# baskuit/R-NaD

Hardware: AMD Instinct MI355X
Metric: env_steps_per_sec (rollout + R-NaD update, one iteration of learn/rnad.py:495-526 per step) (higher is better)
Workload: dtype f32; 1 GPU; depth-6 3x3 matrix tree, C=1, S=66431, global batch 2^20 episodes x T=12 env steps, MLP width 256, BASELINE.json configs[1]; global_batch=1048576, per_gpu_batch=1048576, T=12, T_buffer=12, parallelism=single GPU (no collectives)

## Files before the change

include/rnad_hip.h:

```cpp
#ifndef RNAD_HIP_H
#define RNAD_HIP_H

#include <stdint.h>

#ifdef __cplusplus
extern "C" {
#endif
#pragma GCC visibility push(default)

#define RNAD_MAX_ACTIONS 8
#define RNAD_MAX_TRANSITIONS 8

const char *rnad_last_error(void);
int rnad_version(void);

typedef struct rnad_tree rnad_tree_t;

int rnad_tree_create(rnad_tree_t **out, int64_t S, int C, int A, const int64_t *index, const float *value,
                     const float *chance, const float *expected_value, const float *legal, int device);
void rnad_tree_destroy(rnad_tree_t *tree);
int64_t rnad_tree_info(const rnad_tree_t *tree, int which);

int rnad_observe(const rnad_tree_t *tree, int64_t B, const int32_t *idx, int player, void *obs, int obs_half,
                 uint8_t *mask_bits, float *mask, void *stream);

int rnad_policy_head(int64_t N, int A, const float *logits, const uint8_t *mask_bits, const float *mask,
                     float *policy, float *log_policy, void *stream);

int64_t rnad_mlp_packed_size(int A, int W);
int rnad_mlp_pack(int A, int W, const float *vw0, const float *vb0, const float *vw1, const float *vb1, const float *pw0,
                  const float *pb0, const float *pw1, const float *pb1, float *packed, void *stream);
int rnad_mlp_pack_multi(int n_nets, int A, int W, const float *const *weights, float *const *packed, void *stream);
int rnad_mlp_forward(int64_t N, int A, int W, const float *packed, const void *obs, int obs_half, float *logits,
                     float *value, void *stream);
int rnad_mlp_forward_multi(int n_nets, int64_t N, int A, int W, const float *const *packed, const void *obs, int obs_half,
                           float *const *logits, float *const *value, void *stream);
int64_t rnad_mlp_backward_workspace(int64_t N, int A, int W);
int rnad_mlp_backward(int64_t N, int A, int W, const float *packed, const void *obs, int obs_half, const float *dlogits,
                      const float *dvalue, float *g_vw0, float *g_vb0, float *g_vw1, float *g_vb1, float *g_pw0,
                      float *g_pb0, float *g_pw1, float *g_pb1, float *workspace, void *stream);

int64_t rnad_compact_workspace(int64_t N);
int rnad_compact_valid(int64_t N, const int32_t *indices, int32_t *rows, int64_t *n_rows, int32_t *block_counts, void *stream);
int rnad_mlp_forward_rows(int64_t max_rows, const int32_t *rows, const int64_t *n_rows, int A, int W, const float *packed,
                          const void *obs, int obs_half, float *logits, float *value, void *stream);
int rnad_mlp_backward_rows(int64_t max_rows, const int32_t *rows, const int64_t *n_rows, int A, int W, const float *packed,
                           const void *obs, int obs_half, const float *dlogits, const float *dvalue, float *g_vw0,
                           float *g_vb0, float *g_vw1, float *g_vb1, float *g_pw0, float *g_pb0, float *g_pw1, float *g_pb1,
                           float *workspace, void *stream);

int rnad_conv_supported(int A, int Ch, int depth);
int64_t rnad_conv_packed_size(int A, int Ch, int depth);
int64_t rnad_conv_param_count(int A, int Ch, int depth);
int rnad_conv_pack(int A, int Ch, int depth, const float *const *weights, float *packed, void *stream);
int rnad_conv_forward(int64_t N, const int32_t *rows, const int64_t *n_rows, int A, int Ch, int depth, const float *packed,
                      const float *obs, float *logits, float *value, void *stream);
int64_t rnad_conv_backward_workspace(int64_t N, int A, int Ch, int depth);
int rnad_conv_backward(int64_t N, const int32_t *rows, const int64_t *n_rows, int A, int Ch, int depth, const float *packed,
                       const float *obs, const float *dlogits, const float *dvalue, float *grads, float *workspace, void *stream);

int64_t rnad_mlp_fold_packed_size(int A, int W);
int rnad_mlp_pack_fold_multi(int n_nets, int A, int W, const float *const *weights, float *const *packed, void *stream);
int rnad_mlp_forward_fold(int n_nets, int64_t N, const int32_t *rows, const int64_t *n_rows, int A, int W, const float *const *packed,
                          const void *obs, int obs_half, float *const *logits, float *const *value, void *stream);
int rnad_mlp_forward_actor(const rnad_tree_t *tree, const int32_t *rows, const int64_t *n_rows, int W, int fold, const float *packed,
                           const void *obs, int obs_half, float *logits, float *policy_rows, void *stream);
int rnad_mlp_backward_fold(int64_t N, const int32_t *rows, const int64_t *n_rows, int A, int W, const float *packed, const void *obs,
                           int obs_half, const float *dlogits, const float *dvalue, float *g_vw0, float *g_vb0, float *g_vw1, float *g_vb1,
                           float *g_pw0, float *g_pb0, float *g_pw1, float *g_pb1, float *workspace, void *stream);

int rnad_sample(int64_t B, int n, const float *probs, const float *noise, uint64_t seed, int64_t lane0, int step,
                int stream_id, int32_t *out, void *stream);

int rnad_transition(const rnad_tree_t *tree, int64_t B, const int32_t *idx, const int32_t *row_actions,
                    const int32_t *col_actions, const float *noise, uint64_t seed, int64_t lane0, int step,
                    int32_t *idx_out, float *reward, int32_t *alive, void *stream);

typedef struct rnad_traj {
    int32_t T_cap;
    int32_t obs_half;
    int64_t B;
    int32_t *indices;
    void *observations;
    uint8_t *mask_bits;
    float *policy;
    int32_t *actions;
    float *rewards;
    float *values;
    int32_t *alive;
} rnad_traj_t;

int rnad_rollout_begin(const rnad_tree_t *tree, const rnad_traj_t *traj, void *stream);

int rnad_rollout_step(const rnad_tree_t *tree, const rnad_traj_t *traj, int t, int mode, const float *logits,
                      const float *policy_in, const int32_t *actions_in, const float *value,
                      const float *noise_action, const float *noise_chance, uint64_t seed, int64_t lane0,
                      void *stream);

int rnad_rollout_run(const rnad_tree_t *tree, const rnad_traj_t *traj, int W, const float *packed, float *logits_ws,
                     int64_t logits_step_stride, float *value_ws, uint64_t seed, int64_t lane0, int32_t *live_rows,
                     int64_t *n_live, int32_t *block_counts, void *stream);

int rnad_rollout_run_tabular(const rnad_tree_t *tree, const rnad_traj_t *traj, const float *logits_table,
                             const float *value_table, uint64_t seed, int64_t lane0, void *stream);

int rnad_rollout_end(const rnad_tree_t *tree, const rnad_traj_t *traj, void *stream);

int rnad_process_policy(int64_t N, int A, const float *policy, const float *mask, int n_disc, float eps,
                        float *out, void *stream);

int rnad_vtrace(int T, int64_t B, int A, const float *v, const float *valid, const int32_t *player_id,
                const float *mu, const float *pi, const float *logpi, const void *actions, int actions_onehot,
                const float *reward, int player, float eta, float lambda_, float c, float rho, float gamma,
                float *v_target, int32_t *has_played, float *q, void *stream);

int rnad_mask_sum(int64_t N, const float *mask, double *out, void *stream);
int rnad_loss_v(int64_t N, const float *v, const float *v_target, const float *mask, const double *norm, float weight,
                double *loss, float *dv, int accumulate, void *stream);
int rnad_loss_nerd(int64_t N, int A, const float *logit, const float *pi, const float *q, const float *mask,
                   const float *legal, const double *norm, float clip, float threshold, float weight, double *loss,
                   float *dlogit, int accumulate, void *stream);

typedef struct rnad_learn_params {
    float alpha, one_minus_alpha;
    float eta, lambda_, c, rho, gamma;
    float clip, threshold;
    float w_v, w_n;
    float eps_threshold;
    int32_t n_disc;
} rnad_learn_params_t;

int rnad_learn_fused(int T, int64_t B, int A, const int32_t *indices, const uint8_t *mask_bits,
                     const int32_t *actions, const float *rewards, const float *mu, const float *logit,
                     const float *v, const float *v_target_net, const float *logit_reg, const float *logit_reg_,
                     const double *norm, const rnad_learn_params_t *hp, double *losses, float *dlogit, float *dv,
                     float *pi_out, float *v_target_out, float *q_out, void *stream);

int64_t rnad_learn_tabular_workspace(const rnad_tree_t *tree, int T, int64_t B);
int rnad_learn_fused_tabular(const rnad_tree_t *tree, int T, int64_t B, const int32_t *indices, const uint8_t *mask_bits,
                             const int32_t *actions, const float *rewards, const float *mu, const float *logit_tab,
                             const float *v_tab, const float *v_target_tab, const float *logit_reg_tab,
                             const float *logit_reg_tab_, const double *norm, const rnad_learn_params_t *hp, double *losses,
                             void *workspace, float *dlogit_tab, float *dv_tab, void *stream);
int64_t rnad_row_sums_workspace(const rnad_tree_t *tree);
int rnad_row_sums(const rnad_tree_t *tree, int T, int64_t B, const int32_t *indices, const float *dlogit, const float *dv,
                  void *workspace, float *dlogit_tab, float *dv_tab, void *stream);

int64_t rnad_learn_gather_workspace(const rnad_tree_t *tree);
int rnad_learn_fused_gather(const rnad_tree_t *tree, int T, int64_t B, const int32_t *indices, const uint8_t *mask_bits,
                            const int32_t *actions, const float *rewards, const float *mu, const float *logit_tab,
                            const float *v_tab, const float *v_target_tab, const float *logit_reg_tab,
                            const float *logit_reg_tab_, const double *norm, const rnad_learn_params_t *hp, double *losses,
                            void *workspace, float *dlogit, float *dv, void *stream);

typedef struct rnad_step_params {
    uint64_t seed;
    float alpha, one_minus_alpha;
} rnad_step_params_t;
typedef struct rnad_row_groups {
    int32_t n_groups;
    const int32_t *start;
    const int32_t *order;
    const int32_t *first;
    int32_t rows_below_cut;
} rnad_row_groups_t;

int rnad_step_params_set(rnad_step_params_t *device_params, uint64_t seed, float alpha, float one_minus_alpha, void *stream);
#define RNAD_STEP_QUEUE 32
typedef struct rnad_step_queue {
    rnad_step_params_t live;
    int64_t cursor, n;
    rnad_step_params_t ahead[RNAD_STEP_QUEUE];
} rnad_step_queue_t;
int rnad_step_queue_set(rnad_step_queue_t *device_queue, int n, const rnad_step_params_t *entries, void *stream);
int rnad_bucket_plan(const rnad_tree_t *tree, int64_t B, int64_t *out);
int rnad_bucket_map(const rnad_tree_t *tree, int64_t B, int32_t *bucket_of, int32_t *n_groups);
int rnad_bucket_shared_steps(const rnad_tree_t *tree, int64_t B, int32_t *n_shared);
int rnad_rollout_bucketed(const rnad_tree_t *tree, const rnad_traj_t *traj, const float *table, int64_t table_stride,
                          int table_is_policy, const float *value_table, int64_t value_stride, uint64_t seed, int64_t lane0,
                          const rnad_step_params_t *device_params, void *scratch, int32_t *lane_ids, int32_t *items, int32_t *n_items,
                          double *norm, void *stream);
int rnad_rollout_bucketed_compact(const rnad_tree_t *tree, int T_cap, int64_t B, const float *table, int64_t table_stride,
                                  int table_is_policy, uint64_t seed, int64_t lane0, const rnad_step_params_t *device_params,
                                  void *scratch, int32_t *lane_ids, int32_t *items, int32_t *n_items, double *norm, void *states,
                                  int32_t *alive, uint64_t *acts, float *final_reward, int32_t *visited, void *stream);
int rnad_rollout_bucketed_compact_expand(const rnad_tree_t *tree, int T_cap, int64_t B, const float *table, int64_t table_stride,
                                         int table_is_policy, uint64_t seed, int64_t lane0, const rnad_step_params_t *device_params,
                                         void *scratch, int32_t *lane_ids, int32_t *items, int32_t *n_items, double *norm, void *states,
                                         int32_t *alive, uint64_t *acts, float *final_reward, int32_t *visited, const int32_t *rep_of,
                                         int n_tables, float *const *tables, const int32_t *floats_per_row, void *stream);
#define RNAD_PLAY_LEARN_FINISH 1
#define RNAD_PLAY_LEARN_DISTINCT 2
typedef struct rnad_leaf_paths {
    int64_t n_cols;
    int32_t rows, T_cap;
    const void *states;
    const uint64_t *acts;
    const float *final_reward;
    const int32_t *items;
    const int32_t *n_items;
    int32_t max_items;
    const int32_t *col_of;
    int32_t *col_count;
    const int32_t *bucket_col0;
    int32_t crowded_lanes;
} rnad_leaf_paths_t;
int rnad_leaf_paths_pack(const rnad_tree_t *tree, int64_t plan_B, int T1, int64_t n_cols, const int32_t *indices, const int32_t *items,
                         const int32_t *n_items, int32_t max_items, void *states, int32_t *mismatch, int32_t *rows_out, int32_t *rel_bytes_out,
                         void *stream);
int rnad_rollout_learn_bucketed_compact(const rnad_tree_t *tree, int T_cap, int64_t B, const float *table, int64_t table_stride,
                                        uint64_t seed, int64_t lane0, const rnad_step_params_t *device_params, void *scratch,
                                        int32_t *lane_ids, int32_t *items, int32_t *n_items, double *norm, void *states, int32_t *alive,
                                        uint64_t *acts, float *final_reward, const int32_t *rep_of, int n_tables, float *const *tables,
                                        const int32_t *floats_per_row, const float *fast_records, const rnad_learn_params_t *hp,
                                        void *accumulators, int flags, const double *norm_global, float *dlogit_tab, float *dv_tab,
                                        const int32_t *rows, const int64_t *n_rows, const rnad_row_groups_t *groups,
                                        const rnad_leaf_paths_t *leaf, void *stream);
int rnad_bucket_indices(const rnad_tree_t *tree, int T1, int64_t B, const void *states, const int32_t *items, const int32_t *n_items,
                        int32_t *indices, void *stream);
int rnad_bucket_pack_states(const rnad_tree_t *tree, int T1, int64_t B, const int32_t *indices, const int32_t *items,
                            const int32_t *n_items, void *states, int32_t *mismatch, void *stream);
int rnad_bucket_expand(const rnad_tree_t *tree, int T, int64_t B, const int32_t *indices, const uint64_t *acts,
                       const float *final_reward, const float *records, uint8_t *mask_bits, float *policy, int32_t *actions,
                       float *rewards, void *stream);
int rnad_bucket_log_stats(const rnad_tree_t *tree, int T, int64_t B, const void *states, const int32_t *items, const int32_t *n_items,
                          const int32_t *alive, const float *records, const float *logit_target_tab, float *row_stats, double *out,
                          void *stream);
int64_t rnad_bucket_record_stride(int A);
int64_t rnad_bucket_fast_record_stride(int A);
int64_t rnad_bucket_policy_row_stride(int A);
int rnad_bucket_records(const rnad_tree_t *tree, const float *logit_tab, const float *v_tab, const float *v_target_tab,
                        const float *logit_reg_tab, const float *logit_reg_tab_, const rnad_learn_params_t *hp,
                        const rnad_step_params_t *device_params, float *records, float *fast_records, float *policy_rows,
                        const int32_t *rows, const int64_t *n_rows, void *stream);
int rnad_rows_expand(int64_t rows, const int32_t *rep_of, int n_tables, float *const *tables, const int32_t *floats_per_row, void *stream);
int rnad_rows_segment_sum(int n_groups, const int32_t *start, const int32_t *order, int A, float *dlogit_tab, float *dv_tab, void *stream);

int rnad_mlp_rows_records_supported(int A, int W, int fold, int policy_from_table);
int rnad_mlp_rows_actor_supported(int A, int W, int fold);
int rnad_mlp_rows_actor(const rnad_tree_t *tree, const int32_t *rows, const int64_t *n_rows, int W, int fold, const float *packed, const void *obs,
                        int obs_half, float *logits, float *policy_rows, void *stream);
int rnad_mlp_rows_records(const rnad_tree_t *tree, int W, int fold, const float *packed_net, const float *packed_target, const void *obs,
                          int obs_half, const int32_t *rows, const int64_t *n_rows, int policy_from_table, float *logit_tab, float *v_tab,
                          float *v_target_tab, const float *logit_reg_tab, const float *logit_reg_tab_, const rnad_learn_params_t *hp,
                          const rnad_step_params_t *device_params, float *records, float *fast_records, float *policy_rows, void *stream);
int rnad_learn_bucketed(const rnad_tree_t *tree, int T, int64_t B, const int32_t *indices, const int32_t *actions,
                        const float *rewards, const float *mu, const float *records, const int32_t *items, const int32_t *n_items,
                        const double *norm, const rnad_learn_params_t *hp, void *accumulators, double *losses, float *dlogit_tab,
                        float *dv_tab, void *stream);
int rnad_learn_bucketed_compact(const rnad_tree_t *tree, int T, int64_t B, const void *states, const uint64_t *acts,
                                const float *final_reward, const float *fast_records, const float *records, const int32_t *items,
                                const int32_t *n_items, const double *norm, const rnad_learn_params_t *hp, void *accumulators,
                                double *losses, float *dlogit_tab, float *dv_tab, const int32_t *rows, const int64_t *n_rows,
                                const void *rollout_scratch, int rollout_T_cap, int32_t *alive, double *norm_out,
                                const rnad_row_groups_t *groups, void *stream);
int rnad_bucket_alive(const rnad_tree_t *tree, int T_cap, int64_t B, const void *scratch, int32_t *alive, double *norm, void *stream);
int rnad_bucket_sort(const rnad_tree_t *tree, int T_cap, int64_t B, const float *table, int64_t table_stride, int table_is_policy,
                     uint64_t seed, int64_t lane0, const rnad_step_params_t *device_params, void *scratch, int32_t *lane_ids,
                     int32_t *items, int32_t *n_items, double *norm, int32_t *group_flags, int32_t *staged_rows, int64_t *n_staged,
                     int32_t *visited, void *stage, int32_t *stage_rows0, void *stream);
int64_t rnad_bucket_stage_bytes(const rnad_tree_t *tree, int64_t B);
int rnad_bucket_stage_rows(const rnad_tree_t *tree, int64_t B, int level, uint64_t seed, const rnad_step_params_t *device_params, void *stage,
                           int32_t *rows, void *stream);
int rnad_bucket_stage_walk(const rnad_tree_t *tree, int T_cap, int64_t B, const float *policy_rows, int64_t stride, uint64_t seed, int64_t lane0,
                           const rnad_step_params_t *device_params, const void *scratch, const int32_t *lane_ids, void *stage, void *stream);
int rnad_bucket_play(const rnad_tree_t *tree, int T_cap, int64_t B, const float *table, int64_t table_stride, int table_is_policy,
                     const int32_t *rows, const int64_t *n_rows, uint64_t seed, int64_t lane0, const rnad_step_params_t *device_params,
                     void *scratch, const int32_t *lane_ids, const int32_t *items, const int32_t *n_items, double *norm, void *states,
                     int32_t *alive, uint64_t *acts, float *final_reward, int32_t *visited, int visited_is_clear, void *stream);
int rnad_bucket_finish(const rnad_tree_t *tree, int64_t B, const double *norm, const rnad_learn_params_t *hp, void *accumulators,
                       double *losses, float *dlogit_tab, float *dv_tab, const int32_t *rows, const int64_t *n_rows,
                       const rnad_row_groups_t *groups, void *stream);

int rnad_clip_grad_norm(int64_t n, float *grads, float max_norm, float *total_norm, void *stream);

typedef struct rnad_adam_params {
    float lr, beta1, beta2, eps;
    float max_norm;
    float ema;
} rnad_adam_params_t;
int rnad_optimizer_step(int n_tensors, const int64_t *sizes, float *const *param, float *grads, float *const *exp_avg,
                        float *const *exp_avg_sq, float *const *step, float *const *target, const rnad_adam_params_t *hp,
                        float *total_norm, int mlp_A, int mlp_W, int mlp_fold, float *packed_param, float *packed_target, rnad_step_queue_t *advance,
                        uint32_t *ticket, void *stream);
int rnad_nashconv(const rnad_tree_t *tree, const float *joint_policy, const float *root_policy,
                  int64_t state_index, float reach, float *row_best, float *col_best, float *reach_out,
                  int32_t *depth_out, void *stream);
int rnad_observe_all(const rnad_tree_t *tree, float *obs_row, float *obs_col, void *stream);

int64_t rnad_tree_generate(int A, int C, int depth_bound, float transition_threshold, const float *terminal_values,
                           int n_terminal_values, int prune_num, int prune_den, uint64_t seed, int64_t capacity,
                           int64_t *index, float *value, float *chance, float *expected_value, float *legal,
                           float *root_value, float *solution);
int rnad_solve_matrix(const float *M, int ra, int ca, int max_actions, float *solution, float *value);

int rnad_prof_enable(int mask);
int rnad_prof_read(int which, int64_t *launches, double *total_ms);

#pragma GCC visibility pop
#ifdef __cplusplus
}
#endif
#endif
```

r-nad_amd/csrc/bucket.hip:

```cpp
#include "learn_math.hpp"
#include "row_records.hpp"
#include "rollout_math.hpp"

#include <algorithm>
#include <cstdlib>
#include <utility>

using namespace rnad;
using namespace rnad::dev;

#ifndef RNAD_ABLATE
#define RNAD_ABLATE 0
#endif

namespace {

constexpr int kThreads = 256;
constexpr int kMaxPath = 32;
#ifndef RNAD_PATH_SLOTS
#define RNAD_PATH_SLOTS 16
#endif
constexpr int kPathSlots = RNAD_PATH_SLOTS;
constexpr int kMaxBuckets = 12288;
constexpr int kMaxUpper = 8192;
constexpr int kSortThreads = 1024;
constexpr int kSortLanes = 4096;
constexpr int kChunkDefault = 256;
constexpr int kReplicas = 64;
constexpr int kMaxSteps = 64;
constexpr int kLaneBits = 22;
constexpr int kLearnLds = 64 * 1024;
constexpr int kKeysLds = 144 * 1024;
constexpr int kPackedSteps = 10;
constexpr int kCompactSteps = 21;
constexpr int kSharedRoot = 256;
constexpr int kFinishRows = 4;
constexpr int kTicketGroups = 64;
constexpr int kTargetLanes = 1024;
constexpr int kMinLanesLevelCut = 128;

#ifndef RNAD_PLAY_LDS
#define RNAD_PLAY_LDS 1
#endif
constexpr int kPlayLds = RNAD_PLAY_LDS;
constexpr int kMinSortTile = kSortThreads * kPlayLds > 1024 ? kSortThreads * kPlayLds : 1024;
#define RNAD_DISPATCH_TILE(p_, ...)                                                          \
    switch ((p_).tile) {                                                                     \
        case 1024: { constexpr int kTile = kMinSortTile > 1024 ? kMinSortTile : 1024; __VA_ARGS__; } break; \
        case 2048: { constexpr int kTile = kMinSortTile > 2048 ? kMinSortTile : 2048; __VA_ARGS__; } break; \
        case 8192: { constexpr int kTile = 8192; __VA_ARGS__; } break;                        \
        default: { constexpr int kTile = kSortLanes; __VA_ARGS__; } break;                    \
    }

inline unsigned blocks_for(int64_t n, int per = kThreads) { return (unsigned)((n + per - 1) / per); }

struct Switch {
    bool set;
    int v;
};
struct Switches {
    Switch bucket_rows;
    Switch bucket_chunk;
    Switch sort_tile;
    Switch keys_stage_bytes;
    Switch keys_global;
    Switch keys_lds;
    Switch keys_hybrid;
    Switch expand_blocks;
    Switch scatter_rows;
    Switch fused_distinct;
    Switch fused_chunk;
};
Switches read_switches() {
    auto read = [](const char *name) {
        const char *text = getenv(name);
        return text ? Switch{true, atoi(text)} : Switch{false, 0};
    };
    return {read("RNAD_BUCKET_ROWS"), read("RNAD_BUCKET_CHUNK"), read("RNAD_SORT_TILE"), read("RNAD_KEYS_STAGE_BYTES"),
            read("RNAD_KEYS_GLOBAL"), read("RNAD_KEYS_LDS"), read("RNAD_KEYS_HYBRID"), read("RNAD_EXPAND_BLOCKS"),
            read("RNAD_SCATTER_ROWS"), read("RNAD_FUSED_DISTINCT"), read("RNAD_FUSED_CHUNK")};
}

struct Plan {
    const BucketCut *cut = nullptr;
    int lds = 0, path_words = 0, sort_blocks = 0, chunk = kChunkDefault;
    int tile = kSortLanes;
    int rel_bytes = 1;
    int forced = 0;
    int64_t max_items = 0;
};

struct UpperWalk {
    int32_t next, key;
    float chance;
};

__global__ __launch_bounds__(kThreads) void k_upper_walk(int n, int AAC, const int32_t *__restrict__ upper_list, const Trans *__restrict__ trans,
                                                         const int32_t *__restrict__ bucket_of, UpperWalk *__restrict__ out) {
    const int i = blockIdx.x * kThreads + threadIdx.x;
    if (i >= n * AAC) return;
    const Trans t = trans[(int64_t)upper_list[i / AAC] * AAC + i % AAC];
    out[i] = UpperWalk{t.next, bucket_of[t.next], t.chance};
}

struct HostCut {
    int rows = 0, n_groups = 0, n_upper = 0, n_buckets = 0, max_path = 0;
    std::vector<int32_t> bucket_of, lo, span, path, upper_list, path_states;
    std::vector<int32_t> group_by_lo;
    std::vector<int32_t> anchor1;
};

HostCut build_cut(const rnad_tree_t *tree, int rows) {
    HostCut h;
    h.rows = rows;
    const int64_t S = tree->S;
    std::vector<int32_t> &bucket_of = h.bucket_of, &lo = h.lo, &span = h.span, &path = h.path, &upper_list = h.upper_list;
    bucket_of.assign((size_t)S, -1);
    h.anchor1.assign((size_t)S, 0);
    auto anchor_below = [&](int64_t c) {
        for (int64_t i = tree->child_offsets[(size_t)c]; i < tree->child_offsets[(size_t)c + 1]; ++i) {
            const int64_t d = tree->children[(size_t)i], d_hi = d + tree->subtree_size[(size_t)d];
            for (int64_t x = d; x < d_hi; ++x) h.anchor1[(size_t)x] = (int32_t)d;
        }
    };
    std::vector<int32_t> parent_upper((size_t)S, 0);
    std::vector<int32_t> group_parent;
    auto is_upper = [&](int64_t s) { return tree->subtree_size[(size_t)s] > rows; };
    if (!is_upper(1)) {
        lo.push_back(1);
        span.push_back((int32_t)tree->subtree_size[1]);
        path.push_back(kSharedRoot);
        group_parent.push_back(0);
        anchor_below(1);
        for (int64_t s = 1; s < S; ++s)
            if (tree->level_of[(size_t)s] >= 0) bucket_of[(size_t)s] = 0;
    } else {
        for (int64_t u = 1; u < S; ++u) {
            if (tree->level_of[(size_t)u] < 0 || !is_upper(u)) continue;
            upper_list.push_back((int32_t)u);
            const int level = tree->level_of[(size_t)u];
            int64_t g_lo = -1, g_hi = -1;
            int g_subtrees = 0;
            auto close = [&]() {
                if (g_lo < 0) return;
                const int32_t gid = (int32_t)lo.size();
                lo.push_back((int32_t)g_lo);
                span.push_back((int32_t)(g_hi - g_lo));
                path.push_back(2 * (level + 1) | (g_subtrees == 1 ? kSharedRoot : 0));
                group_parent.push_back((int32_t)u);
                for (int64_t x = g_lo; x < g_hi; ++x) bucket_of[(size_t)x] = gid;
                g_lo = g_hi = -1;
            };
            for (int64_t i = tree->child_offsets[(size_t)u]; i < tree->child_offsets[(size_t)u + 1]; ++i) {
                const int64_t c = tree->children[(size_t)i];
                if (is_upper(c)) {
                    parent_upper[(size_t)c] = (int32_t)u;
                    close();
                    continue;
                }
                const int64_t c_hi = c + tree->subtree_size[(size_t)c];
                anchor_below(c);
                if (g_lo >= 0 && c == g_hi && c_hi - g_lo <= rows) {
                    g_hi = c_hi;
                    ++g_subtrees;
                } else {
                    close();
                    g_lo = c;
                    g_hi = c_hi;
                    g_subtrees = 1;
                }
            }
            close();
        }
    }
    h.n_groups = (int)lo.size();
    h.n_upper = (int)upper_list.size();
    h.n_buckets = h.n_groups + h.n_upper;
    for (int i = 0; i < h.n_upper; ++i) {
        const int32_t u = upper_list[(size_t)i];
        bucket_of[(size_t)u] = h.n_groups + i;
        lo.push_back(u);
        span.push_back(0);
        path.push_back(2 * tree->level_of[(size_t)u] + 2);
        group_parent.push_back(u);
    }
    int max_path = 0;
    for (int32_t v : path) max_path = std::max(max_path, (int)(v & (kSharedRoot - 1)) + ((v & kSharedRoot) ? 2 : 0));
    h.max_path = max_path;
    const int stride = std::max(max_path, 1);
    h.path_states.assign((size_t)h.n_buckets * stride, 0);
    if (max_path <= kMaxPath) {
        for (int b = 0; b < h.n_buckets; ++b) {
            int32_t *row = h.path_states.data() + (size_t)b * stride;
            for (int32_t u = group_parent[(size_t)b]; u != 0; u = parent_upper[(size_t)u]) {
                const int l = tree->level_of[(size_t)u];
                row[2 * l] = row[2 * l + 1] = u;
            }
            if (path[(size_t)b] & kSharedRoot) {
                const int n_path = path[(size_t)b] & (kSharedRoot - 1);
                row[n_path] = row[n_path + 1] = lo[(size_t)b];
            }
        }
    }
    if (upper_list.empty()) upper_list.push_back(0);
    h.group_by_lo.resize((size_t)h.n_groups);
    for (int g = 0; g < h.n_groups; ++g) h.group_by_lo[(size_t)g] = g;
    std::sort(h.group_by_lo.begin(), h.group_by_lo.end(), [&](int32_t a, int32_t b) { return lo[(size_t)a] < lo[(size_t)b]; });
    return h;
}

bool cut_fits(const HostCut &c) { return c.n_buckets <= kMaxBuckets && c.n_upper <= kMaxUpper && c.max_path <= kMaxPath; }

const BucketCut *get_cut(const rnad_tree_t *tree, int rows, const Switches &sw) {
    auto it = tree->cuts.find(rows);
    if (it != tree->cuts.end()) return &it->second;
    HostCut h = build_cut(tree, rows);
    BucketCut cut;
    cut.rows = rows;
    cut.n_groups = h.n_groups;
    cut.n_upper = h.n_upper;
    cut.n_buckets = h.n_buckets;
    cut.max_path = h.max_path;
    DeviceGuard guard(tree->device);
    auto up = [&](int32_t **dst, const std::vector<int32_t> &src) {
        if (hipMalloc((void **)dst, std::max<size_t>(src.size(), 1) * sizeof(int32_t)) != hipSuccess) return false;
        return src.empty() || hipMemcpy(*dst, src.data(), src.size() * sizeof(int32_t), hipMemcpyHostToDevice) == hipSuccess;
    };
    if (!guard.ok || !up(&cut.bucket_of, h.bucket_of) || !up(&cut.bucket_lo, h.lo) || !up(&cut.bucket_path, h.path) ||
        !up(&cut.upper_list, h.upper_list) || !up(&cut.path_states, h.path_states) || !up(&cut.bucket_span, h.span) ||
        !up(&cut.group_by_lo, h.group_by_lo) || !up(&cut.anchor1, h.anchor1)) {
        for (int32_t *ptr : {cut.bucket_of, cut.bucket_lo, cut.bucket_path, cut.upper_list, cut.path_states, cut.bucket_span, cut.group_by_lo, cut.anchor1})
            if (ptr) (void)hipFree(ptr);
        return nullptr;
// ... 546 lines not shown
                }
            }
        }
#pragma unroll
        for (int l = 0; l < L; ++l) {
            const int64_t b = b0 + (int64_t)l * kSortThreads;
            my_keys[pass][l] = b < B ? key[l] : -1;
            if (b < B) {
                keys[b] = key[l];
                decisions[b] = packed[l] | ((unsigned long long)min(steps[l], kPackedSteps) << 60);
                if (stage.root) {
                    const int root = key[l] < n_groups ? state[l] : 0;
                    stage.root[b] = (uint32_t)root | ((uint32_t)steps[l] << kStageRootBits);
                    if (root) stage.mark0[root] = stage_stamp(seed);
                }
            }
        }
    }
    __syncthreads();
    int32_t *cnt = reinterpret_cast<int32_t *>(keys_smem);
    for (int i = threadIdx.x; i < n_buckets; i += kSortThreads) cnt[i] = 0;
    __syncthreads();
#pragma unroll
    for (int pass = 0; pass < kPasses; ++pass)
#pragma unroll
        for (int l = 0; l < L; ++l)
            if (my_keys[pass][l] >= 0) atomicAdd(&cnt[my_keys[pass][l]], 1);
    __syncthreads();
    int32_t *row = hist + (int64_t)blockIdx.x * n_buckets;
    for (int i = threadIdx.x; i < n_buckets; i += kSortThreads) row[i] = cnt[i];
}

template <int TILE>
__global__ __launch_bounds__(kSortThreads) void k_bucket_hist(int64_t B, int n_buckets, const int32_t *__restrict__ keys,
                                                              int32_t *__restrict__ hist) {
    extern __shared__ int32_t cnt[];
    for (int i = threadIdx.x; i < n_buckets; i += kSortThreads) cnt[i] = 0;
    __syncthreads();
    const int64_t base = (int64_t)blockIdx.x * TILE;
#pragma unroll
    for (int r = 0; r < TILE / kSortThreads; ++r) {
        const int64_t b = base + (int64_t)r * kSortThreads + threadIdx.x;
        if (b < B) atomicAdd(&cnt[keys[b]], 1);
    }
    __syncthreads();
    int32_t *row = hist + (int64_t)blockIdx.x * n_buckets;
    for (int i = threadIdx.x; i < n_buckets; i += kSortThreads) row[i] = cnt[i];
}

#ifndef RNAD_XCD_ITEMS
#define RNAD_XCD_ITEMS 1
#endif
__device__ __forceinline__ int xcd_item(int n) {
#if RNAD_XCD_ITEMS
    const int q = n >> 3, r = n & 7, xcd = (int)blockIdx.x & 7, k = (int)blockIdx.x >> 3;
    const int cnt = q + (xcd < r ? 1 : 0), start = xcd < r ? xcd * (q + 1) : r * (q + 1) + (xcd - r) * q;
    return k < cnt ? start + k : -1;
#else
    return (int)blockIdx.x < n ? (int)blockIdx.x : -1;
#endif
}

constexpr int kStagePer = 4;
template <int LEVEL>
__device__ __forceinline__ void stage_rows_chunk(int64_t chunk, int64_t S, const uint32_t *__restrict__ mark, const int32_t *__restrict__ anchor1,
                                                 uint32_t stamp, int32_t *__restrict__ rows, unsigned long long *__restrict__ count) {
    __shared__ int32_t wave_n[kSortThreads / 64];
    __shared__ unsigned long long base_s;
    const int lane = threadIdx.x & 63, wave = threadIdx.x >> 6;
    const int64_t s0 = (chunk * (kSortThreads / 64) + wave) * (kStagePer * 64) + lane;
    uint64_t votes[kStagePer];
    int32_t mine = 0;
#pragma unroll
    for (int r = 0; r < kStagePer; ++r) {
        const int64_t s = s0 + r * 64;
        bool hit = false;
        if (s > 0 && s < S) {
            if (LEVEL == 0) {
                hit = mark[s] == stamp;
            } else {
                const int32_t a = anchor1[s];
                hit = a != 0 && mark[a] == stamp;
            }
        }
        votes[r] = __ballot(hit);
        mine += (int32_t)__popcll(votes[r]);
    }
    if (lane == 0) wave_n[wave] = mine;
    __syncthreads();
    int32_t before = 0, total = 0;
#pragma unroll
    for (int w = 0; w < kSortThreads / 64; ++w) {
        if (w < wave) before += wave_n[w];
        total += wave_n[w];
    }
    if (threadIdx.x == 0) base_s = total ? atomicAdd(count, 2ull * (unsigned long long)total) : 0ull;
    __syncthreads();
    unsigned long long at = base_s + 2ull * (unsigned long long)before;
#pragma unroll
    for (int r = 0; r < kStagePer; ++r) {
        if ((votes[r] >> lane) & 1ull) {
            const unsigned long long mine_at = at + 2ull * (unsigned long long)__popcll(votes[r] & ((1ull << lane) - 1ull));
            rows[mine_at] = (int32_t)(s0 + r * 64);
            rows[mine_at + 1] = (int32_t)(S + s0 + r * 64);
        }
        at += 2ull * (unsigned long long)__popcll(votes[r]);
    }
    __syncthreads();
}

template <int LEVEL>
__global__ __launch_bounds__(kSortThreads) void k_stage_rows(int64_t S, const uint32_t *__restrict__ mark, const int32_t *__restrict__ anchor1,
                                                             uint64_t seed, const rnad_step_params_t *__restrict__ sp,
                                                             int32_t *__restrict__ rows, unsigned long long *__restrict__ count) {
    if (sp) seed = sp->seed;
    stage_rows_chunk<LEVEL>(blockIdx.x, S, mark, anchor1, stage_stamp(seed), rows, count);
}

template <int A>
__global__ __launch_bounds__(kThreads) void k_stage_walk(const Trans *__restrict__ trans, int C, int64_t S, int64_t B, int T_cap,
                                                         const float *__restrict__ policy_tab, int64_t tab_stride, int vec4,
                                                         const uint32_t *__restrict__ sorted, const int32_t *__restrict__ lane_ids,
                                                         uint64_t seed, const rnad_step_params_t *__restrict__ sp, int64_t lane0,
                                                         uint32_t *__restrict__ mark1) {
    const int nb = (int)gridDim.x, xq = nb >> 3, xr = nb & 7, xcd = (int)blockIdx.x & 7, xk = (int)blockIdx.x >> 3;
    const int64_t blk = (xcd < xr ? xcd * (xq + 1) : xr * (xq + 1) + (xcd - xr) * xq) + xk;
    if (xk >= xq + (xcd < xr ? 1 : 0)) return;
    const int64_t j = blk * kThreads + threadIdx.x;
    if (j >= B) return;
    const uint32_t word = sorted[j];
    const int root = (int)(word & ((1u << kStageRootBits) - 1u)), t = (int)(word >> kStageRootBits);
    if (root == 0 || t + 1 >= T_cap) return;
    if (sp) seed = sp->seed;
    const int64_t b = lane_ids[j];
    float pol0[A], pol1[A], u[3];
    load_policy_row<A>(policy_tab, root, tab_stride, vec4 != 0, pol0);
    load_policy_row<A>(policy_tab, S + root, tab_stride, vec4 != 0, pol1);
    rnad_decision_uniforms(seed, (uint64_t)(lane0 + b), (uint32_t)t, u);
    const int a0 = pick<A>(pol0, u[0]), a1 = pick<A>(pol1, u[1]);
    int next;
    float rew;
    transition_lane<A>(trans, C, root, a0, a1, nullptr, u[2], next, rew);
    if (next != 0) mark1[next] = stage_stamp(seed);
}

constexpr int kScanCols = 16, kScanParts = kSortThreads / kScanCols;

struct Item {
    int32_t begin, count, bucket, single;
};

constexpr int kItemsInline = 16;

__device__ __forceinline__ void items_phase(int n_buckets, int chunk, const int32_t *__restrict__ totals, int32_t *__restrict__ start_s,
                                            int32_t *__restrict__ first_s, bool write_items, Item *__restrict__ items,
                                            int32_t *__restrict__ n_items, int32_t *__restrict__ bucket_start_out = nullptr) {
    __shared__ int32_t wave_l[16], wave_i[16];
    __shared__ int32_t total_s, most;
    if (threadIdx.x == 0) most = 0;
    __syncthreads();
    const int per = (n_buckets + kSortThreads - 1) / kSortThreads;
    const int b0 = min(n_buckets, (int)threadIdx.x * per), b1 = min(n_buckets, b0 + per);
    int32_t own_l = 0, own_i = 0;
    bool big = false;
    for (int i = b0; i < b1; ++i) {
        const int32_t n = totals[i], ni = (n + chunk - 1) / chunk;
        own_l += n;
        own_i += ni;
        big |= ni > kItemsInline;
    }
    if (big) most = kItemsInline + 1;
    int32_t sl = own_l, si = own_i;
#pragma unroll
    for (int off = 1; off < 64; off <<= 1) {
        const int32_t a = __shfl_up(sl, off, 64), b = __shfl_up(si, off, 64);
        if ((int)(threadIdx.x & 63) >= off) {
            sl += a;
            si += b;
        }
    }
    if ((threadIdx.x & 63) == 63) {
        wave_l[threadIdx.x >> 6] = sl;
        wave_i[threadIdx.x >> 6] = si;
    }
    __syncthreads();
    int32_t run_l = sl - own_l, run_i = si - own_i;
    for (int w = 0; w < (int)(threadIdx.x >> 6); ++w) {
        run_l += wave_l[w];
        run_i += wave_i[w];
    }
    if (threadIdx.x == kSortThreads - 1) total_s = run_i + own_i;
    for (int i = b0; i < b1; ++i) {
        const int32_t n = totals[i], ni = (n + chunk - 1) / chunk;
        start_s[i] = run_l;
        first_s[i] = run_i;
        if (write_items && bucket_start_out) bucket_start_out[i] = run_l;
        run_l += n;
        run_i += ni;
    }
    __syncthreads();
    const int32_t total = total_s;
    if (threadIdx.x == 0) {
        first_s[n_buckets] = total;
        if (write_items) *n_items = total;
    }
    __syncthreads();
    if (!write_items) return;
    if (most <= kItemsInline) {
        for (int i = threadIdx.x; i < n_buckets; i += kSortThreads) {
            const int32_t n = totals[i], first = first_s[i], ni = first_s[i + 1] - first, start = start_s[i];
            for (int32_t j = 0; j < ni; ++j) items[first + j] = Item{start + j * chunk, min(chunk, n - j * chunk), i, ni == 1 ? 1 : 0};
        }
        return;
    }
    for (int32_t k = threadIdx.x; k < total; k += kSortThreads) {
        int lo = 0, hi = n_buckets;
        while (hi - lo > 1) {
            const int mid = (lo + hi) >> 1;
            if (first_s[mid] <= k) lo = mid;
            else hi = mid;
        }
        const int32_t n = totals[lo], j = k - first_s[lo], start = start_s[lo];
        items[k] = Item{start + j * chunk, min(chunk, n - j * chunk), lo, n <= chunk ? 1 : 0};
    }
}

__global__ __launch_bounds__(kSortThreads) void k_bucket_scan(int n_blocks, int n_buckets, int32_t *__restrict__ hist,
                                                              int32_t *__restrict__ totals, int scan_blocks, KeysExpand ex) {
    if ((int)blockIdx.x >= scan_blocks) {
        keys_expand_share(ex, kSortThreads, (int)blockIdx.x - scan_blocks, (int)gridDim.x - scan_blocks);
        return;
    }
    __shared__ int32_t part[kScanParts][kScanCols + 1];
    const int col = threadIdx.x & (kScanCols - 1), g = threadIdx.x / kScanCols;
    const int c = blockIdx.x * kScanCols + col;
    const int per = (n_blocks + kScanParts - 1) / kScanParts, r0 = min(n_blocks, g * per), r1 = min(n_blocks, r0 + per);
    constexpr int kScanKeep = 16;
    const bool keep = per <= kScanKeep;
    int32_t v[kScanKeep];
    int32_t sum = 0;
    if (c < n_buckets) {
        if (keep) {
#pragma unroll
            for (int k = 0; k < kScanKeep; ++k) v[k] = r0 + k < r1 ? hist[(int64_t)(r0 + k) * n_buckets + c] : 0;
#pragma unroll
            for (int k = 0; k < kScanKeep; ++k) sum += v[k];
        } else {
            for (int r = r0; r < r1; ++r) sum += hist[(int64_t)r * n_buckets + c];
        }
    }
    part[g][col] = sum;
    __syncthreads();
    if (g == 0) {
        int32_t run = 0;
        for (int i = 0; i < kScanParts; ++i) {
            const int32_t x = part[i][col];
            part[i][col] = run;
            run += x;
        }
        if (c < n_buckets) totals[c] = run;
    }
    __syncthreads();
    if (c < n_buckets) {
        int32_t before = part[g][col];
        if (keep) {
#pragma unroll
            for (int k = 0; k < kScanKeep; ++k) {
                if (r0 + k < r1) hist[(int64_t)(r0 + k) * n_buckets + c] = before;
                before += v[k];
            }
        } else {
            for (int r = r0; r < r1; ++r) {
                const int32_t x = hist[(int64_t)r * n_buckets + c];
                hist[(int64_t)r * n_buckets + c] = before;
                before += x;
            }
        }
    }
}

template <int TILE>
__global__ __launch_bounds__(kSortThreads) void k_bucket_scatter(int64_t B, int n_buckets, const int32_t *__restrict__ keys,
                                                                 const int32_t *__restrict__ hist, const int32_t *__restrict__ totals, int chunk,
                                                                 Item *__restrict__ items, int32_t *__restrict__ n_items,
                                                                 int32_t *__restrict__ lane_ids, int wave_rows, int64_t S, int n_groups,
                                                                 const int32_t *__restrict__ bucket_lo, const int32_t *__restrict__ bucket_span,
                                                                 const int32_t *__restrict__ group_by_lo, int32_t *__restrict__ staged_rows,
                                                                 int64_t *__restrict__ n_staged, int32_t *__restrict__ visited,
                                                                 const uint32_t *__restrict__ stage_root, uint32_t *__restrict__ stage_sorted,
                                                                 const uint32_t *__restrict__ stage_mark0, int32_t *__restrict__ stage_rows0,
                                                                 unsigned long long *__restrict__ stage_count0, uint64_t seed,
                                                                 const rnad_step_params_t *__restrict__ sp, int32_t *__restrict__ bucket_start_out) {
    extern __shared__ int32_t cnt[];
    const int wave = threadIdx.x >> 6, lane = threadIdx.x & 63;
    const int64_t base = (int64_t)blockIdx.x * TILE + (int64_t)wave * (TILE / 16);
    int32_t key[TILE / kSortThreads];
    uint32_t root_word[TILE / kSortThreads];
#pragma unroll
    for (int r = 0; r < TILE / kSortThreads; ++r) {
        const int64_t b = base + r * 64 + lane;
        key[r] = b < B ? keys[b] : -1;
        root_word[r] = (stage_root && b < B) ? stage_root[b] : 0u;
    }
    if (visited) {
        for (int64_t r = (int64_t)blockIdx.x * kSortThreads + threadIdx.x; r < 2 * S; r += (int64_t)gridDim.x * kSortThreads)
            visited[r] = (r == 0 || r == S) ? 1 : 0;
    }
    if (stage_rows0) {
        if (sp) seed = sp->seed;
        const int64_t n_chunks = (S + kSortThreads * kStagePer - 1) / (kSortThreads * kStagePer);
        for (int64_t chunk = blockIdx.x; chunk < n_chunks; chunk += gridDim.x)
            stage_rows_chunk<0>(chunk, S, stage_mark0, nullptr, stage_stamp(seed), stage_rows0, stage_count0);
    }
    if (staged_rows) {
        __shared__ int32_t wave_s[16];
        __shared__ int32_t carry_s;
        int32_t *pre = cnt;
        if (threadIdx.x == 0) carry_s = 0;
        __syncthreads();
        for (int k0 = 0; k0 < n_groups; k0 += kSortThreads) {
            const int k = k0 + threadIdx.x;
            const int g = k < n_groups ? group_by_lo[k] : 0;
            const int32_t n = (k < n_groups && totals[g] > 0) ? bucket_span[g] : 0;
            int32_t incl = n;
#pragma unroll
            for (int off = 1; off < 64; off <<= 1) {
                const int32_t o = __shfl_up(incl, off, 64);
                if (lane >= off) incl += o;
            }
            if (lane == 63) wave_s[wave] = incl;
            __syncthreads();
            int32_t before = carry_s;
            for (int w = 0; w < wave; ++w) before += wave_s[w];
            if (k < n_groups) pre[k] = before + incl - n;
            __syncthreads();
            if (threadIdx.x == kSortThreads - 1) carry_s = before + incl;
            __syncthreads();
        }
        const int32_t total = carry_s;
        if (blockIdx.x == 0 && threadIdx.x == 0) *n_staged = 2 * (int64_t)total;
        for (int k = blockIdx.x * 16 + wave; k < n_groups; k += gridDim.x * 16) {
            const int g = group_by_lo[k];
            if (totals[g] <= 0) continue;
            const int32_t lo = bucket_lo[g], n = bucket_span[g], at = pre[k];
            for (int j = lane; j < n; j += 64) {
                staged_rows[at + j] = lo + j;
                staged_rows[total + at + j] = (int32_t)S + lo + j;
            }
        }
        __syncthreads();
    }
    const int32_t *row = hist + (int64_t)blockIdx.x * n_buckets;
    const int32_t row_first = (int)threadIdx.x < n_buckets ? row[threadIdx.x] : 0;
    items_phase(n_buckets, chunk, totals, cnt, cnt + n_buckets, blockIdx.x == 0, items, n_items, bucket_start_out);
    __syncthreads();
    if ((int)threadIdx.x < n_buckets) cnt[threadIdx.x] += row_first;
    for (int i = threadIdx.x + kSortThreads; i < n_buckets; i += kSortThreads) cnt[i] += row[i];
    __syncthreads();
    const int R = wave_rows, G = 16 / R, my_row = wave / G;
    int32_t *wcnt = cnt + 2 * n_buckets + 1;
    for (int i = threadIdx.x; i < R * n_buckets; i += kSortThreads) wcnt[i] = 0;
    __syncthreads();
    int32_t rank[TILE / kSortThreads];
    for (int turn = 0; turn < G; ++turn) {
        if (wave % G == turn) {
#pragma unroll
            for (int r = 0; r < TILE / kSortThreads; ++r) rank[r] = key[r] >= 0 ? atomicAdd(&wcnt[my_row * n_buckets + key[r]], 1) : 0;
        }
        __syncthreads();
    }
    for (int i = threadIdx.x; i < n_buckets; i += kSortThreads) {
        int32_t at = cnt[i];
        for (int w = 0; w < R; ++w) {
            const int32_t n = wcnt[w * n_buckets + i];
            wcnt[w * n_buckets + i] = at;
            at += n;
        }
    }
    __syncthreads();
#pragma unroll
    for (int r = 0; r < TILE / kSortThreads; ++r)
        if (key[r] >= 0) {
            const int32_t at = wcnt[my_row * n_buckets + key[r]] + rank[r];
            lane_ids[at] = (int32_t)(base + r * 64 + lane);
            if (stage_sorted) stage_sorted[at] = root_word[r];
        }
}

template <int A>
__global__ __launch_bounds__(kThreads) void k_bucket_rollout(const Trans *__restrict__ trans, int C, int64_t S, int64_t B, int T_cap,
                                                             const float *__restrict__ policy_tab, int64_t tab_stride,
                                                             const float *__restrict__ value_tab, int64_t value_stride,
                                                             const uint8_t *__restrict__ mask_tab, uint64_t seed,
                                                             const rnad_step_params_t *__restrict__ sp, int64_t lane0,
                                                             const int32_t *__restrict__ lane_ids,
                                                             const unsigned long long *__restrict__ decisions, int32_t *__restrict__ indices,
                                                             uint8_t *__restrict__ mbits, float *__restrict__ policy,
                                                             int32_t *__restrict__ actions, float *__restrict__ rewards,
                                                             float *__restrict__ values, int32_t *__restrict__ alive_part) {
    __shared__ int32_t cnt[kThreads / 64][kMaxSteps + 1];
    const int64_t j = (int64_t)blockIdx.x * kThreads + threadIdx.x;
    const bool active = j < B;
    if (sp) seed = sp->seed;
    const int32_t lane_local = active ? lane_ids[j] : 0;
    const uint64_t lane = (uint64_t)(lane0 + lane_local);
    const unsigned long long packed = active ? decisions[lane_local] : 0ull;
    const int n_packed = (int)(packed >> 60);
    const int wave = threadIdx.x >> 6;
    int state = 1, prev = 0;
    float u[3] = {0.0f, 0.0f, 0.0f};
    for (int t = 0; t < T_cap; ++t) {
        const uint64_t live = __ballot(active && state != 0);
        if ((threadIdx.x & 63) == 0) cnt[wave][t] = (int32_t)__popcll(live);
        if (active) {
            if (!(t & 1) && t + 1 >= n_packed) rnad_decision_uniforms(seed, lane, (uint32_t)t, u);
            const int64_t i = (int64_t)t * B + j;
            const int64_t row = (int64_t)(t & 1) * S + state;
            const bool replay = t < n_packed;
            const int bits6 = replay ? (int)(packed >> (6 * t)) & 63 : 0;
            int action = bits6 & 7;
            const uint32_t bits = mask_tab[row];
            float pol[A];
#pragma unroll
            for (int a = 0; a < A; ++a) pol[a] = policy_tab[row * tab_stride + a];
            if (!replay) action = pick<A>(pol, u[t & 1]);
            indices[i] = state;
            mbits[i] = (uint8_t)bits;
#pragma unroll
            for (int a = 0; a < A; ++a) policy[i * A + a] = pol[a];
            actions[i] = action;
            if (values) values[i] = value_tab ? value_tab[row * value_stride] : 0.0f;
            int next = state;
            float rew = 0.0f;
            if (t & 1) {
                if (replay)
                    transition_apply<A>(trans, C, state, prev, action, bits6 >> 3, next, rew);
                else
                    transition_lane<A>(trans, C, state, prev, action, nullptr, u[2], next, rew);
            } else {
                prev = action;
            }
            rewards[i] = rew;
            state = next;
        }
    }
    const uint64_t live = __ballot(active && state != 0);
    if ((threadIdx.x & 63) == 0) cnt[wave][T_cap] = (int32_t)__popcll(live);
    if (active) indices[(int64_t)T_cap * B + j] = state;
    __syncthreads();
    if ((int)threadIdx.x <= T_cap) {
        int32_t s = 0;
#pragma unroll
        for (int w = 0; w < kThreads / 64; ++w) s += cnt[w][threadIdx.x];
        alive_part[(int64_t)blockIdx.x * (T_cap + 1) + threadIdx.x] = s;
    }
}

template <typename T>
__device__ __forceinline__ const T *at_bytes(const void *base, uint32_t byte_offset) {
    return reinterpret_cast<const T *>(reinterpret_cast<const char *>(base) + byte_offset);
}
template <typename T>
__device__ __forceinline__ T *at_bytes(void *base, uint32_t byte_offset) {
    return reinterpret_cast<T *>(reinterpret_cast<char *>(base) + byte_offset);
}

template <typename REL>
__device__ __forceinline__ REL rel_of(int state, int lo) {
    return (REL)(state == 0 ? 0 : state - lo + 1);
}

#ifndef RNAD_ROLLOUT_LANES
#define RNAD_ROLLOUT_LANES 1
#endif
constexpr int kRolloutLanes = RNAD_ROLLOUT_LANES;

struct Hand {
    unsigned long long acts, relq;
    float reward;
    int final_rel;
};
constexpr int kHandPairs = 4;

struct Distinct {
    int32_t *count = nullptr;
    int32_t *n = nullptr;
    int32_t *key = nullptr;
    int32_t *column = nullptr;
    int codes = 0;
    int keys = 0;
};

constexpr int kLeafHist = 1024;
struct LeafCount {
    int32_t *col_count = nullptr;
    const int32_t *bucket_col0 = nullptr;
    const int32_t *lane_total = nullptr;
    int32_t crowded_lanes = 0;
};
__device__ __forceinline__ bool leaf_crowded(const LeafCount &lc, int bucket) {
    return lc.col_count != nullptr && lc.crowded_lanes > 0 && lc.lane_total[bucket] >= lc.crowded_lanes &&
           lc.bucket_col0[bucket + 1] - lc.bucket_col0[bucket] <= kLeafHist;
}

template <int A, typename REL, int L, bool DISTINCT = false, bool HIST = false>
__device__ __forceinline__ void rollout_items_body(const Trans *__restrict__ trans, int C, int64_t S, int64_t B, int T_cap,
                                                                   const float *__restrict__ policy_tab, int64_t tab_stride, int vec4,
                                                                   uint64_t seed, const rnad_step_params_t *__restrict__ sp, int64_t lane0,
                                                                   const int32_t *__restrict__ lane_ids,
                                                                   const unsigned long long *__restrict__ decisions,
                                                                   const Item *__restrict__ items, const int32_t *__restrict__ n_items,
                                                                   const int32_t *__restrict__ bucket_path, const int32_t *__restrict__ bucket_lo,
                                                                   const int32_t *__restrict__ path_states, int path_stride, int n_groups,
                                                                   REL *__restrict__ states, int32_t *__restrict__ alive_part,
                                                                   unsigned long long *__restrict__ acts_out,
                                                                   float *__restrict__ reward_out, int32_t *__restrict__ visited,
                                                                   double *__restrict__ norm_rep = nullptr, Hand *hand = nullptr,
                                                                   const Distinct distinct = Distinct{},
                                                                   const int32_t *__restrict__ col_of = nullptr,
                                                                   int32_t *__restrict__ leaf_col = nullptr, const LeafCount lc = LeafCount{}) {
    constexpr int NT = kThreads / L, NW = NT / 64;
    __shared__ int32_t leaf_hist[HIST ? kLeafHist : 1];
    static_assert(NT >= 64 && NT > kCompactSteps, "a wave at least, and a thread per alive counter");
    __shared__ int32_t cnt[NW][kMaxSteps + 1];
    int32_t *my_alive = alive_part + (norm_rep ? (int64_t)(blockIdx.x & (kReplicas - 1)) : (int64_t)blockIdx.x) * (T_cap + 1);
    const int my_item = xcd_item(*n_items);
    if (my_item < 0) {
        if (!norm_rep && (int)threadIdx.x <= T_cap) my_alive[threadIdx.x] = 0;
        return;
    }
    const Item item = items[my_item];
    if (sp) seed = sp->seed;
    const int wave = threadIdx.x >> 6;
    const int path_word = bucket_path[item.bucket];
    const bool shared = item.bucket < n_groups && (path_word & kSharedRoot) != 0;
    const int n_shared = (path_word & (kSharedRoot - 1)) + (shared ? 2 : 0);
    const int lo = bucket_lo[item.bucket];
    const int32_t *my_path = path_states + (int64_t)item.bucket * path_stride;
    const uint32_t B32 = (uint32_t)B;
    if ((threadIdx.x & 63) == 0)
        for (int t = 0; t <= T_cap; ++t) cnt[wave][t] = 0;
    bool count_here = false;
    int32_t col0 = 0, n_bins = 0;
    if constexpr (HIST) {
        count_here = leaf_crowded(lc, item.bucket);
        if (count_here) {
            col0 = lc.bucket_col0[item.bucket];
            n_bins = lc.bucket_col0[item.bucket + 1] - col0;
            for (int i = threadIdx.x; i < n_bins; i += NT) leaf_hist[i] = 0;
            __syncthreads();
        }
    }
    for (int base = 0; base < item.count; base += kThreads) {
        bool active[L];
        uint32_t j[L];
        int32_t lane_local[L];
        uint64_t lane[L];
        unsigned long long packed[L];
#pragma unroll
        for (int l = 0; l < L; ++l) {
            const int k = base + l * NT + (int)threadIdx.x;
            active[l] = k < item.count;
            j[l] = (uint32_t)(item.begin + k);
            lane_local[l] = active[l] ? lane_ids[j[l]] : 0;
            lane[l] = (uint64_t)(lane0 + lane_local[l]);
        }
        if (shared) {
            const unsigned long long first = decisions[lane_ids[item.begin]];
            const unsigned long long uni = ((unsigned long long)(unsigned int)__builtin_amdgcn_readfirstlane((int)(first >> 32)) << 32) |
                                           (unsigned int)__builtin_amdgcn_readfirstlane((int)first);
#pragma unroll
            for (int l = 0; l < L; ++l) packed[l] = uni;
        } else {
#pragma unroll
            for (int l = 0; l < L; ++l) packed[l] = active[l] ? decisions[lane_local[l]] : 0ull;
        }
        int state[L], n_packed[L], t_from = 0;
        unsigned long long relq = 0ull;
        int last_key[L];
        unsigned long long acts[L];
        float reward_final[L];
#pragma unroll
        for (int l = 0; l < L; ++l) {
            n_packed[l] = (int)(packed[l] >> 60);
            last_key[l] = -1;
            state[l] = active[l] ? 1 : 0;
            acts[l] = 0ull;
            reward_final[l] = 0.0f;
        }
        if (shared) {
            const int n_pre = min(min(n_packed[0], T_cap) & ~1, n_shared - 2);
            int32_t live_now = 0;
#pragma unroll
            for (int l = 0; l < L; ++l) live_now += (int32_t)__popcll(__ballot(active[l]));
            for (int t = 0; t < n_pre; t += 2) {
                if ((threadIdx.x & 63) == 0) {
                    cnt[wave][t] += live_now;
                    cnt[wave][t + 1] += live_now;
                }
                const int bits0 = (int)(packed[0] >> (6 * t)) & 63, bits1 = (int)(packed[0] >> (6 * (t + 1))) & 63;
                if (visited && threadIdx.x == 0 && base == 0) {
                    const int at = my_path[t];
                    visited[at] = visited[S + at] = 1;
                }
#pragma unroll
                for (int l = 0; l < L; ++l)
                    acts[l] |= (unsigned long long)(bits0 & 7) << (3 * t) | (unsigned long long)(bits1 & 7) << (3 * (t + 1));
            }
            t_from = n_pre;
#pragma unroll
            for (int l = 0; l < L; ++l) state[l] = active[l] ? my_path[n_pre] : 0;
        }
        for (int t = t_from; t < T_cap; t += 2) {
            const bool two = t + 1 < T_cap;
            int32_t live = 0;
#pragma unroll
            for (int l = 0; l < L; ++l) live += (int32_t)__popcll(__ballot(state[l] != 0));
            if ((threadIdx.x & 63) == 0) {
                cnt[wave][t] += live;
                if (two) cnt[wave][t + 1] += live;
            }
            bool go[L], replay0[L], replay1[L];
            float pol0[L][A], pol1[L][A], u[L][3];
#pragma unroll
            for (int l = 0; l < L; ++l) {
                go[l] = active[l];
                if (go[l] && t >= n_shared) {
                    const REL r = rel_of<REL>(state[l], lo);
                    if (hand && l == 0) relq = (relq << 16) | (unsigned long long)r;
                    *at_bytes<REL>(states, ((uint32_t)t * B32 + j[l]) * (uint32_t)sizeof(REL)) = r;
                    if (two) *at_bytes<REL>(states, ((uint32_t)(t + 1) * B32 + j[l]) * (uint32_t)sizeof(REL)) = r;
                }
                go[l] = go[l] && state[l] != 0;
                replay0[l] = t < n_packed[l];
                replay1[l] = t + 1 < n_packed[l];
                if (go[l]) {
                    const int64_t row0 = state[l], row1 = S + state[l];
                    if (visited) {
                        visited[row0] = 1;
                        if (two) visited[row1] = 1;
                    }
                    if (!replay0[l]) load_policy_row<A>(policy_tab, row0, tab_stride, vec4 != 0, pol0[l]);
                    if (two && !replay1[l]) load_policy_row<A>(policy_tab, row1, tab_stride, vec4 != 0, pol1[l]);
                }
            }
#pragma unroll
            for (int l = 0; l < L; ++l)
                if (go[l] && (!replay0[l] || (two && !replay1[l]))) rnad_decision_uniforms(seed, lane[l], (uint32_t)t, u[l]);
            int a0[L], a1[L], bits1[L];
#pragma unroll
            for (int l = 0; l < L; ++l) {
                if (!go[l]) continue;
                const int bits0 = replay0[l] ? (int)(packed[l] >> (6 * t)) & 63 : 0;
                bits1[l] = replay1[l] ? (int)(packed[l] >> (6 * (t + 1))) & 63 : 0;
                a0[l] = replay0[l] ? (bits0 & 7) : pick<A>(pol0[l], u[l][0]);
                acts[l] |= (unsigned long long)a0[l] << (3 * t);
                if (two) {
                    a1[l] = replay1[l] ? (bits1[l] & 7) : pick<A>(pol1[l], u[l][1]);
                    acts[l] |= (unsigned long long)a1[l] << (3 * (t + 1));
                }
            }
            if (two) {
#pragma unroll
                for (int l = 0; l < L; ++l) {
                    if (!go[l]) continue;
                    int next, outcome;
                    float rew;
                    if (replay1[l]) {
                        outcome = bits1[l] >> 3;
                        transition_apply<A>(trans, C, state[l], a0[l], a1[l], outcome, next, rew);
                    } else {
                        transition_lane<A>(trans, C, state[l], a0[l], a1[l], nullptr, u[l][2], next, rew, &outcome);
                    }
                    if (next == 0) {
                        reward_final[l] = rew;
                        if (DISTINCT) last_key[l] = (state[l] - lo) * distinct.codes + (a0[l] * A + a1[l]) * C + outcome;
                        if (leaf_col)
                        {
                            const int32_t col = col_of[(((uint32_t)state[l] * A + a0[l]) * A + a1[l]) * C + outcome];
                            leaf_col[j[l]] = col;
                            if constexpr (HIST)
                                if (count_here) atomicAdd(&leaf_hist[col - col0], 1);
                        }

                    }
                    state[l] = next;
                }
            }
        }
        int32_t live = 0;
#pragma unroll
        for (int l = 0; l < L; ++l) {
            if (active[l]) {
                acts_out[j[l]] = acts[l];
                reward_out[j[l]] = reward_final[l];
                if (T_cap >= n_shared) *at_bytes<REL>(states, ((uint32_t)T_cap * B32 + j[l]) * (uint32_t)sizeof(REL)) = rel_of<REL>(state[l], lo);
            }
            live += (int32_t)__popcll(__ballot(state[l] != 0));
        }
        if ((threadIdx.x & 63) == 0) cnt[wave][T_cap] += live;
        if (DISTINCT) {
#pragma unroll
            for (int l = 0; l < L; ++l) {
                if (!active[l]) continue;
                const int key = state[l] != 0 ? (state[l] - lo) * distinct.codes + distinct.codes - 1 : last_key[l];
                const bool in_table = key >= 0 && key < distinct.keys;
                if (!in_table || atomicAdd(distinct.count + key, 1) == 0) {
                    const int at = atomicAdd(distinct.n, 1);
                    distinct.key[at] = in_table ? key : distinct.keys;
                    distinct.column[at] = (int32_t)j[l];
                }
            }
        }
        if (hand) *hand = Hand{acts[0], relq, reward_final[0], active[0] ? (int)rel_of<REL>(state[0], lo) : 0};
    }
    __syncthreads();
    if constexpr (HIST) {
        if (count_here) {
            for (int i = threadIdx.x; i < n_bins; i += NT) {
                const int32_t n = leaf_hist[i];
                if (n != 0) atomicAdd(lc.col_count + col0 + i, n);
            }
        }
    }
    if ((int)threadIdx.x <= T_cap) {
        int32_t sum = 0;
#pragma unroll
        for (int w = 0; w < NW; ++w) sum += cnt[w][threadIdx.x];
        if (!norm_rep) my_alive[threadIdx.x] = sum;
        else if (sum != 0) atomicAdd(my_alive + threadIdx.x, sum);
        if (norm_rep) cnt[0][threadIdx.x] = sum;
    }
    if (norm_rep) {
        __syncthreads();
        if (threadIdx.x < 2) {
            int32_t n = 0;
            for (int t = threadIdx.x; t < T_cap; t += 2) n += cnt[0][t];
            if (n != 0) atomicAdd(norm_rep + 2 * (blockIdx.x & (kReplicas - 1)) + threadIdx.x, (double)n);
        }
    }
}

template <int A, typename REL, int L>
__global__ __launch_bounds__(kThreads / L) void k_bucket_rollout_items(const Trans *__restrict__ trans, int C, int64_t S, int64_t B, int T_cap,
                                                                   const float *__restrict__ policy_tab, int64_t tab_stride, int vec4,
                                                                   uint64_t seed, const rnad_step_params_t *__restrict__ sp, int64_t lane0,
                                                                   const int32_t *__restrict__ lane_ids,
                                                                   const unsigned long long *__restrict__ decisions,
                                                                   const Item *__restrict__ items, const int32_t *__restrict__ n_items,
                                                                   const int32_t *__restrict__ bucket_path, const int32_t *__restrict__ bucket_lo,
                                                                   const int32_t *__restrict__ path_states, int path_stride, int n_groups,
                                                                   REL *__restrict__ states, int32_t *__restrict__ alive_part,
                                                                   unsigned long long *__restrict__ acts_out,
                                                                   float *__restrict__ reward_out, int32_t *__restrict__ visited) {
    rollout_items_body<A, REL, L>(trans, C, S, B, T_cap, policy_tab, tab_stride, vec4, seed, sp, lane0, lane_ids, decisions, items, n_items,
                                  bucket_path, bucket_lo, path_states, path_stride, n_groups, states, alive_part, acts_out, reward_out, visited);
}

template <typename REL>
__global__ __launch_bounds__(kThreads) void k_bucket_indices(int T1, int64_t B, const Item *__restrict__ items, const int32_t *__restrict__ n_items,
                                                             const int32_t *__restrict__ bucket_path, const int32_t *__restrict__ bucket_lo,
                                                             const int32_t *__restrict__ path_states, int path_stride, int n_groups,
                                                             const REL *__restrict__ states, int32_t *__restrict__ indices) {
    if ((int)blockIdx.x >= *n_items) return;
    const Item item = items[blockIdx.x];
    const int path_word = bucket_path[item.bucket];
    const int n_shared = (path_word & (kSharedRoot - 1)) + ((item.bucket < n_groups && (path_word & kSharedRoot)) ? 2 : 0);
    const int lo = bucket_lo[item.bucket];
    const int32_t *my_path = path_states + (int64_t)item.bucket * path_stride;
    for (int k = threadIdx.x; k < item.count; k += kThreads) {
        const int64_t j = (int64_t)item.begin + k;
        for (int t = 0; t < T1; ++t) {
            int state;
            if (t < n_shared) {
                state = my_path[t];
            } else {
                const int r = (int)states[(int64_t)t * B + j];
                state = r == 0 ? 0 : lo + r - 1;
            }
            indices[(int64_t)t * B + j] = state;
        }
    }
}

template <typename REL>
__global__ __launch_bounds__(kThreads) void k_bucket_pack(int T1, int64_t B, int rows, const Item *__restrict__ items, const int32_t *__restrict__ n_items,
                                                          const int32_t *__restrict__ bucket_path, const int32_t *__restrict__ bucket_lo,
                                                          const int32_t *__restrict__ path_states, int path_stride, int n_groups,
                                                          const int32_t *__restrict__ indices, REL *__restrict__ states,
                                                          int32_t *__restrict__ bad, int max_count) {
    if ((int)blockIdx.x >= *n_items) return;
    const Item item = items[blockIdx.x];
    if (item.count > max_count && threadIdx.x == 0) *bad = 1;
    const int path_word = bucket_path[item.bucket];
    const int n_shared = (path_word & (kSharedRoot - 1)) + ((item.bucket < n_groups && (path_word & kSharedRoot)) ? 2 : 0);
    const int lo = bucket_lo[item.bucket];
    const int32_t *my_path = path_states + (int64_t)item.bucket * path_stride;
    for (int k = threadIdx.x; k < item.count; k += kThreads) {
        const int64_t j = (int64_t)item.begin + k;
        for (int t = 0; t < T1; ++t) {
            const int state = indices[(int64_t)t * B + j];
            if (t < n_shared) {
                if (state != my_path[t]) *bad = 1;
            } else {
                if (state != 0 && (state < lo || state - lo >= rows)) *bad = 1;
                states[(int64_t)t * B + j] = rel_of<REL>(state, lo);
            }
        }
    }
}

constexpr int kLogStat = 8;
enum { LOG_E = 0, LOG_ET = 1, LOG_K = 2, LOG_N = 3, LOG_SUM = 4, LOG_MIN = 5, LOG_MAX = 6, LOG_SPARE = 7 };

__device__ __forceinline__ unsigned long long ordered_of(double d) {
    const unsigned long long u = (unsigned long long)__double_as_longlong(d);
    return (u >> 63) ? ~u : (u | 0x8000000000000000ull);
}
__device__ __forceinline__ double double_of_ordered(unsigned long long e) {
    return __longlong_as_double((long long)((e >> 63) ? (e & 0x7fffffffffffffffull) : ~e));
}

template <int A>
__global__ __launch_bounds__(kThreads) void k_log_row_stats(int64_t rows, const float *__restrict__ rec_, const float *__restrict__ logit_target,
                                                            float *__restrict__ row_stats, double *__restrict__ out) {
    if (blockIdx.x == 0 && threadIdx.x < kLogStat) {
        double init = 0.0;
        if (threadIdx.x == LOG_MIN) init = __longlong_as_double((long long)ordered_of(__longlong_as_double(0x7ff0000000000000ll)));
        if (threadIdx.x == LOG_MAX) init = __longlong_as_double((long long)ordered_of(__longlong_as_double((long long)0xfff0000000000000ull)));
        out[threadIdx.x] = init;
    }
    const int64_t r = (int64_t)blockIdx.x * kThreads + threadIdx.x;
    if (r >= rows) return;
    constexpr int RS = kRowStride<A>;
    float rec[RS];
    const float4 *rp = reinterpret_cast<const float4 *>(rec_ + r * RS);
#pragma unroll
    for (int u = 0; u < RS / 4; ++u) {
        const float4 r4 = rp[u];
        rec[4 * u] = r4.x; rec[4 * u + 1] = r4.y; rec[4 * u + 2] = r4.z; rec[4 * u + 3] = r4.w;
    }
    const uint32_t bits = __float_as_uint(rec[3 * A + 2]) & ((1u << A) - 1u);
    float lt[A], pit[A], lpt[A];
#pragma unroll
    for (int a = 0; a < A; ++a) lt[a] = logit_target[r * A + a];
    policy_head<A>(lt, bits, pit, lpt);
    const float log_q = logf(1.0f / (float)__popc(bits));
    float e = 0.0f, et = 0.0f, k = 0.0f, sum = 0.0f, lo = rec[0], hi = rec[0];
#pragma unroll
    for (int a = 0; a < A; ++a) {
        const float lg = rec[a], pi = rec[3 * A + 3 + a];
        sum += lg;
        lo = fminf(lo, lg);
        hi = fmaxf(hi, lg);
        if ((bits >> a) & 1) {
            const float log_pi = logf(pi);
            e += pi * (log_pi - log_q);
            et += pit[a] * (logf(pit[a]) - log_q);
            k += pi * (log_pi - log_pi);
        }
    }
    float4 *o4 = reinterpret_cast<float4 *>(row_stats + r * kLogStat);
    o4[0] = float4{e, et, k, sum};
    o4[1] = float4{lo, hi, 0.0f, 0.0f};
}

struct LogAcc {
    double s[5] = {0.0, 0.0, 0.0, 0.0, 0.0};
    float lo = __builtin_inff(), hi = -__builtin_inff();
    __device__ __forceinline__ void add_row(const float *__restrict__ row_stats, uint32_t row, int count) {
        const float4 *sp = at_bytes<float4>(row_stats, row * (uint32_t)(kLogStat * sizeof(float)));
        const float4 a = sp[0], b = sp[1];
        const double c = (double)count;
        s[LOG_E] += c * (double)a.x;
        s[LOG_ET] += c * (double)a.y;
        s[LOG_K] += c * (double)a.z;
        s[LOG_N] += c;
        s[LOG_SUM] += c * (double)a.w;
        lo = fminf(lo, b.x);
        hi = fmaxf(hi, b.y);
    }
};

template <typename REL>
__global__ __launch_bounds__(kThreads) void k_log_count(int T, int64_t B, int64_t S, int tab_rows, int n_groups, const Item *__restrict__ items,
                                                        const int32_t *__restrict__ n_items, const int32_t *__restrict__ bucket_lo,
                                                        const int32_t *__restrict__ bucket_path, const int32_t *__restrict__ path_states,
                                                        int path_stride, const REL *__restrict__ states, const float *__restrict__ row_stats,
                                                        double *__restrict__ out) {
    extern __shared__ int32_t visits[];
    __shared__ double part[kThreads / 64][5];
    __shared__ float part_lo[kThreads / 64], part_hi[kThreads / 64];
    if ((int)blockIdx.x >= *n_items) return;
// ... 259 lines not shown
        unsigned long long x = 0ull;
#pragma unroll
        for (int c = 0; c < kPathSlots; ++c) x += tab[(t * kPathSlots + c) * PS + a];
        tab[kPathWords + ((t & 1) * sub_rows + (path_state[t] - s_b)) * TS + a] += x;
    }
    __syncthreads();
    const int end = (int)(S - s_b < sub_rows ? S - s_b : sub_rows);
#pragma unroll
    for (int P = 0; P < 2; ++P) {
        unsigned long long *dst0 = acc + ((int64_t)P * S + s_b) * (A + 1);
        for (int r = threadIdx.x; r < end * (A + 1); r += kThreads) {
            const int row = r / (A + 1), a = r % (A + 1);
            const unsigned long long x = tab[kPathWords + (P * sub_rows + row) * TS + a];
            if (x != 0ull && !(RNAD_ABLATE & 32)) {
                if (item.single) dst0[r] = x;
                else atomicAdd(dst0 + r, x);
            }
        }
    }
}

template <int A>
__global__ __launch_bounds__(kThreads) void k_bucket_learn(int T, int64_t B, int64_t S, int sub_rows, int path_words, int n_groups, int up_stride,
                                                           const Item *__restrict__ items, const int32_t *__restrict__ n_items,
                                                           const int32_t *__restrict__ bucket_of, const int32_t *__restrict__ bucket_lo,
                                                           const int32_t *__restrict__ bucket_path, const int32_t *__restrict__ indices,
                                                           const int32_t *__restrict__ actions, const float *__restrict__ rewards,
                                                           const float *__restrict__ mu_, const float *__restrict__ rec_,
                                                           rnad_learn_params_t hp, FixedPoint fx, unsigned long long *__restrict__ acc,
                                                           unsigned long long *__restrict__ rep, double *__restrict__ losses_raw,
                                                           int32_t *__restrict__ overflow) {
    extern __shared__ unsigned long long tab[];
    constexpr int PS = (A + 1) | 1, TS = kTabStride<A>;
    const int kPathWords = path_words;
    __shared__ int32_t path_state[kMaxPath];
    __shared__ double loss_part[kThreads / 64][4];
    if ((int)blockIdx.x >= *n_items) return;
    const Item item = items[blockIdx.x];
    const int s_b = bucket_lo[item.bucket];
    const int n_path = bucket_path[item.bucket] & (kSharedRoot - 1);
    const int n_shared = n_path + ((bucket_path[item.bucket] & kSharedRoot) ? 2 : 0);
    constexpr int RS = kRowStride<A>;
    const int n_tab = item.bucket < n_groups ? kPathWords + 2 * sub_rows * TS : n_path * kPathSlots * PS;
    for (int i = threadIdx.x; i < n_tab; i += kThreads) tab[i] = 0ull;
    __syncthreads();
    const VtHp vh{-hp.eta, hp.lambda_, hp.c, hp.rho, hp.gamma};
    double part[4] = {0.0, 0.0, 0.0, 0.0};
    bool ovf = false;
    for (int base = 0; base < item.count; base += kThreads) {
        const bool active = base + (int)threadIdx.x < item.count;
        const int64_t j = (int64_t)item.begin + base + threadIdx.x;
        Carry cy[2];
        constexpr int kFetch = kRowLearn<A>;
        struct Slot {
            int act;
            float rew;
            float mu[A];
            float rec[kFetch];
        };
        auto fetch = [&](int t, int state, Slot &o) {
            if (state == 0) return;
            const int64_t i = (int64_t)t * B + j;
            const int64_t row = (int64_t)(t & 1) * S + state;
            const float4 *rp = reinterpret_cast<const float4 *>(rec_ + row * RS);
#pragma unroll
            for (int u = 0; u < kFetch / 4; ++u) {
                const float4 r4 = rp[u];
                o.rec[4 * u] = r4.x; o.rec[4 * u + 1] = r4.y; o.rec[4 * u + 2] = r4.z; o.rec[4 * u + 3] = r4.w;
            }
            o.act = actions[i];
#pragma unroll
            for (int a = 0; a < A; ++a) o.mu[a] = mu_[i * A + a];
            o.rew = (t & 1) ? rewards[i] : 0.0f;
        };
        int s_next = active ? indices[(int64_t)(T - 1) * B + j] : 0;
        int s_next2 = (active && T >= 2) ? indices[(int64_t)(T - 2) * B + j] : 0;
        Slot nxt;
        fetch(T - 1, s_next, nxt);
        for (int t = T - 1; t >= 0; --t) {
            const int state = s_next;
            const Slot cur = nxt;
            s_next = s_next2;
            if (t >= 1) fetch(t - 1, s_next, nxt);
            s_next2 = (active && t >= 2) ? indices[(int64_t)(t - 2) * B + j] : 0;
            const bool valid = state != 0;
            const int P = t & 1;
            long long q[A + 1];
#pragma unroll
            for (int a = 0; a <= A; ++a) q[a] = 0;
            if (valid) {
                const int act = cur.act;
                const float *rec = cur.rec;
                const uint32_t bits = __float_as_uint(rec[3 * A + 2]);
                float mu[A], lg[A], pip[A], lpol[A], legal[A], oh[A];
#pragma unroll
                for (int a = 0; a < A; ++a) {
                    mu[a] = cur.mu[a];
                    lg[a] = rec[a];
                    pip[a] = rec[A + 2 + a];
                    lpol[a] = rec[2 * A + 2 + a];
                    legal[a] = (float)((bits >> a) & 1);
                    oh[a] = act == a ? 1.0f : 0.0f;
                }
                const float rew = cur.rew;
                const float vtn = rec[A + 1];
                float vt[2], qv[2][A];
                vtrace_step<A>(cy[0], vh, true, P == 0, 1.0f, vtn, rew, mu, pip, lpol, oh, vt[0], qv[0]);
                vtrace_step<A>(cy[1], vh, true, P == 1, 1.0f, vtn, -rew, mu, pip, lpol, oh, vt[1], qv[1]);
                const float d = rec[A] - (P ? vt[1] : vt[0]);
                float qp[A], g[A];
#pragma unroll
                for (int a = 0; a < A; ++a) qp[a] = P ? qv[1][a] : qv[0][a];
                const float nerd = nerd_row<A>(lg, pip, qp, legal, hp.clip, hp.threshold, g);
                part[P] += (double)(d * d);
                part[2 + P] += -(double)nerd;
                const float gv = 2.0f * d;
                ovf |= !(fabsf(gv) < fx.limit_v);
                q[A] = round_to_ll((double)gv * fx.scale_v);
#pragma unroll
                for (int a = 0; a < A; ++a) {
                    ovf |= !(fabsf(g[a]) < fx.limit_l);
                    q[a] = round_to_ll((double)(-g[a]) * fx.scale_l);
                }
            } else {
                cy[0] = Carry{};
                cy[1] = Carry{};
            }
            if (t < n_shared) {
                if (threadIdx.x == 0 && base == 0) path_state[t] = state;
                if (valid) {
                    unsigned long long *dst = tab + (t * kPathSlots + (threadIdx.x & (kPathSlots - 1))) * PS;
#pragma unroll
                    for (int a = 0; a <= A; ++a) atomicAdd(dst + a, (unsigned long long)q[a]);
                }
            } else if (valid) {
                unsigned long long *dst = tab + kPathWords + (P * sub_rows + (state - s_b)) * TS;
#pragma unroll
                for (int a = 0; a <= A; ++a) atomicAdd(dst + a, (unsigned long long)q[a]);
            }
        }
    }
    learn_epilogue<A>(tab, path_state, item, s_b, n_path, n_shared, kPathWords, sub_rows, S, n_groups, up_stride, bucket_of, part, ovf,
                      loss_part, acc, rep, losses_raw, overflow);
}

#ifndef RNAD_PHASE2_VMEM
#define RNAD_PHASE2_VMEM 0
#endif
#ifdef RNAD_LEARN_WAVES
#define RNAD_LEARN_ATTR __attribute__((amdgpu_waves_per_eu(RNAD_LEARN_WAVES, RNAD_LEARN_WAVES)))
#else
#define RNAD_LEARN_ATTR
#endif
template <int A, typename REL, bool LOSSES, bool DISTINCT = false, bool WEIGHTED = false>
__device__ __forceinline__ void learn_c_body(int T, int64_t B, int64_t S, int sub_rows, int path_words, int n_groups, int up_stride,
                                                             const Item *__restrict__ items, const int32_t *__restrict__ n_items,
                                                             const int32_t *__restrict__ bucket_of, const int32_t *__restrict__ bucket_lo,
                                                             const int32_t *__restrict__ bucket_path, const int32_t *__restrict__ path_states,
                                                             int path_stride, const REL *__restrict__ states, const float *__restrict__ rec_,
                                                             const unsigned long long *__restrict__ acts_,
                                                             const float *__restrict__ reward_, const float *__restrict__ logit_,
                                                             rnad_learn_params_t hp, FixedPoint fx, unsigned long long *__restrict__ acc,
                                                             unsigned long long *__restrict__ rep, double *__restrict__ losses_raw,
                                                             int32_t *__restrict__ overflow, const int32_t *__restrict__ alive_part,
                                                             int alive_blocks, int T1, int32_t *__restrict__ alive,
                                                             double *__restrict__ norm_out, const Hand *hand = nullptr,
                                                             const Distinct distinct = Distinct{}, const int32_t *__restrict__ leaf_col = nullptr,
                                                             const int32_t *__restrict__ lane_start = nullptr,
                                                             const int32_t *__restrict__ lane_total = nullptr, const LeafCount lc = LeafCount{}) {
    extern __shared__ unsigned long long tab[];
    constexpr int PS = (A + 1) | 1, TS = kTabStride<A>, FS = kFastStride<A>, RS = kRowStride<A>;
    const int kPathWords = path_words;
    __shared__ int32_t path_state[kMaxPath];
    __shared__ double loss_part[kThreads / 64][4];
    if (alive_part && (int)blockIdx.x < T1) alive_column(alive_blocks, T1, blockIdx.x, alive_part, alive, norm_out);
    const int my_item = xcd_item(*n_items);
    if (my_item < 0) return;
    const Item item = items[my_item];
    const int s_b = bucket_lo[item.bucket];
    const int path_word = bucket_path[item.bucket];
    const int n_path = path_word & (kSharedRoot - 1);
    const int n_shared = n_path + ((item.bucket < n_groups && (path_word & kSharedRoot)) ? 2 : 0);
    const int32_t *my_path = path_states + (uint32_t)item.bucket * (uint32_t)path_stride;
    const int n_tab = item.bucket < n_groups ? kPathWords + 2 * sub_rows * TS : n_path * kPathSlots * PS;
    for (int i = threadIdx.x; i < n_tab; i += kThreads) tab[i] = 0ull;
    if ((int)threadIdx.x < n_shared) path_state[threadIdx.x] = my_path[threadIdx.x];
    __syncthreads();
    const VtHp vh{-hp.eta, hp.lambda_, hp.c, hp.rho, hp.gamma};
    const uint32_t B32 = (uint32_t)B, S32 = (uint32_t)S;
    const int t_low = min(T, n_shared);
    double part[4] = {0.0, 0.0, 0.0, 0.0};
    bool ovf = false;
    constexpr bool by_trajectory = DISTINCT || WEIGHTED;
    __shared__ int32_t w_lds[WEIGHTED ? kThreads : 1];
    if (WEIGHTED) {
        if (leaf_crowded(lc, item.bucket)) {
            int32_t w = 0;
            if ((int)threadIdx.x < item.count) {
                w = lc.col_count[item.begin + threadIdx.x];
                if (w != 0) lc.col_count[item.begin + threadIdx.x] = 0;
            }
            w_lds[threadIdx.x] = w;
        } else {
            w_lds[threadIdx.x] = 0;
            __syncthreads();
            const int32_t l0 = lane_start[item.bucket], ln = lane_total[item.bucket];
            for (int i = threadIdx.x; i < ln; i += kThreads) {
                const uint32_t c = (uint32_t)(leaf_col[l0 + i] - item.begin);
                if (c < (uint32_t)item.count) atomicAdd(&w_lds[c], 1);
            }
        }
        __syncthreads();
    }
    const int n_work = DISTINCT ? *distinct.n : item.count;
    for (int base = 0; base < n_work; base += kThreads) {
        bool active = base + (int)threadIdx.x < n_work;
        const uint32_t j = DISTINCT ? (uint32_t)(active ? distinct.column[base + threadIdx.x] : item.begin) : (uint32_t)(item.begin + base) + threadIdx.x;
        long long weight = DISTINCT ? (long long)(active ? distinct.count[distinct.key[base + threadIdx.x]] : 0) : 1ll;
        if (WEIGHTED) {
            const int32_t w = active ? w_lds[threadIdx.x] : 0;
            weight = w;
            active = w != 0;
            if (__ballot(active) == 0ull) continue;
        }
        Carry cy[2];
        const bool handed = hand != nullptr && item.count <= kThreads;
        const unsigned long long acts = handed ? hand->acts : active ? acts_[j] : 0ull;
        const float reward_final = handed ? hand->reward : active ? reward_[j] : 0.0f;
        const int last_pair = (T - 1) >> 1;
        auto state_at = [&](int t) {
            if (handed) {
                if (t == T) return hand->final_rel;
                const int k = last_pair - (t >> 1);
                if (k < kHandPairs) return (int)((hand->relq >> (16 * k)) & 0xffffull);
            }
            return (int)*at_bytes<REL>(states, ((uint32_t)t * B32 + j) * (uint32_t)sizeof(REL));
        };
        bool after_zero = active && (T < n_shared ? false : state_at(T) == 0);
        if (t_low < T && !(RNAD_ABLATE & 8)) {
            struct Slot {
                float rec[FS];
                float lg[A];
            };
            auto fetch = [&](int t, int rel, Slot &o) {
                if (rel == 0) return;
                const uint32_t row = (uint32_t)(t & 1) * S32 + (uint32_t)(s_b + rel - 1);
                const float4 *rp = at_bytes<float4>(rec_, row * (uint32_t)(FS * sizeof(float)));
#pragma unroll
                for (int u = 0; u < FS / 4; ++u) {
                    const float4 r4 = rp[u];
                    o.rec[4 * u] = r4.x; o.rec[4 * u + 1] = r4.y; o.rec[4 * u + 2] = r4.z; o.rec[4 * u + 3] = r4.w;
                }
                if (LOSSES) {
                    const float *lp = at_bytes<float>(logit_, row * (uint32_t)(RS * sizeof(float)));
#pragma unroll
                    for (int a = 0; a < A; ++a) o.lg[a] = lp[a];
                }
            };
            int r_next = active ? state_at(T - 1) : 0;
            int r_next2 = (active && T - 2 >= t_low) ? state_at(T - 2) : 0;
            Slot nxt;
            fetch(T - 1, r_next, nxt);
            for (int t = T - 1; t >= t_low; --t) {
                const int rel = r_next;
                const Slot cur = nxt;
                r_next = r_next2;
                if (t - 1 >= t_low) fetch(t - 1, r_next, nxt);
                r_next2 = (active && t - 2 >= t_low) ? state_at(t - 2) : 0;
                const bool valid = rel != 0;
                long long q[A + 1];
#pragma unroll
                for (int a = 0; a <= A; ++a) q[a] = 0;
                if (valid) {
                    const int act = (int)(acts >> (3 * t)) & 7;
                    if (t & 1)
                        fast_slot<A, LOSSES, 1>(cur.rec, cur.lg, act, after_zero ? reward_final : 0.0f, vh, hp, fx, cy, q, part, ovf);
                    else
                        fast_slot<A, LOSSES, 0>(cur.rec, cur.lg, act, 0.0f, vh, hp, fx, cy, q, part, ovf);
#if RNAD_ABLATE & 1
                    ovf |= (q[0] ^ q[1] ^ q[A]) == 0x123456789ll;
#else
                    unsigned long long *dst = tab + kPathWords + ((t & 1) * sub_rows + (rel - 1)) * TS;
#pragma unroll
                    for (int a = 0; a <= A; ++a) atomicAdd(dst + a, (unsigned long long)(by_trajectory ? q[a] * weight : q[a]));
#endif
                } else {
                    cy[0] = Carry{};
                    cy[1] = Carry{};
                }
                after_zero = !valid;
            }
        }
        if (active && t_low > 0 && !(RNAD_ABLATE & 16)) {
            auto row_of = [&](int t, int state) { return (uint32_t)(t & 1) * S32 + (uint32_t)state; };
            auto load_rec = [&](uint32_t row, float (&f)[FS], float (&lg)[A]) {
#if RNAD_PHASE2_VMEM
                asm volatile("" : "+v"(row));
                const float4 *r4p = at_bytes<float4>(rec_, row * (uint32_t)(FS * sizeof(float)));
#pragma unroll
                for (int u = 0; u < FS / 4; ++u) {
                    const float4 r4 = r4p[u];
                    f[4 * u] = r4.x; f[4 * u + 1] = r4.y; f[4 * u + 2] = r4.z; f[4 * u + 3] = r4.w;
                }
#else
                const float *rp = at_bytes<float>(rec_, row * (uint32_t)(FS * sizeof(float)));
#pragma unroll
                for (int u = 0; u < FS; ++u) f[u] = rp[u];
#endif
                if (LOSSES) {
                    const float *lp = at_bytes<float>(logit_, row * (uint32_t)(RS * sizeof(float)));
#pragma unroll
                    for (int a = 0; a < A; ++a) lg[a] = lp[a];
                }
            };
            auto slot = [&](int t, const float (&f)[FS], const float (&lg)[A]) {
                const int act = (int)(acts >> (3 * t)) & 7;
                long long q[A + 1];
                if (t & 1)
                    fast_slot<A, LOSSES, 1>(f, lg, act, after_zero ? reward_final : 0.0f, vh, hp, fx, cy, q, part, ovf);
                else
                    fast_slot<A, LOSSES, 0>(f, lg, act, 0.0f, vh, hp, fx, cy, q, part, ovf);
                after_zero = false;
#if RNAD_ABLATE & 1
                ovf |= (q[0] ^ q[1] ^ q[A]) == 0x123456789ll;
#else
                unsigned long long *dst = tab + (t * kPathSlots + (threadIdx.x & (kPathSlots - 1))) * PS;
#pragma unroll
                for (int a = 0; a <= A; ++a) atomicAdd(dst + a, (unsigned long long)(by_trajectory ? q[a] * weight : q[a]));
#endif
            };
            float fa[FS], la[A], fb[FS], lb[A];
            int t = t_low - 1;
            load_rec(row_of(t, __builtin_amdgcn_readfirstlane(my_path[t])), fa, la);
            if (!(t & 1)) {
                slot(t, fa, la);
                --t;
                if (t >= 0) load_rec(row_of(t, __builtin_amdgcn_readfirstlane(my_path[t])), fa, la);
            }
            for (; t >= 1; t -= 2) {
                load_rec(row_of(t - 1, __builtin_amdgcn_readfirstlane(my_path[t - 1])), fb, lb);
                slot(t, fa, la);
                if (t >= 2) load_rec(row_of(t - 2, __builtin_amdgcn_readfirstlane(my_path[t - 2])), fa, la);
                slot(t - 1, fb, lb);
            }
        }
    }
    learn_epilogue<A>(tab, path_state, item, s_b, n_path, n_shared, kPathWords, sub_rows, S, n_groups, up_stride, bucket_of, part, ovf,
                      loss_part, acc, rep, losses_raw, overflow);
}

template <int A, typename REL, bool LOSSES, bool WEIGHTED = false>
__global__ __launch_bounds__(kThreads) RNAD_LEARN_ATTR void k_bucket_learn_c(int T, int64_t B, int64_t S, int sub_rows, int path_words, int n_groups, int up_stride,
                                                             const Item *__restrict__ items, const int32_t *__restrict__ n_items,
                                                             const int32_t *__restrict__ bucket_of, const int32_t *__restrict__ bucket_lo,
                                                             const int32_t *__restrict__ bucket_path, const int32_t *__restrict__ path_states,
                                                             int path_stride, const REL *__restrict__ states, const float *__restrict__ rec_,
                                                             const unsigned long long *__restrict__ acts_,
                                                             const float *__restrict__ reward_, const float *__restrict__ logit_,
                                                             rnad_learn_params_t hp, FixedPoint fx, unsigned long long *__restrict__ acc,
                                                             unsigned long long *__restrict__ rep, double *__restrict__ losses_raw,
                                                             int32_t *__restrict__ overflow, const int32_t *__restrict__ alive_part,
                                                             int alive_blocks, int T1, int32_t *__restrict__ alive,
                                                             double *__restrict__ norm_out, const int32_t *__restrict__ leaf_col,
                                                             const int32_t *__restrict__ lane_start, const int32_t *__restrict__ lane_total,
                                                             LeafCount lc) {
    learn_c_body<A, REL, LOSSES, false, WEIGHTED>(T, B, S, sub_rows, path_words, n_groups, up_stride, items, n_items, bucket_of, bucket_lo, bucket_path,
                                                  path_states, path_stride, states, rec_, acts_, reward_, logit_, hp, fx, acc, rep, losses_raw, overflow,
                                                  alive_part, alive_blocks, T1, alive, norm_out, nullptr, Distinct{}, leaf_col, lane_start, lane_total, lc);
}

template <int A, typename REL>
__global__ __launch_bounds__(kThreads) void k_bucket_play_count(const Trans *__restrict__ trans, int C, int64_t S, int64_t B, int T_cap,
                                                                const float *__restrict__ policy_tab, int64_t tab_stride, int vec4, uint64_t seed,
                                                                const rnad_step_params_t *__restrict__ sp, int64_t lane0,
                                                                const int32_t *__restrict__ lane_ids,
                                                                const unsigned long long *__restrict__ decisions, const Item *__restrict__ items,
                                                                const int32_t *__restrict__ n_items, const int32_t *__restrict__ bucket_path,
                                                                const int32_t *__restrict__ bucket_lo, const int32_t *__restrict__ path_states,
                                                                int path_stride, int n_groups, REL *__restrict__ states,
                                                                int32_t *__restrict__ alive_rep, double *__restrict__ norm_rep,
                                                                unsigned long long *__restrict__ acts_out, float *__restrict__ reward_out,
                                                                const int32_t *__restrict__ col_of, int32_t *__restrict__ leaf_col, LeafCount lc) {
    rollout_items_body<A, REL, 1, false, true>(trans, C, S, B, T_cap, policy_tab, tab_stride, vec4, seed, sp, lane0, lane_ids, decisions, items, n_items,
                                  bucket_path, bucket_lo, path_states, path_stride, n_groups, states, alive_rep, acts_out, reward_out, nullptr,
                                  norm_rep, nullptr, Distinct{}, col_of, leaf_col, lc);
}

#ifndef RNAD_HANDOVER
#define RNAD_HANDOVER 0
#endif
#ifndef RNAD_PLAY_LEARN_WAVES
#define RNAD_PLAY_LEARN_WAVES 0
#endif
#if RNAD_PLAY_LEARN_WAVES > 0
#define RNAD_PLAY_LEARN_ATTR __attribute__((amdgpu_waves_per_eu(RNAD_PLAY_LEARN_WAVES, RNAD_PLAY_LEARN_WAVES)))
#else
#define RNAD_PLAY_LEARN_ATTR
#endif
template <int A, typename REL, bool DISTINCT>
__global__ __launch_bounds__(kThreads) RNAD_PLAY_LEARN_ATTR void k_bucket_play_learn(
    const Trans *__restrict__ trans, int C, int64_t S, int64_t B, int T_cap, const float *__restrict__ policy_tab, int64_t tab_stride, int vec4,
    uint64_t seed, const rnad_step_params_t *__restrict__ sp, int64_t lane0, const int32_t *__restrict__ lane_ids,
    const unsigned long long *__restrict__ decisions, const Item *__restrict__ items, const int32_t *__restrict__ n_items,
    const int32_t *__restrict__ bucket_path, const int32_t *__restrict__ bucket_lo, const int32_t *__restrict__ path_states, int path_stride,
    int n_groups, REL *states, int32_t *__restrict__ alive_rep, double *__restrict__ norm_rep, unsigned long long *acts, float *reward,
    int sub_rows, int path_words, int up_stride, const int32_t *__restrict__ bucket_of, const float *__restrict__ rec_, rnad_learn_params_t hp,
    FixedPoint fx, unsigned long long *__restrict__ acc, unsigned long long *__restrict__ rep, int32_t *__restrict__ overflow,
    int distinct_words, int distinct_keys, int distinct_capacity) {
    extern __shared__ unsigned long long lds_all[];
    Distinct dd;
    dd.count = reinterpret_cast<int32_t *>(lds_all + distinct_words);
    dd.n = dd.count + distinct_keys + 1;
    dd.key = dd.n + 1;
    dd.column = dd.key + distinct_capacity;
    dd.codes = A * A * C + 1;
    dd.keys = distinct_keys;
    if (DISTINCT) {
        for (int i = threadIdx.x; i < distinct_keys + 2; i += kThreads) dd.count[i] = i == distinct_keys ? 1 : 0;
        __syncthreads();
    }
    Hand hand{0ull, 0ull, 0.0f, 0};
    rollout_items_body<A, REL, 1, DISTINCT>(trans, C, S, B, T_cap, policy_tab, tab_stride, vec4, seed, sp, lane0, lane_ids, decisions, items, n_items,
                                  bucket_path, bucket_lo, path_states, path_stride, n_groups, states, alive_rep, acts, reward, nullptr, norm_rep,
                                  RNAD_HANDOVER ? &hand : nullptr, dd);
    learn_c_body<A, REL, false, DISTINCT>(T_cap, B, S, sub_rows, path_words, n_groups, up_stride, items, n_items, bucket_of, bucket_lo, bucket_path,
                                path_states, path_stride, states, rec_, acts, reward, nullptr, hp, fx, acc, rep, nullptr, overflow, nullptr, 0,
                                T_cap + 1, nullptr, nullptr, RNAD_HANDOVER ? &hand : nullptr, dd);
}

template <int A>
__global__ __launch_bounds__(kThreads) void k_bucket_finish(int64_t S, int row_blocks, const int32_t *__restrict__ row_list,
                                                            const int64_t *__restrict__ n_rows, int n_upper, int n_groups,
                                                            const int32_t *__restrict__ upper_list, const int32_t *__restrict__ bucket_of,
                                                            unsigned long long *__restrict__ acc, unsigned long long *__restrict__ rep,
                                                            const double *__restrict__ norm, float w_v, float w_n, FixedPoint fx,
                                                            int32_t *__restrict__ overflow, double *__restrict__ losses_raw,
                                                            double *__restrict__ losses, float *__restrict__ dlogit_tab,
                                                            float *__restrict__ dv_tab, int upper_blocks, int n_multi,
                                                            const int32_t *__restrict__ multi_start,
                                                            const int32_t *__restrict__ multi_order,
                                                            const int32_t *__restrict__ multi_first, int rows_below_cut,
                                                            int32_t *__restrict__ alive_rep,
                                                            double *__restrict__ norm_rep, int T1, int32_t *__restrict__ alive_out,
                                                            double *__restrict__ norm_out) {
    static_assert(kReplicas == 64, "one replica per lane");
    float nf0, nf1;
    if (norm_rep) {
        double n0 = norm_rep[2 * (threadIdx.x & 63)], n1 = norm_rep[2 * (threadIdx.x & 63) + 1];
#pragma unroll
        for (int off = 32; off > 0; off >>= 1) {
            n0 += __shfl_xor(n0, off, 64);
            n1 += __shfl_xor(n1, off, 64);
        }
        nf0 = norm ? norm_of(norm) : norm_of(&n0);
        nf1 = norm ? norm_of(norm + 1) : norm_of(&n1);
        if (blockIdx.x == 0) alive_from_replicas(T1, alive_rep, norm_rep, alive_out, norm_out);
    } else {
        nf0 = norm_of(norm);
        nf1 = norm_of(norm + 1);
    }
    const bool bad = *overflow != 0;
    const float nan = __uint_as_float(0x7fc00000u);
    if (blockIdx.x == 0 && threadIdx.x == 0 && losses) {
        losses[0] = losses_raw[0] / (double)nf0 + losses_raw[1] / (double)nf1;
        losses[1] = losses_raw[2] / (double)nf0 + losses_raw[3] / (double)nf1;
    }
#ifndef RNAD_FINISH_ABLATE
#define RNAD_FINISH_ABLATE 0
#endif
    if ((int)blockIdx.x < row_blocks) {
        if (RNAD_FINISH_ABLATE & 1) return;
        const int64_t limit = row_list ? *n_rows : 2 * S;
        const int64_t stride = (int64_t)row_blocks * kThreads;
        for (int64_t i0 = (int64_t)blockIdx.x * kThreads + threadIdx.x; i0 < limit; i0 += stride * kFinishRows) {
            int64_t r[kFinishRows];
            bool on[kFinishRows];
            long long x[kFinishRows][A + 1];
#pragma unroll
            for (int k = 0; k < kFinishRows; ++k) {
                const int64_t i = i0 + k * stride;
                r[k] = i < limit ? (row_list ? (int64_t)row_list[i] : i) : 0;
                on[k] = i < limit;
            }
#pragma unroll
            for (int k = 0; k < kFinishRows; ++k) {
                const int64_t s = r[k] >= S ? r[k] - S : r[k];
                if (!rows_below_cut) on[k] = on[k] && !(n_upper > 0 && bucket_of[s] >= n_groups);
            }
#pragma unroll
            for (int k = 0; k < kFinishRows; ++k)
#pragma unroll
                for (int a = 0; a <= A; ++a) x[k][a] = on[k] ? (long long)acc[r[k] * (A + 1) + a] : 0ll;
#pragma unroll
            for (int k = 0; k < kFinishRows; ++k) {
                if (!on[k]) continue;
#pragma unroll
                for (int a = 0; a <= A; ++a)
                    if (x[k][a] != 0) acc[r[k] * (A + 1) + a] = 0ull;
                const float nf = r[k] >= S ? nf1 : nf0;
#pragma unroll
                for (int a = 0; a < A; ++a) dlogit_tab[r[k] * A + a] = bad ? nan : w_n * ((float)((double)x[k][a] * fx.inv_l) / nf);
                dv_tab[r[k]] = bad ? nan : w_v * ((float)((double)x[k][A] * fx.inv_v) / nf);
            }
        }
    } else if ((int)blockIdx.x >= row_blocks + upper_blocks) {
        const int g = ((int)blockIdx.x - row_blocks - upper_blocks) * (kThreads / 64) + (threadIdx.x >> 6), lane = threadIdx.x & 63;
        if (RNAD_FINISH_ABLATE & 2) return;
        if (g < n_multi) {
            float sum[A + 1];
#pragma unroll
            for (int a = 0; a <= A; ++a) sum[a] = 0.0f;
            auto add_rows = [&](const int64_t (&r)[kFinishRows]) {
                long long x[kFinishRows][A + 1];
#pragma unroll
                for (int k = 0; k < kFinishRows; ++k)
#pragma unroll
                    for (int a = 0; a <= A; ++a) x[k][a] = r[k] >= 0 ? (long long)acc[r[k] * (A + 1) + a] : 0ll;
#pragma unroll
                for (int k = 0; k < kFinishRows; ++k) {
                    if (r[k] < 0) continue;
#pragma unroll
                    for (int a = 0; a <= A; ++a)
                        if (x[k][a] != 0) acc[r[k] * (A + 1) + a] = 0ull;
                    const float nf = r[k] >= S ? nf1 : nf0;
#pragma unroll
                    for (int a = 0; a < A; ++a) sum[a] += bad ? nan : w_n * ((float)((double)x[k][a] * fx.inv_l) / nf);
                    sum[A] += bad ? nan : w_v * ((float)((double)x[k][A] * fx.inv_v) / nf);
                }
            };
            int64_t rep_row;
            if (multi_first) {
                int64_t r[kFinishRows];
#pragma unroll
                for (int k = 0; k < kFinishRows; ++k) r[k] = (int64_t)multi_first[((int64_t)g * kFinishRows + k) * 64 + lane];
                const int lo = multi_start[g], hi = multi_start[g + 1];
                rep_row = __shfl(r[0], 0, 64);
                add_rows(r);
                for (int i0 = lo + 64 * kFinishRows + lane; i0 < hi; i0 += 64 * kFinishRows) {
#pragma unroll
                    for (int k = 0; k < kFinishRows; ++k) r[k] = i0 + 64 * k < hi ? (int64_t)multi_order[i0 + 64 * k] : -1;
                    add_rows(r);
                }
            } else {
                const int lo = multi_start[g], hi = multi_start[g + 1];
                for (int i0 = lo + lane; i0 < hi; i0 += 64 * kFinishRows) {
                    int64_t r[kFinishRows];
#pragma unroll
                    for (int k = 0; k < kFinishRows; ++k) r[k] = i0 + 64 * k < hi ? (int64_t)multi_order[i0 + 64 * k] : -1;
                    add_rows(r);
                }
                rep_row = multi_order[lo];
            }
#pragma unroll
            for (int off = 32; off > 0; off >>= 1) {
#pragma unroll
                for (int a = 0; a <= A; ++a) sum[a] += __shfl_xor(sum[a], off, 64);
            }
            if (lane == 0) {
                const int64_t r = rep_row;
#pragma unroll
                for (int a = 0; a < A; ++a) dlogit_tab[r * A + a] = sum[a];
                dv_tab[r] = sum[A];
            }
        }
    } else {
        const int u = ((int)blockIdx.x - row_blocks) * (kThreads / 64) + (threadIdx.x >> 6), c = threadIdx.x & 63;
        if (RNAD_FINISH_ABLATE & 4) return;
        if (u < 2 * n_upper) {
            const int P = u / n_upper, pos = u % n_upper;
            unsigned long long *src = rep + (((int64_t)P * n_upper + pos) * kReplicas + c) * (A + 1);
            const int64_t r = (int64_t)P * S + upper_list[pos];
            long long x[A + 1];
#pragma unroll
            for (int a = 0; a <= A; ++a) {
                const unsigned long long v = src[a];
                if (v != 0ull) src[a] = 0ull;
                x[a] = wave_total_in_lane63((long long)v);
            }
            if (c == 63) {
                const float nf = P ? nf1 : nf0;
// ... 14 lines not shown
        if (atomicAdd(sub + g, 1) == members - 1) {
            sub[g] = 0;
            if (atomicAdd(ticket, 1) == groups - 1) {
                *ticket = 0;
                *overflow = 0;
#pragma unroll
                for (int u = 0; u < 4; ++u) losses_raw[u] = 0.0;
                last_s = 1;
            }
        }
    }
    if (norm_rep) {
        __syncthreads();
        if (last_s) {
            for (int i = threadIdx.x; i < kReplicas * T1; i += kThreads) alive_rep[i] = 0;
            if (threadIdx.x < 2 * kReplicas) norm_rep[threadIdx.x] = 0.0;
        }
    }
}

FixedPoint fixed_point_for(const rnad_learn_params_t &hp) {
    const int budget = 62 - kLaneBits;
    int e_l = 1;
    while (std::ldexp(1.0, e_l) <= 2.0 * std::fabs((double)hp.clip) && e_l < 30) ++e_l;
    const int e_v = 11;
    FixedPoint fx;
    fx.scale_l = std::ldexp(1.0, budget - e_l);
    fx.scale_v = std::ldexp(1.0, budget - e_v);
    fx.inv_l = std::ldexp(1.0, -(budget - e_l));
    fx.inv_v = std::ldexp(1.0, -(budget - e_v));
    fx.limit_l = (float)std::ldexp(1.0, e_l);
    fx.limit_v = (float)std::ldexp(1.0, e_v);
    fx.scale_l32 = (float)fx.scale_l;
    fx.scale_v32 = (float)fx.scale_v;
    fx.check_l = !(2.0 * std::fabs((double)hp.clip) < std::ldexp(1.0, e_l)) ? 1 : 0;
    return fx;
}

}

namespace {
struct Carver {
    uintptr_t at;
    template <class T>
    T *take(int64_t n) {
        T *first = (T *)at;
        at += (uintptr_t)n * sizeof(T);
        return first;
    }
};

struct Accumulators {
    unsigned long long *acc;
    unsigned long long *rep;
    double *losses_raw;
    int32_t *overflow;
    double *norm_rep;
    int32_t *alive_rep;
    int64_t bytes;
};
Accumulators carve_accumulators(void *base, const rnad_tree_t *tree, const Plan &p) {
    const int64_t A1 = tree->A + 1;
    Carver c{(uintptr_t)base};
    Accumulators a;
    a.acc = c.take<unsigned long long>(2 * tree->S * A1);
    a.rep = c.take<unsigned long long>((int64_t)kReplicas * 2 * std::max(p.cut->n_upper, 1) * A1);
    a.losses_raw = c.take<double>(4);
    a.overflow = c.take<int32_t>(2 + kTicketGroups);
    a.norm_rep = c.take<double>(2 * kReplicas);
    a.alive_rep = c.take<int32_t>(kReplicas * (kCompactSteps + 1));
    a.bytes = (int64_t)(c.at - (uintptr_t)base) + 8;
    return a;
}

int64_t alive_rows(int64_t B, const Plan &p, bool compact) { return compact ? p.max_items : (int64_t)blocks_for(B); }
int64_t alive_rows_max(int64_t B, const Plan &p) { return std::max<int64_t>(p.max_items, (int64_t)blocks_for(B)); }
struct Scratch {
    unsigned long long *decisions;
    int32_t *keys;
    int32_t *hist;
    int32_t *totals, *bucket_start;
    int32_t *alive_part;
    float *policy;
    int64_t bytes;
};
Scratch carve_scratch(void *ws, const rnad_tree_t *tree, int64_t B, const Plan &p) {
    const int64_t nb = p.cut->n_buckets;
    Carver c{(uintptr_t)ws};
    Scratch s;
    s.decisions = c.take<unsigned long long>(B);
    s.keys = c.take<int32_t>(B);
    s.hist = c.take<int32_t>(p.sort_blocks * nb);
    s.totals = c.take<int32_t>(nb);
    s.bucket_start = c.take<int32_t>(nb);
    s.alive_part = c.take<int32_t>(alive_rows_max(B, p) * (kMaxSteps + 1));
    const uintptr_t pad = (0 - c.at) & 15;
    c.at += pad;
    s.policy = c.take<float>(2 * tree->S * ((tree->A + 3) & ~3));
    s.bytes = (int64_t)(c.at - pad - (uintptr_t)ws) + 256;
    return s;
}

StageOut carve_stage(void *stage, int64_t B, int64_t S, int64_t *bytes = nullptr) {
    StageOut st;
    if (!stage && !bytes) return st;
    Carver c{(uintptr_t)stage};
    st.counts = c.take<unsigned long long>(2);
    st.root = c.take<uint32_t>(B);
    st.sorted = c.take<uint32_t>(B);
    st.mark0 = c.take<uint32_t>(S);
    st.mark1 = c.take<uint32_t>(S);
    if (bytes) *bytes = (int64_t)(c.at - (uintptr_t)stage);
    return st;
}

#define RNAD_DISPATCH_REL(p_, ...)        \
    if ((p_).rel_bytes == 1) {            \
        using REL = uint8_t;              \
        __VA_ARGS__;                      \
    } else {                              \
        using REL = uint16_t;             \
        __VA_ARGS__;                      \
    }

template <class... Params, class... Args>
int launch_lds(void (*kern)(Params...), dim3 grid, dim3 block, size_t lds, hipStream_t stream, Args &&...args) {
    if (lds > 48 * 1024) RNAD_HIP_OK(hipFuncSetAttribute((const void *)kern, hipFuncAttributeMaxDynamicSharedMemorySize, (int)lds));
    hipLaunchKernelGGL(kern, grid, block, lds, stream, std::forward<Args>(args)...);
    return 0;
}
}

extern "C" int rnad_bucket_plan(const rnad_tree_t *tree, int64_t B, int64_t *out) {
    RNAD_REQUIRE(tree && out, "rnad_bucket_plan: null argument");
    Plan p;
    if (!make_plan(tree, B, read_switches(), p)) {
        set_error("rnad_bucket_plan: this tree / batch cannot be bucketed (ids not DFS pre-order, no level whose subtree table fits "
                  "the LDS, or more than 2^%d lanes)", kLaneBits);
        return 3;
    }
    out[0] = p.cut->rows;
    out[1] = p.cut->n_buckets;
    out[2] = p.cut->n_upper;
    out[3] = p.cut->n_groups;
    out[4] = p.max_items;
    out[5] = carve_scratch(nullptr, tree, B, p).bytes;
    out[6] = carve_accumulators(nullptr, tree, p).bytes;
    out[7] = p.lds;
    out[8] = p.rel_bytes;
    out[9] = p.tile;
    out[10] = p.chunk;
    note_sized(tree, B, p);
    return 0;
}

extern "C" int rnad_bucket_map(const rnad_tree_t *tree, int64_t B, int32_t *bucket_of, int32_t *n_groups) {
    RNAD_REQUIRE(tree && bucket_of && n_groups, "rnad_bucket_map: null argument");
    Plan p;
    if (int rc = plan_for(tree, B, read_switches(), "rnad_bucket_map", false, p)) return rc;
    std::copy(p.cut->host_bucket_of.begin(), p.cut->host_bucket_of.end(), bucket_of);
    *n_groups = p.cut->n_groups;
    return 0;
}

extern "C" int rnad_bucket_shared_steps(const rnad_tree_t *tree, int64_t B, int32_t *n_shared) {
    RNAD_REQUIRE(tree && n_shared, "rnad_bucket_shared_steps: null argument");
    Plan p;
    if (int rc = plan_for(tree, B, read_switches(), "rnad_bucket_shared_steps", false, p)) return rc;
    std::vector<int32_t> path((size_t)p.cut->n_buckets);
    DeviceGuard guard(tree->device);
    RNAD_HIP_OK(hipMemcpy(path.data(), p.cut->bucket_path, path.size() * sizeof(int32_t), hipMemcpyDeviceToHost));
    for (int b = 0; b < p.cut->n_buckets; ++b)
        n_shared[b] = (path[(size_t)b] & (kSharedRoot - 1)) + ((b < p.cut->n_groups && (path[(size_t)b] & kSharedRoot)) ? 2 : 0);
    return 0;
}

namespace {
__global__ void k_step_params_set(rnad_step_params_t *dst, uint64_t seed, float alpha, float one_minus_alpha) {
    dst->seed = seed;
    dst->alpha = alpha;
    dst->one_minus_alpha = one_minus_alpha;
}

struct QueueEntries {
    rnad_step_params_t e[RNAD_STEP_QUEUE];
};
__global__ void k_step_queue_set(rnad_step_queue_t *q, int n, QueueEntries entries) {
    const int k = threadIdx.x;
    if (k < n) q->ahead[k] = entries.e[k];
    if (k == 0) {
        q->live = entries.e[0];
        q->cursor = 0;
        q->n = n;
    }
}
}

extern "C" int rnad_step_queue_set(rnad_step_queue_t *device_queue, int n, const rnad_step_params_t *entries, void *stream) {
    RNAD_REQUIRE(device_queue && entries && n >= 1 && n <= RNAD_STEP_QUEUE, "rnad_step_queue_set: 1..%d entries", RNAD_STEP_QUEUE);
    QueueEntries q{};
    for (int k = 0; k < n; ++k) q.e[k] = entries[k];
    hipLaunchKernelGGL(k_step_queue_set, dim3(1), dim3(64), 0, (hipStream_t)stream, device_queue, n, q);
    RNAD_HIP_OK(hipGetLastError());
    return 0;
}

extern "C" int rnad_step_params_set(rnad_step_params_t *device_params, uint64_t seed, float alpha, float one_minus_alpha, void *stream) {
    RNAD_REQUIRE(device_params, "rnad_step_params_set: null argument");
    hipLaunchKernelGGL(k_step_params_set, dim3(1), dim3(1), 0, (hipStream_t)stream, device_params, seed, alpha, one_minus_alpha);
    RNAD_HIP_OK(hipGetLastError());
    return 0;
}

extern "C" int64_t rnad_bucket_record_stride(int A) { return (4 * (int64_t)A + 3 + 3) & ~(int64_t)3; }
extern "C" int64_t rnad_bucket_fast_record_stride(int A) { return 4 + 4 * (int64_t)A; }
extern "C" int64_t rnad_bucket_policy_row_stride(int A) { return ((int64_t)A + 3) & ~(int64_t)3; }

extern "C" int rnad_bucket_records(const rnad_tree_t *tree, const float *logit_tab, const float *v_tab, const float *v_target_tab,
                                   const float *logit_reg_tab, const float *logit_reg_tab_, const rnad_learn_params_t *hp,
                                   const rnad_step_params_t *device_params, float *records, float *fast_records, float *policy_rows,
                                   const int32_t *rows, const int64_t *n_rows, void *stream) {
    RNAD_REQUIRE(tree && logit_tab && v_tab && v_target_tab && logit_reg_tab && logit_reg_tab_ && hp && records,
                 "rnad_bucket_records: null argument");
    RNAD_REQUIRE(((uintptr_t)records & 15) == 0 && ((uintptr_t)fast_records & 15) == 0 && ((uintptr_t)policy_rows & 15) == 0,
                 "rnad_bucket_records: records must be 16-byte aligned");
    RNAD_REQUIRE(hp->n_disc >= 1, "rnad_bucket_records: n_disc must be positive");
    RNAD_REQUIRE(!rows == !n_rows, "rnad_bucket_records: rows and n_rows go together");
    RNAD_DISPATCH_A(tree->A, hipLaunchKernelGGL((k_row_records<kA>), dim3(blocks_for(2 * tree->S)), dim3(kThreads), 0, (hipStream_t)stream,
                                                2 * tree->S, logit_tab, v_tab, v_target_tab, logit_reg_tab, logit_reg_tab_,
                                                (const uint8_t *)tree->mask_tab, *hp, device_params, records, fast_records, policy_rows, rows, n_rows));
    RNAD_HIP_OK(hipGetLastError());
    return 0;
}

namespace {
__global__ __launch_bounds__(kThreads) void k_clear_visited(int64_t rows, int64_t S, int32_t *__restrict__ visited) {
#pragma unroll
    for (int u = 0; u < 4; ++u) {
        const int64_t r = ((int64_t)blockIdx.x * 4 + u) * kThreads + threadIdx.x;
        if (r < rows) visited[r] = (r == 0 || r == S) ? 1 : 0;
    }
}

struct ActorTable {
    const float *table;
    int64_t stride;
    int is_policy;
};
struct LaneDraws {
    uint64_t seed;
    int64_t lane0;
    const rnad_step_params_t *device_params;
};
struct SortBuffers {
    void *scratch;
    int32_t *lane_ids, *items, *n_items;
    double *norm;
};
struct CompactTraj {
    void *states = nullptr;
    int32_t *alive = nullptr;
    unsigned long long *acts = nullptr;
    float *final_reward = nullptr;
    int32_t *visited = nullptr;
};
struct FusedLearn {
    const float *fast;
    const rnad_learn_params_t *hp;
    void *accumulators;
    bool distinct;
    const rnad_leaf_paths_t *leaf = nullptr;
};
struct RolloutRequest {
    int T_cap;
    int64_t B;
    ActorTable actor;
    LaneDraws draws;
    SortBuffers sort;
    hipStream_t stream;
    int phases = 3;
    const rnad_traj_t *dense = nullptr;
    CompactTraj out;
    const float *value_table = nullptr;
    int64_t value_stride = 1;
    int32_t *group_flags = nullptr, *staged_rows = nullptr, *stage_rows0 = nullptr;
    int64_t *n_staged = nullptr;
    void *stage = nullptr;
    const int32_t *play_rows = nullptr;
    const int64_t *n_play_rows = nullptr;
    bool visited_is_clear = false;
    KeysExpand expand;
    const FusedLearn *fused = nullptr;
};

int keys_expand_for(const char *who, const rnad_tree_t *tree, const int32_t *rep_of, int n_tables, float *const *tables,
                    const int32_t *floats_per_row, KeysExpand &ex) {
    ex.rep_of = rep_of;
    ex.rows = 2 * tree->S;
    ex.n = n_tables;
    for (int k = 0; k < n_tables; ++k) {
        RNAD_REQUIRE(tables[k] && floats_per_row[k] > 0 && floats_per_row[k] % 4 == 0 && ((uintptr_t)tables[k] & 15) == 0,
                     "%s: table %d must be 16-byte aligned with a row of a multiple of 4 floats", who, k);
        ex.tab[k] = reinterpret_cast<float4 *>(tables[k]);
        ex.quads[k] = floats_per_row[k] / 4;
        ex.max_quads = std::max(ex.max_quads, ex.quads[k]);
    }
    return 0;
}

enum class KeysWalk { Lds, Hybrid, Global };
struct KeysChoice {
    KeysWalk walk;
    size_t lds;
};
KeysChoice choose_keys_walk(const rnad_tree_t *tree, const Plan &p, const Switches &sw) {
    const BucketCut &cut = *p.cut;
    const bool walk_global = sw.keys_global.set && sw.keys_global.v != 0;
    const bool no_full_lds = sw.keys_lds.set && sw.keys_lds.v == 0;
    const bool no_hybrid = sw.keys_hybrid.set && sw.keys_hybrid.v == 0;
    const size_t full = keys_lds_bytes(cut.n_upper, cut.n_buckets, tree->A, tree->C);
    if (cut.upper_walk && full <= kKeysLds && !walk_global && !no_full_lds) return {KeysWalk::Lds, full};
    if (cut.upper_walk && cut.n_hot > 0 && cut.n_hot < cut.n_upper && !walk_global && !no_hybrid)
        return {KeysWalk::Hybrid,
                std::max(keys_hybrid_lds_bytes(cut.n_hot, cut.n_upper, tree->A, tree->C), (size_t)cut.n_buckets * sizeof(int32_t))};
    return {KeysWalk::Global, 0};
}

constexpr int kFusedChunkDefault = 512;
constexpr int kFusedLdsBudget = 26 * 1024;
struct FusedPlan {
    int chunk;
    int distinct_keys;
    size_t lds;
};
FusedPlan plan_fused(const rnad_tree_t *tree, const Plan &p, const Switches &sw, bool asked) {
    if (sw.fused_distinct.set) asked = sw.fused_distinct.v != 0;
    const int keys = asked ? p.cut->rows * (tree->A * tree->A * tree->C + 1) : 0;
    auto lds_with = [&](int chunk) { return (size_t)p.lds + ((size_t)keys + 2 + 2 * (size_t)chunk) * 4; };
    FusedPlan f{p.chunk, 0, (size_t)p.lds};
    if (keys == 0) return f;
    const int chunk = std::max(sw.fused_chunk.set ? std::max(64, sw.fused_chunk.v) : kFusedChunkDefault, p.chunk);
    if (lds_with(chunk) <= (size_t)kFusedLdsBudget) f.chunk = chunk;
    if ((f.chunk > p.chunk || sw.fused_chunk.set) && lds_with(f.chunk) <= (size_t)kFusedLdsBudget) {
        f.distinct_keys = keys;
        f.lds = lds_with(f.chunk);
    }
    return f;
}

struct RolloutCall {
    const rnad_tree_t *tree;
    const RolloutRequest &rq;
    const Switches &sw;
    const Plan &p;
    const BucketCut &cut;
    const Scratch s;
    const StageOut stage;
    const FusedPlan fplan;
    const int64_t B, S;
    const int n_steps;
    const hipStream_t stream;
    const uint64_t seed;
    const int64_t lane0;
    const rnad_step_params_t *device_params;
    const float *policy_tab;
    int64_t policy_stride;
    int vec4;

    template <int A, int TILE>
    int keys_lds(size_t lds, const KeysExpand &ex) const {
        return launch_lds(k_bucket_keys_lds<A, kPlayLds, TILE>, dim3(p.sort_blocks), dim3(kSortThreads), lds, stream, (const UpperWalk *)cut.upper_walk,
                          (const int32_t *)cut.upper_list, cut.n_upper, cut.n_buckets, tree->C, S, B, n_steps, policy_tab, policy_stride,
                          (int)cut.host_bucket_of[1], cut.n_groups, seed, device_params, lane0, s.keys, s.decisions, s.hist, rq.sort.norm, stage, ex);
    }
    template <int A, int TILE>
    int keys_hybrid(size_t lds) const {
        return launch_lds(k_bucket_keys_hybrid<A, kPlayLds, TILE>, dim3(p.sort_blocks), dim3(kSortThreads), lds, stream, (const UpperWalk *)cut.upper_walk,
                          (const int32_t *)cut.upper_list, (const int32_t *)cut.hot_list, (const int32_t *)cut.hot_of, cut.n_hot, cut.n_upper,
                          tree->trans, (const int32_t *)cut.bucket_of, tree->C, S, B, n_steps, policy_tab, policy_stride, vec4,
                          (int)cut.host_bucket_of[1], cut.n_groups, seed, device_params, lane0, s.keys, s.decisions, rq.sort.norm, stage,
                          cut.n_buckets, s.hist);
    }
    template <int A>
    void keys_global() const {
        hipLaunchKernelGGL((k_bucket_keys<A, kPlay>), dim3(blocks_for(B, kThreads * kPlay)), dim3(kThreads), 0, stream, tree->trans, tree->C, S, B, n_steps,
                           policy_tab, policy_stride, vec4, (const int32_t *)cut.bucket_of, cut.n_groups, seed, device_params, lane0, s.keys,
                           s.decisions, rq.sort.norm, stage);
    }
    template <int A>
    void rollout_dense() const {
        const rnad_traj_t &tr = *rq.dense;
        hipLaunchKernelGGL((k_bucket_rollout<A>), dim3(blocks_for(B)), dim3(kThreads), 0, stream, tree->trans, tree->C, S, B, rq.T_cap, policy_tab,
                           policy_stride, rq.value_table, rq.value_stride, (const uint8_t *)tree->mask_tab, seed, device_params, lane0,
                           (const int32_t *)rq.sort.lane_ids, (const unsigned long long *)s.decisions, tr.indices, tr.mask_bits, tr.policy, tr.actions,
                           tr.rewards, tr.values, s.alive_part);
    }
    template <int A, class REL>
    void rollout_items() const {
        hipLaunchKernelGGL((k_bucket_rollout_items<A, REL, kRolloutLanes>), dim3((unsigned)p.max_items), dim3(kThreads / kRolloutLanes), 0, stream,
                           tree->trans, tree->C, S, B, rq.T_cap, policy_tab, policy_stride, vec4, seed, device_params, lane0,
                           (const int32_t *)rq.sort.lane_ids, (const unsigned long long *)s.decisions, (const Item *)rq.sort.items,
                           (const int32_t *)rq.sort.n_items, (const int32_t *)cut.bucket_path, (const int32_t *)cut.bucket_lo,
                           (const int32_t *)cut.path_states, std::max(cut.max_path, 1), cut.n_groups, (REL *)rq.out.states, s.alive_part, rq.out.acts,
                           rq.out.final_reward, rq.out.visited);
    }
    template <int A, class REL>
    int play_learn(const Accumulators &acc, const FixedPoint &fx) const {
        auto kern = fplan.distinct_keys > 0 ? k_bucket_play_learn<A, REL, true> : k_bucket_play_learn<A, REL, false>;
        return launch_lds(kern, dim3((unsigned)p.max_items), dim3(kThreads), fplan.lds, stream, tree->trans, tree->C, S, B, rq.T_cap, policy_tab,
                          policy_stride, vec4, seed, device_params, lane0, (const int32_t *)rq.sort.lane_ids, (const unsigned long long *)s.decisions,
                          (const Item *)rq.sort.items, (const int32_t *)rq.sort.n_items, (const int32_t *)cut.bucket_path,
                          (const int32_t *)cut.bucket_lo, (const int32_t *)cut.path_states, std::max(cut.max_path, 1), cut.n_groups,
                          (REL *)rq.out.states, acc.alive_rep, acc.norm_rep, rq.out.acts, rq.out.final_reward, cut.rows, p.path_words,
                          std::max(cut.n_upper, 1), (const int32_t *)cut.bucket_of, rq.fused->fast, *rq.fused->hp, fx, acc.acc, acc.rep, acc.overflow,
                          p.lds / 8, fplan.distinct_keys, fplan.chunk);
    }
    template <int A, class REL>
    int play_count(const Accumulators &acc, const FixedPoint &fx, const LeafCount &lcount) const {
        const rnad_leaf_paths_t &lf = *rq.fused->leaf;
        hipLaunchKernelGGL((k_bucket_play_count<A, REL>), dim3((unsigned)p.max_items), dim3(kThreads), 0, stream, tree->trans, tree->C, S, B, rq.T_cap,
                           policy_tab, policy_stride, vec4, seed, device_params, lane0, (const int32_t *)rq.sort.lane_ids,
                           (const unsigned long long *)s.decisions, (const Item *)rq.sort.items, (const int32_t *)rq.sort.n_items,
                           (const int32_t *)cut.bucket_path, (const int32_t *)cut.bucket_lo, (const int32_t *)cut.path_states,
                           std::max(cut.max_path, 1), cut.n_groups, (REL *)rq.out.states, acc.alive_rep, acc.norm_rep, rq.out.acts,
                           rq.out.final_reward, lf.col_of, s.keys, lcount);
        return launch_lds(k_bucket_learn_c<A, REL, false, true>, dim3((unsigned)lf.max_items + 7), dim3(kThreads), (size_t)p.lds, stream, rq.T_cap,
                          lf.n_cols, S, cut.rows, p.path_words, cut.n_groups, std::max(cut.n_upper, 1), (const Item *)lf.items, lf.n_items,
                          (const int32_t *)cut.bucket_of, (const int32_t *)cut.bucket_lo, (const int32_t *)cut.bucket_path,
                          (const int32_t *)cut.path_states, std::max(cut.max_path, 1), (const REL *)lf.states, rq.fused->fast,
                          (const unsigned long long *)lf.acts, lf.final_reward, (const float *)nullptr, *rq.fused->hp, fx, acc.acc, acc.rep,
                          (double *)nullptr, acc.overflow, (const int32_t *)nullptr, 0, rq.T_cap + 1, (int32_t *)nullptr, (double *)nullptr,
                          (const int32_t *)s.keys, (const int32_t *)s.bucket_start, (const int32_t *)s.totals, lcount);
    }

    int sort_lanes() const {
        const int nb = cut.n_buckets;
        const KeysChoice keys = choose_keys_walk(tree, p, sw);
        bool copies = rq.expand.rep_of != nullptr;
        {
            ProfScope one(PROF_BUCKET_KEYS, stream);
            if (copies && keys.walk != KeysWalk::Lds) {
                float *tabs[4];
                int32_t widths[4];
                for (int k = 0; k < rq.expand.n; ++k) {
                    tabs[k] = reinterpret_cast<float *>(rq.expand.tab[k]);
                    widths[k] = 4 * rq.expand.quads[k];
                }
                if (int rc = rnad_rows_expand(rq.expand.rows, rq.expand.rep_of, rq.expand.n, tabs, widths, stream)) return rc;
                copies = false;
            }
            if (keys.walk == KeysWalk::Lds) {
                RNAD_DISPATCH_TILE(p, RNAD_DISPATCH_A(tree->A, if (int rc = keys_lds<kA, kTile>(keys.lds, copies ? rq.expand : KeysExpand{})) return rc));
            } else if (keys.walk == KeysWalk::Hybrid) {
                RNAD_DISPATCH_TILE(p, RNAD_DISPATCH_A(tree->A, if (int rc = keys_hybrid<kA, kTile>(keys.lds)) return rc));
            } else {
                RNAD_DISPATCH_A(tree->A, keys_global<kA>());
            }
        }
        ProfScope sort_passes(PROF_BUCKET_SORT, stream);
        if (keys.walk == KeysWalk::Global)
            RNAD_DISPATCH_TILE(p, hipLaunchKernelGGL(k_bucket_hist<kTile>, dim3(p.sort_blocks), dim3(kSortThreads), (size_t)nb * sizeof(int32_t), stream, B, nb,
                                                     (const int32_t *)s.keys, s.hist));
        const int scan_blocks = (nb + kScanCols - 1) / kScanCols;
        int copy_blocks = 0;
        if (copies) {
            copy_blocks = (int)std::min<int64_t>(1024, std::max<int64_t>(1, (rq.expand.rows * rq.expand.max_quads + 2 * kSortThreads - 1) / (2 * kSortThreads)));
            if (sw.expand_blocks.set) copy_blocks = std::max(1, sw.expand_blocks.v);
        }
        hipLaunchKernelGGL(k_bucket_scan, dim3(scan_blocks + copy_blocks), dim3(kSortThreads), 0, stream, p.sort_blocks, nb, s.hist, s.totals, scan_blocks,
                           copies ? rq.expand : KeysExpand{});
        int wave_rows = 16;
        while (wave_rows > 1 && ((2 + wave_rows) * (size_t)nb + 1) * sizeof(int32_t) > kKeysLds) wave_rows >>= 1;
        if (sw.scatter_rows.set) wave_rows = std::max(1, std::min(wave_rows, sw.scatter_rows.v));
        const size_t scatter_lds = ((2 + wave_rows) * (size_t)nb + 1) * sizeof(int32_t);
        RNAD_REQUIRE(scatter_lds <= 160 * 1024, "rnad_bucket_sort: %d buckets do not fit the sort's LDS", nb);
        RNAD_DISPATCH_TILE(p, if (int rc = launch_lds(k_bucket_scatter<kTile>, dim3(p.sort_blocks), dim3(kSortThreads), scatter_lds, stream, B, nb,
                                                      (const int32_t *)s.keys, (const int32_t *)s.hist, (const int32_t *)s.totals, fplan.chunk,
                                                      (Item *)rq.sort.items, rq.sort.n_items, rq.sort.lane_ids, wave_rows, S, cut.n_groups,
                                                      (const int32_t *)cut.bucket_lo, (const int32_t *)cut.bucket_span, (const int32_t *)cut.group_by_lo,
                                                      rq.staged_rows, rq.n_staged, rq.out.visited, (const uint32_t *)stage.root, stage.sorted,
                                                      (const uint32_t *)stage.mark0, stage.root ? rq.stage_rows0 : nullptr, stage.counts, seed,
                                                      device_params, s.bucket_start)) return rc);
        if (rq.group_flags)
            hipLaunchKernelGGL(k_group_flags, dim3(blocks_for(S)), dim3(kThreads), 0, stream, S, (const int32_t *)cut.bucket_of, cut.n_groups,
                               (const int32_t *)s.totals, rq.group_flags);
        return 0;
    }

    int play_lanes() const {
        const FusedLearn *fused = rq.fused;
        ProfScope one(fused ? PROF_BUCKET_LEARN : PROF_BUCKET_ROLLOUT, stream);
        if (rq.dense) {
            RNAD_DISPATCH_A(tree->A, rollout_dense<kA>());
            return 0;
        }
        RNAD_REQUIRE(rq.sort.items && rq.sort.n_items, "rnad_rollout_bucketed_compact: the work list of the sort is needed to play");
        if (!fused) {
            RNAD_DISPATCH_REL(p, RNAD_DISPATCH_A(tree->A, rollout_items<kA, REL>()));
            return 0;
        }
        const Accumulators acc = carve_accumulators(fused->accumulators, tree, p);
        const FixedPoint fx = fixed_point_for(*fused->hp);
        RNAD_REQUIRE(!fx.check_l, "rnad_rollout_learn_bucketed_compact: a NeuRD clip of 2^29 or more takes the two-launch path");
        RNAD_REQUIRE(!rq.out.visited, "rnad_rollout_learn_bucketed_compact: no visited flags (lazy rows evaluate their records after the rollout)");
        if (!fused->leaf) {
            RNAD_DISPATCH_REL(p, RNAD_DISPATCH_A(tree->A, if (int rc = play_learn<kA, REL>(acc, fx)) return rc));
            return 0;
        }
        const rnad_leaf_paths_t &lf = *fused->leaf;
        RNAD_REQUIRE(lf.n_cols >= 1 && lf.states && lf.acts && lf.final_reward && lf.items && lf.n_items && lf.col_of && lf.max_items >= 1,
                     "rnad_rollout_learn_bucketed_compact: incomplete rnad_leaf_paths_t");
        RNAD_REQUIRE(lf.rows == cut.rows && lf.T_cap == rq.T_cap && rq.T_cap == 2 * tree->max_depth,
                     "rnad_rollout_learn_bucketed_compact: the leaf paths were built for another cut / window (rows %d vs %d, T_cap %d vs %d, "
                     "2 * depth %d)", lf.rows, cut.rows, lf.T_cap, rq.T_cap, 2 * tree->max_depth);
        LeafCount lcount;
        if (lf.col_count && lf.bucket_col0 && lf.crowded_lanes > 0)
            lcount = LeafCount{lf.col_count, lf.bucket_col0, (const int32_t *)s.totals, lf.crowded_lanes};
        RNAD_DISPATCH_REL(p, RNAD_DISPATCH_A(tree->A, if (int rc = play_count<kA, REL>(acc, fx, lcount)) return rc));
        return 0;
    }
};

int rollout_bucketed_impl(const rnad_tree_t *tree, const Switches &sw, const RolloutRequest &rq) {
    Plan p;
    if (int rc = plan_for(tree, rq.B, sw, "rnad_rollout_bucketed", true, p)) return rc;
    const int64_t B = rq.B, S = tree->S;
    const hipStream_t stream = rq.stream;
    RolloutCall c{tree, rq, sw, p, *p.cut, carve_scratch(rq.sort.scratch, tree, B, p), carve_stage(rq.stage, B, S),
                  rq.fused ? plan_fused(tree, p, sw, rq.fused->distinct) : FusedPlan{p.chunk, 0, (size_t)p.lds}, B, S,
                  std::min(p.cut->max_path, rq.T_cap), stream, rq.draws.seed, rq.draws.lane0, rq.draws.device_params, rq.actor.table, rq.actor.stride, 0};
    ProfScope prof(PROF_ACT, stream);
    const bool sort_phase = (rq.phases & 1) != 0, play_phase = (rq.phases & 2) != 0;
    if (rq.out.visited && play_phase && !sort_phase && !rq.visited_is_clear)
        hipLaunchKernelGGL(k_clear_visited, dim3(blocks_for(2 * S, kThreads * 4)), dim3(kThreads), 0, stream, 2 * S, S, rq.out.visited);
    if (!rq.actor.is_policy) {
        const bool upper = rq.phases == 1, listed = rq.phases == 2;
        const int nu = upper ? p.cut->n_upper : 0;
        RNAD_REQUIRE(!listed || (rq.play_rows && rq.n_play_rows), "rnad_bucket_play: a logits table needs the list of rows that were evaluated for it");
        RNAD_DISPATCH_A(tree->A, hipLaunchKernelGGL((k_policy_rows<kA>), dim3(blocks_for(upper ? 2 * ((int64_t)nu + 1) : 2 * S)), dim3(kThreads), 0, stream,
                                                    2 * S, rq.actor.table, rq.actor.stride, (const uint8_t *)tree->mask_tab, c.s.policy,
                                                    listed ? rq.play_rows : nullptr, listed ? rq.n_play_rows : nullptr,
                                                    upper ? (const int32_t *)p.cut->upper_list : nullptr, nu, S));
        c.policy_tab = c.s.policy;
        c.policy_stride = (tree->A + 3) & ~3;
    }
    c.vec4 = (c.policy_stride % 4 == 0 && ((uintptr_t)c.policy_tab & 15) == 0) ? 1 : 0;
    if (sort_phase)
        if (int rc = c.sort_lanes()) return rc;
    RNAD_HIP_OK(hipGetLastError());
    if (!play_phase) return 0;
    if (int rc = c.play_lanes()) return rc;
    int32_t *alive = rq.dense ? rq.dense->alive : rq.out.alive;
    if (alive && !rq.fused)
        hipLaunchKernelGGL(k_bucket_alive, dim3(rq.T_cap + 1), dim3(kThreads), 0, stream, (int)alive_rows(B, p, !rq.dense), rq.T_cap + 1,
                           (const int32_t *)c.s.alive_part, alive, rq.sort.norm);
    RNAD_HIP_OK(hipGetLastError());
    return 0;
}

struct FinishOut {
    double *losses;
    float *dlogit_tab, *dv_tab;
    const int32_t *rows = nullptr;
    const int64_t *n_rows = nullptr;
    const rnad_row_groups_t *groups = nullptr;
};
struct Counts {
    int T1;
    int32_t *alive_out;
    double *norm_out;
};
int finish_impl(const rnad_tree_t *tree, const Plan &p, const Accumulators &acc, const double *norm, const rnad_learn_params_t *hp,
                const FinishOut &out, hipStream_t stream, const Counts *counts = nullptr) {
    const int64_t S = tree->S;
    const int nu = p.cut->n_upper;
    const rnad_row_groups_t *groups = out.groups;
    const FixedPoint fx = fixed_point_for(*hp);
    const int n_multi = groups ? groups->n_groups : 0;
    RNAD_REQUIRE(n_multi >= 0 && (n_multi == 0 || (groups->start && groups->order && out.rows)),
                 "rnad_bucket_finish: row groups come with their start / order arrays and with the list of the rows outside them");
    ProfScope fin(PROF_BUCKET_FINISH, stream);
    const unsigned row_blocks = std::min(blocks_for(2 * S, kThreads * kFinishRows), 512u), upper_blocks = nu > 0 ? blocks_for(2 * (int64_t)nu, kThreads / 64) : 0;
    const unsigned group_blocks = n_multi > 0 ? blocks_for(n_multi, kThreads / 64) : 0;
    RNAD_DISPATCH_A(tree->A, hipLaunchKernelGGL((k_bucket_finish<kA>), dim3(row_blocks + upper_blocks + group_blocks), dim3(kThreads), 0, stream, S,
                                                (int)row_blocks, out.rows, out.n_rows, nu, p.cut->n_groups, (const int32_t *)p.cut->upper_list,
                                                (const int32_t *)p.cut->bucket_of, acc.acc, acc.rep, norm, hp->w_v, hp->w_n, fx, acc.overflow,
                                                acc.losses_raw, out.losses, out.dlogit_tab, out.dv_tab, (int)upper_blocks, n_multi,
                                                n_multi ? groups->start : (const int32_t *)nullptr,
                                                n_multi ? groups->order : (const int32_t *)nullptr,
                                                n_multi ? groups->first : (const int32_t *)nullptr, (groups && out.rows) ? groups->rows_below_cut : 0,
                                                counts ? acc.alive_rep : (int32_t *)nullptr, counts ? acc.norm_rep : (double *)nullptr,
                                                counts ? counts->T1 : 0, counts ? counts->alive_out : (int32_t *)nullptr,
                                                counts ? counts->norm_out : (double *)nullptr));
    RNAD_HIP_OK(hipGetLastError());
    return 0;
}
}

extern "C" int rnad_bucket_sort(const rnad_tree_t *tree, int T_cap, int64_t B, const float *table, int64_t table_stride, int table_is_policy,
                                uint64_t seed, int64_t lane0, const rnad_step_params_t *device_params, void *scratch, int32_t *lane_ids,
                                int32_t *items, int32_t *n_items, double *norm, int32_t *group_flags, int32_t *staged_rows, int64_t *n_staged,
                                int32_t *visited, void *stage, int32_t *stage_rows0, void *stream) {
    RNAD_REQUIRE(tree && table && scratch && lane_ids && items && n_items, "rnad_bucket_sort: null argument");
    RNAD_REQUIRE(!stage_rows0 || stage, "rnad_bucket_sort: stage_rows0 goes with stage");
    RNAD_REQUIRE(!staged_rows == !n_staged, "rnad_bucket_sort: staged_rows and n_staged go together");
    RNAD_REQUIRE(T_cap >= 1 && T_cap <= kCompactSteps && B >= 1, "rnad_bucket_sort: 1 <= T_cap <= %d, got %d", kCompactSteps, T_cap);
    RNAD_REQUIRE(table_stride >= tree->A, "rnad_bucket_sort: bad table stride");
    RolloutRequest rq{T_cap, B, {table, table_stride, table_is_policy}, {seed, lane0, device_params}, {scratch, lane_ids, items, n_items, norm},
                      (hipStream_t)stream};
    rq.phases = 1;
    rq.out.visited = visited;
    rq.group_flags = group_flags;
    rq.staged_rows = staged_rows;
    rq.n_staged = n_staged;
    rq.stage = stage;
    rq.stage_rows0 = stage_rows0;
    return rollout_bucketed_impl(tree, read_switches(), rq);
}

extern "C" int64_t rnad_bucket_stage_bytes(const rnad_tree_t *tree, int64_t B) {
    if (!tree || B < 1) return -1;
    if (tree->S > ((int64_t)1 << kStageRootBits)) return -1;
    int64_t bytes = 0;
    carve_stage(nullptr, B, tree->S, &bytes);
    return bytes;
}

extern "C" int rnad_bucket_stage_rows(const rnad_tree_t *tree, int64_t B, int level, uint64_t seed, const rnad_step_params_t *device_params,
                                      void *stage, int32_t *rows, void *stream) {
    RNAD_REQUIRE(tree && stage && rows && (level == 0 || level == 1), "rnad_bucket_stage_rows: null argument / level must be 0 or 1");
    Plan p;
    if (int rc = plan_for(tree, B, read_switches(), "rnad_bucket_stage_rows", true, p)) return rc;
    const StageOut st = carve_stage(stage, B, tree->S);
    if (level == 0)
        hipLaunchKernelGGL(k_stage_rows<0>, dim3(blocks_for(tree->S, kSortThreads * kStagePer)), dim3(kSortThreads), 0, (hipStream_t)stream, tree->S, (const uint32_t *)st.mark0,
                           (const int32_t *)p.cut->anchor1, seed, device_params, rows, st.counts);
    else
        hipLaunchKernelGGL(k_stage_rows<1>, dim3(blocks_for(tree->S, kSortThreads * kStagePer)), dim3(kSortThreads), 0, (hipStream_t)stream, tree->S, (const uint32_t *)st.mark1,
                           (const int32_t *)p.cut->anchor1, seed, device_params, rows, st.counts + 1);
    RNAD_HIP_OK(hipGetLastError());
    return 0;
}

extern "C" int rnad_bucket_stage_walk(const rnad_tree_t *tree, int T_cap, int64_t B, const float *policy_rows, int64_t stride, uint64_t seed,
                                      int64_t lane0, const rnad_step_params_t *device_params, const void *scratch, const int32_t *lane_ids,
                                      void *stage, void *stream) {
    RNAD_REQUIRE(tree && policy_rows && scratch && stage && lane_ids, "rnad_bucket_stage_walk: null argument");
    RNAD_REQUIRE(stride >= tree->A && T_cap >= 1, "rnad_bucket_stage_walk: bad table stride / T_cap");
    Plan p;
    if (int rc = plan_for(tree, B, read_switches(), "rnad_bucket_stage_walk", true, p)) return rc;
    const StageOut st = carve_stage(stage, B, tree->S);
    const int vec4 = (stride % 4 == 0 && ((uintptr_t)policy_rows & 15) == 0) ? 1 : 0;
    RNAD_DISPATCH_A(tree->A, hipLaunchKernelGGL((k_stage_walk<kA>), dim3(blocks_for(B)), dim3(kThreads), 0, (hipStream_t)stream, tree->trans, tree->C,
                                                tree->S, B, T_cap, policy_rows, stride, vec4, (const uint32_t *)st.sorted, lane_ids, seed,
                                                device_params, lane0, st.mark1));
    RNAD_HIP_OK(hipGetLastError());
    return 0;
}

extern "C" int rnad_bucket_play(const rnad_tree_t *tree, int T_cap, int64_t B, const float *table, int64_t table_stride, int table_is_policy,
                                const int32_t *rows, const int64_t *n_rows, uint64_t seed, int64_t lane0,
                                const rnad_step_params_t *device_params, void *scratch, const int32_t *lane_ids, const int32_t *items,
                                const int32_t *n_items, double *norm, void *states, int32_t *alive, uint64_t *acts, float *final_reward,
                                int32_t *visited, int visited_is_clear, void *stream) {
    RNAD_REQUIRE(tree && table && scratch && lane_ids && items && n_items && states && acts && final_reward, "rnad_bucket_play: null argument");
    RNAD_REQUIRE(T_cap >= 1 && T_cap <= kCompactSteps && B >= 1, "rnad_bucket_play: 1 <= T_cap <= %d, got %d", kCompactSteps, T_cap);
    RNAD_REQUIRE(table_stride >= tree->A && (!rows == !n_rows), "rnad_bucket_play: bad table stride / row list");
    RolloutRequest rq{T_cap, B, {table, table_stride, table_is_policy}, {seed, lane0, device_params},
                      {scratch, const_cast<int32_t *>(lane_ids), const_cast<int32_t *>(items), const_cast<int32_t *>(n_items), norm}, (hipStream_t)stream};
    rq.phases = 2;
    rq.out = {states, alive, (unsigned long long *)acts, final_reward, visited};
    rq.play_rows = rows;
    rq.n_play_rows = n_rows;
    rq.visited_is_clear = visited_is_clear != 0;
    return rollout_bucketed_impl(tree, read_switches(), rq);
}

extern "C" int rnad_bucket_alive(const rnad_tree_t *tree, int T_cap, int64_t B, const void *scratch, int32_t *alive, double *norm, void *stream) {
    RNAD_REQUIRE(tree && scratch && alive, "rnad_bucket_alive: null argument");
    RNAD_REQUIRE(T_cap >= 1 && T_cap <= kMaxSteps && B >= 1, "rnad_bucket_alive: bad shape");
    Plan p;
    if (int rc = plan_for(tree, B, read_switches(), "rnad_bucket_alive", true, p)) return rc;
// ... 349 lines not shown
```

r-nad_amd/rnad_hip/__init__.py:

```python
import ctypes as C
import os
import threading
import weakref

import torch

_HERE = os.path.dirname(os.path.realpath(__file__))
SO_PATH = os.environ.get("RNAD_HIP_SO") or os.path.join(_HERE, "..", "csrc", "librnad_hip.so")

MAX_ACTIONS = 8
MAX_TRANSITIONS = 8


class RnadHipError(RuntimeError):
    pass


class Traj(C.Structure):

    _fields_ = [
        ("T_cap", C.c_int32), ("obs_half", C.c_int32), ("B", C.c_int64),
        ("indices", C.c_void_p), ("observations", C.c_void_p), ("mask_bits", C.c_void_p),
        ("policy", C.c_void_p), ("actions", C.c_void_p), ("rewards", C.c_void_p),
        ("values", C.c_void_p), ("alive", C.c_void_p),
# ... 667 lines not shown
    T, B, A = mu.shape
    onehot = actions.dtype == F32
    v_target = torch.empty((T, B), dtype=F32, device=mu.device)
    q = torch.empty((T, B, A), dtype=F32, device=mu.device)
    has_played = torch.empty((T, B), dtype=I32, device=mu.device) if want_has_played else None
    _check(lib().rnad_vtrace(T, C.c_int64(B), A, _dp(v, F32, "v"), _dp(valid, F32, "valid"), _dp(player_id, I32, "player_id", True),
                             _dp(mu, F32, "mu"), _dp(pi, F32, "pi"), _dp(logpi, F32, "logpi"),
                             _dp(actions, F32 if onehot else I32, "actions"), int(onehot), _dp(reward, F32, "reward"), int(player),
                             C.c_float(eta), C.c_float(lambda_), C.c_float(c), C.c_float(rho), C.c_float(gamma),
                             _dp(v_target, F32, "v_target"), _dp(has_played, I32, "has_played", True), _dp(q, F32, "q"), _stream()))
    return v_target, has_played, q


def mask_sum(mask):
    out = torch.empty((1,), dtype=F64, device=mask.device)
    _check(lib().rnad_mask_sum(C.c_int64(mask.numel()), _dp(mask, F32, "mask"), _dp(out, F64, "out"), _stream()))
    return out


def loss_v(v, v_target, mask, norm, weight, loss, dv, accumulate):
    _check(lib().rnad_loss_v(C.c_int64(v.numel()), _dp(v, F32, "v"), _dp(v_target, F32, "v_target"), _dp(mask, F32, "mask"),
                             _dp(norm, F64, "norm"), C.c_float(weight), _dp(loss, F64, "loss", True), _dp(dv, F32, "dv", True),
                             int(accumulate), _stream()))


def loss_nerd(logit, pi, q, mask, legal, norm, clip, threshold, weight, loss, dlogit, accumulate):
    A = logit.shape[-1]
    _check(lib().rnad_loss_nerd(C.c_int64(logit.numel() // A), A, _dp(logit, F32, "logit"), _dp(pi, F32, "pi"), _dp(q, F32, "q"),
                                _dp(mask, F32, "mask"), _dp(legal, F32, "legal"), _dp(norm, F64, "norm"), C.c_float(clip),
                                C.c_float(threshold), C.c_float(weight), _dp(loss, F64, "loss", True),
                                _dp(dlogit, F32, "dlogit", True), int(accumulate), _stream()))


def learn_fused(indices, mask_bits, actions, rewards, mu, logit, v, v_target_net, logit_reg, logit_reg_, norm, hp,
                want_aux=False):
    T, B, A = mu.shape
    dev = mu.device
    dlogit = torch.empty((T, B, A), dtype=F32, device=dev)
    dv = torch.empty((T, B), dtype=F32, device=dev)
    losses = torch.empty((2,), dtype=F64, device=dev)
    pi = torch.empty((T, B, A), dtype=F32, device=dev) if want_aux else None
    vt = torch.empty((2, T, B), dtype=F32, device=dev) if want_aux else None
    q = torch.empty((2, T, B, A), dtype=F32, device=dev) if want_aux else None
    _check(lib().rnad_learn_fused(T, C.c_int64(B), A, _dp(indices, I32, "indices"), _dp(mask_bits, U8, "mask_bits"),
                                  _dp(actions, I32, "actions"), _dp(rewards, F32, "rewards"), _dp(mu, F32, "mu"),
                                  _dp(logit, F32, "logit"), _dp(v, F32, "v"), _dp(v_target_net, F32, "v_target_net"),
                                  _dp(logit_reg, F32, "logit_reg"), _dp(logit_reg_, F32, "logit_reg_"), _dp(norm, F64, "norm"),
                                  C.byref(hp), _dp(losses, F64, "losses"), _dp(dlogit, F32, "dlogit"), _dp(dv, F32, "dv"),
                                  _dp(pi, F32, "pi", True), _dp(vt, F32, "vt", True), _dp(q, F32, "q", True), _stream()))
    return dlogit, dv, losses, pi, vt, q


def learn_fused_tabular(tree, indices, mask_bits, actions, rewards, mu, logit_tab, v_tab, v_target_tab, logit_reg_tab, logit_reg_tab_,
                        norm, hp):
    T, B, A = mu.shape
    dev = mu.device
    S = tree.S
    ws = torch.empty((int(lib().rnad_learn_tabular_workspace(tree.ptr, T, C.c_int64(B))) // 8 + 1,), dtype=F64, device=dev)
    dlogit = torch.empty((2 * S, A), dtype=F32, device=dev)
    dv = torch.empty((2 * S, 1), dtype=F32, device=dev)
    losses = torch.empty((2,), dtype=F64, device=dev)
    _check(lib().rnad_learn_fused_tabular(tree.ptr, T, C.c_int64(B), _dp(indices, I32, "indices"), _dp(mask_bits, U8, "mask_bits"),
                                          _dp(actions, I32, "actions"), _dp(rewards, F32, "rewards"), _dp(mu, F32, "mu"),
                                          _dp(logit_tab, F32, "logit_tab"), _dp(v_tab, F32, "v_tab"), _dp(v_target_tab, F32, "v_target_tab"),
                                          _dp(logit_reg_tab, F32, "logit_reg_tab"), _dp(logit_reg_tab_, F32, "logit_reg_tab_"),
                                          _dp(norm, F64, "norm"), C.byref(hp), _dp(losses, F64, "losses"), _dp(ws, F64, "workspace"),
                                          _dp(dlogit, F32, "dlogit_tab"), _dp(dv, F32, "dv_tab"), _stream()))
    return dlogit, dv, losses


def row_sums(tree, indices, dlogit, dv):
    T, B = indices.shape
    A, S, dev = tree.A, tree.S, indices.device
    ws = torch.empty((int(lib().rnad_row_sums_workspace(tree.ptr)) // 8 + 1,), dtype=F64, device=dev)
    out_l = torch.empty((2 * S, A), dtype=F32, device=dev)
    out_v = torch.empty((2 * S, 1), dtype=F32, device=dev)
    _check(lib().rnad_row_sums(tree.ptr, T, C.c_int64(B), _dp(indices, I32, "indices"), _dp(dlogit, F32, "dlogit"), _dp(dv, F32, "dv"),
                               _dp(ws, F64, "workspace"), _dp(out_l, F32, "dlogit_tab"), _dp(out_v, F32, "dv_tab"), _stream()))
    return out_l, out_v


class TabularMLP(torch.autograd.Function):

    @staticmethod
    def forward(ctx, table, indices, tree, A, packed, *weights):
        T, B = indices.shape
        logit_tab, v_tab = mlp_forward(packed, weights[0].shape[0], table, A)
        rows = (indices.long() + (torch.arange(T, device=indices.device) & 1).view(T, 1) * tree.S).reshape(-1)
        ctx.A, ctx.tree = A, tree
        ctx.save_for_backward(table, indices, packed, *weights)
        return logit_tab.index_select(0, rows), v_tab.index_select(0, rows)

    @staticmethod
    def backward(ctx, dlogits, dvalue):
        table, indices, packed, *weights = ctx.saved_tensors
        T, B = indices.shape
        dl_tab, dv_tab = row_sums(ctx.tree, indices, dlogits.contiguous().view(T, B, ctx.A), dvalue.contiguous().view(T, B))
        grads = mlp_backward(packed, weights, table, ctx.A, dl_tab, dv_tab)
        return (None, None, None, None, None, *grads)


def learn_fused_gather(tree, indices, mask_bits, actions, rewards, mu, logit_tab, v_tab, v_target_tab, logit_reg_tab, logit_reg_tab_,
                       norm, hp):
    T, B, A = mu.shape
    dev = mu.device
    dlogit = torch.empty((T, B, A), dtype=F32, device=dev)
    dv = torch.empty((T, B), dtype=F32, device=dev)
    losses = torch.empty((2,), dtype=F64, device=dev)
    ws = torch.empty((int(lib().rnad_learn_gather_workspace(tree.ptr)) // 4,), dtype=F32, device=dev)
    _check(lib().rnad_learn_fused_gather(tree.ptr, T, C.c_int64(B), _dp(indices, I32, "indices"), _dp(mask_bits, U8, "mask_bits"),
                                         _dp(actions, I32, "actions"), _dp(rewards, F32, "rewards"), _dp(mu, F32, "mu"),
                                         _dp(logit_tab, F32, "logit_tab"), _dp(v_tab, F32, "v_tab"), _dp(v_target_tab, F32, "v_target_tab"),
                                         _dp(logit_reg_tab, F32, "logit_reg_tab"), _dp(logit_reg_tab_, F32, "logit_reg_tab_"),
                                         _dp(norm, F64, "norm"), C.byref(hp), _dp(losses, F64, "losses"), _dp(ws, F32, "workspace"),
                                         _dp(dlogit, F32, "dlogit"), _dp(dv, F32, "dv"), _stream()))
    return dlogit, dv, losses


class BucketPlan:

    def __init__(self, tree, B, out):
        self.B = B
        (self.rows, self.n_buckets, self.n_upper, self.n_groups, self.max_items, self.scratch_bytes, self.acc_bytes, self.lds,
         self.rel_bytes, self.sort_tile, self.chunk) = (int(x) for x in out)
        dev = tree.device
        self.scratch = torch.empty((self.scratch_bytes // 4 + 1,), dtype=I32, device=dev)
        self.accumulators = torch.zeros((self.acc_bytes // 8 + 1,), dtype=torch.int64, device=dev)


_owner = threading.local()


class WorkspaceToken:

    __slots__ = ("__weakref__",)


class workspace_owner:

    def __init__(self, token):
        self.token, self.prev = token, None

    def __enter__(self):
        self.prev = getattr(_owner, "token", None)
        _owner.token = self.token
        return self

    def __exit__(self, *exc):
        _owner.token = self.prev
        return False


def plan_knobs():
    return tuple(os.environ.get(k) for k in ("RNAD_BUCKET_ROWS", "RNAD_BUCKET_CHUNK", "RNAD_SORT_TILE"))


def bucket_plan(tree, B):
    destroy_deferred()
    token = getattr(_owner, "token", None)
    if token is None:
        cache = tree.__dict__.setdefault("_bucket_plans", {})
    else:
        cache = tree.__dict__.setdefault("_owner_plans", weakref.WeakKeyDictionary()).setdefault(token, {})
    key = (B,) + plan_knobs()
    if key not in cache:
        out = (C.c_int64 * 11)()
        rc = lib().rnad_bucket_plan(tree.ptr, B, out)
        cache[key] = BucketPlan(tree, B, list(out)) if rc == 0 else None
    return cache[key]


def bucket_map(tree, B):
    out = torch.empty((tree.S,), dtype=I32)
    n_groups = C.c_int32()
    _check(lib().rnad_bucket_map(tree.ptr, B, C.c_void_p(out.data_ptr()), C.byref(n_groups)))
    return out, n_groups.value


def bucket_shared_steps(tree, B):
    plan = bucket_plan(tree, B)
    out = torch.empty((plan.n_buckets,), dtype=I32)
    _check(lib().rnad_bucket_shared_steps(tree.ptr, B, C.c_void_p(out.data_ptr())))
    return out


def stored_state_slots(tree, buckets, T):
    n = int(buckets.n_items.item())
    items = buckets.items[:n].cpu().long()
    shared = bucket_shared_steps(tree, buckets.plan.B).long()[items[:, 2]]
    return int((items[:, 1] * (T + 1 - shared).clamp(min=0)).sum().item())


class Buckets:

    def __init__(self, plan, device):
        self.plan = plan
        self.lane_ids = torch.empty((plan.B,), dtype=I32, device=device)
        self.items = torch.empty((plan.max_items, 4), dtype=I32, device=device)
        self.n_items = torch.empty((1,), dtype=I32, device=device)
        self.norm = torch.empty((2,), dtype=F64, device=device)
        self.alive_pending = None


def rollout_bucketed(tree, traj, table, value_table=None, seed=0, lane0=0, table_is_policy=False, column=0, step_params=None):
    plan = bucket_plan(tree, traj.B)
    if plan is None:
        raise RnadHipError(lib().rnad_last_error().decode())
    assert table.shape[0] == 2 * tree.S and table.shape[1] >= column + tree.A
    buckets = Buckets(plan, traj.device)
    base = _dp(table, F32, "table")
    _check(lib().rnad_rollout_bucketed(tree.ptr, C.byref(traj.c), C.c_void_p(base.value + 4 * column), table.shape[1], int(table_is_policy),
                                       _dp(value_table, F32, "value_table", True), 1, seed, lane0,
                                       _dp(step_params, torch.int64, "step_params", True), _dp(plan.scratch, I32, "scratch"),
                                       _dp(buckets.lane_ids, I32, "lane_ids"), _dp(buckets.items, I32, "items"),
                                       _dp(buckets.n_items, I32, "n_items"), _dp(buckets.norm, F64, "norm"), _stream()))
    return buckets


COMPACT_MAX_STEPS = 21
BUCKET_REPLICAS = 64
BUCKET_MAX_LANES = 1 << 22


def rollout_bucketed_compact(tree, traj, table, seed=0, lane0=0, step_params=None, table_is_policy=True, column=None, visited=None,
                             defer_alive=False):
    assert traj.compact and traj.T_cap <= COMPACT_MAX_STEPS
    plan = bucket_plan(tree, traj.B)
    if plan is None:
        raise RnadHipError(lib().rnad_last_error().decode())
    given = table
    pol_rows = getattr(table, "_policy_rows", None)
    if table_is_policy and column is None and pol_rows is not None:
        table, column = pol_rows, 0
    if column is None:
        column = policy_column(tree.A) if table_is_policy else 0
    assert table.shape[0] == 2 * tree.S and table.shape[1] >= column + tree.A
    assert visited is None or visited.numel() == 2 * tree.S
    buckets = Buckets(plan, traj.device)
    _complete_pending(tree, plan)
    base = _dp(table, F32, "table")
    pending = getattr(given, "_expand", None) if table_is_policy else None
    if pending is not None:
        dedup, tabs = pending
        tabs = [t for t in tabs if t is not None]
        ptrs = (C.c_void_p * len(tabs))(*[_dp(t, F32, "table").value for t in tabs])
        widths = (C.c_int32 * len(tabs))(*[int(t.shape[1]) for t in tabs])
        _check(lib().rnad_rollout_bucketed_compact_expand(
            tree.ptr, traj.T_cap, traj.B, C.c_void_p(base.value + 4 * column), table.shape[1], int(table_is_policy), seed, lane0,
            _dp(step_params, torch.int64, "step_params", True), _dp(plan.scratch, I32, "scratch"), _dp(buckets.lane_ids, I32, "lane_ids"),
            _dp(buckets.items, I32, "items"), _dp(buckets.n_items, I32, "n_items"), _dp(buckets.norm, F64, "norm"),
            _dp(traj.states, traj.states.dtype, "states"), None if defer_alive else _dp(traj.alive, I32, "alive"),
            _dp(traj.acts, torch.int64, "acts"), _dp(traj.final_reward, F32, "final_reward"), _dp(visited, I32, "visited", True),
            _dp(dedup.rep_of, I32, "rep_of"), len(tabs), ptrs, widths, _stream()))
        given._expand = None
    else:
        _rollout_compact_plain(tree, traj, table, base, column, table_is_policy, seed, lane0, step_params, plan, buckets, defer_alive, visited)
    buckets.alive_pending = traj if defer_alive else None
    plan._pending = buckets if defer_alive else None
    traj._owner = (tree, buckets)
    traj.invalidate()
    return buckets


PLAY_LEARN_FINISH, PLAY_LEARN_DISTINCT = 1, 2


class _LeafPathsC(C.Structure):

    _fields_ = [("n_cols", C.c_int64), ("rows", C.c_int32), ("T_cap", C.c_int32), ("states", C.c_void_p), ("acts", C.c_void_p),
                ("final_reward", C.c_void_p), ("items", C.c_void_p), ("n_items", C.c_void_p), ("max_items", C.c_int32),
                ("col_of", C.c_void_p), ("col_count", C.c_void_p), ("bucket_col0", C.c_void_p), ("crowded_lanes", C.c_int32)]


LEAF_CROWDED_SHARE = 4.0


class LeafPaths:

    def __init__(self, tree, plan_B, index, chance, value):
        dev = tree.device
        S, Cc, A = tree.S, tree.C, tree.A
        T_cap = 2 * tree.max_depth
        assert T_cap <= COMPACT_MAX_STEPS
        bucket_of, n_groups = bucket_map(tree, plan_B)
        cols = leaf_columns(index.to(dev), chance.to(dev), value.to(dev), bucket_of.to(dev), tree.max_depth)
        n = cols["n_cols"]
        self.n_cols, self.T_cap, self.plan_B = n, T_cap, plan_B
        indices = cols["indices"]
        self.acts, self.final_reward, self.col_of = cols["acts"], cols["final_reward"], cols["col_of"]
        items = leaf_items(cols["bucket"], max(64, min(256, int(os.environ.get("RNAD_LEAF_CHUNK", "256")))))
        self.max_items = len(items)
        self.items = torch.tensor(items, dtype=I32, device=dev).contiguous()
        self.n_items = torch.tensor([len(items)], dtype=I32, device=dev)
        bad = torch.zeros((1,), dtype=I32, device=dev)
        rows, rel = C.c_int32(), C.c_int32()
        states8 = torch.empty((T_cap + 1, n), dtype=torch.int16, device=dev)
        _check(lib().rnad_leaf_paths_pack(tree.ptr, C.c_int64(plan_B), T_cap + 1, C.c_int64(n), _dp(indices, I32, "indices"),
                                          _dp(self.items, I32, "items"), _dp(self.n_items, I32, "n_items"), self.max_items,
                                          C.c_void_p(states8.data_ptr()), _dp(bad, I32, "mismatch"), C.byref(rows), C.byref(rel), _stream()))
        if int(bad.item()) != 0:
            raise RnadHipError("leaf paths: a column does not lie in its work item's bucket")
        self.rows, self.rel_bytes = rows.value, rel.value
        self.states = states8
        self.indices = indices
        plan = bucket_plan(tree, plan_B)
        self.col_count = torch.zeros((n,), dtype=I32, device=dev)
        self.bucket_col0 = torch.searchsorted(cols["bucket"].long().contiguous(), torch.arange(plan.n_buckets + 1, device=dev)).to(I32).contiguous()
# ... 592 lines not shown
```

Before: 72.93 billion env-steps/s.

## Size fused play-learn chunks to resident block slots with balanced item splits

For the non-distinct fused play+learn path, the chunk size is now chosen from the device's resident block capacity (CUs times occupancy) so the number of work items roughly fits one wave of resident blocks. Buckets are split into equal-sized items instead of fixed-chunk pieces, the grid is trimmed to the expected item count, and each block loops over multiple passes of its item with split prologue/pass/epilogue helpers. This aims to cut tail effects and per-item overhead of many small blocks, at the cost of larger per-block work and dependence on the occupancy query.

```diff
diff --git a/include/rnad_hip.h b/include/rnad_hip.h
--- a/include/rnad_hip.h
+++ b/include/rnad_hip.h
@@ -175,6 +175,7 @@
 int rnad_step_queue_set(rnad_step_queue_t *device_queue, int n, const rnad_step_params_t *entries, void *stream);
 int rnad_bucket_plan(const rnad_tree_t *tree, int64_t B, int64_t *out);
 int rnad_bucket_map(const rnad_tree_t *tree, int64_t B, int32_t *bucket_of, int32_t *n_groups);
+int rnad_fused_chunk(int64_t B, int n_buckets, int slots);
 int rnad_bucket_shared_steps(const rnad_tree_t *tree, int64_t B, int32_t *n_shared);
 int rnad_rollout_bucketed(const rnad_tree_t *tree, const rnad_traj_t *traj, const float *table, int64_t table_stride,
                           int table_is_policy, const float *value_table, int64_t value_stride, uint64_t seed, int64_t lane0,
diff --git a/r-nad_amd/csrc/bucket.hip b/r-nad_amd/csrc/bucket.hip
--- a/r-nad_amd/csrc/bucket.hip
+++ b/r-nad_amd/csrc/bucket.hip
@@ -4,6 +4,7 @@
 
 #include <algorithm>
 #include <cstdlib>
+#include <mutex>
 #include <utility>
 
 using namespace rnad;
@@ -70,6 +71,7 @@
     Switch scatter_rows;
     Switch fused_distinct;
     Switch fused_chunk;
+    Switch fused_slots;
 };
 Switches read_switches() {
     auto read = [](const char *name) {
@@ -78,7 +80,19 @@
     };
     return {read("RNAD_BUCKET_ROWS"), read("RNAD_BUCKET_CHUNK"), read("RNAD_SORT_TILE"), read("RNAD_KEYS_STAGE_BYTES"),
             read("RNAD_KEYS_GLOBAL"), read("RNAD_KEYS_LDS"), read("RNAD_KEYS_HYBRID"), read("RNAD_EXPAND_BLOCKS"),
-            read("RNAD_SCATTER_ROWS"), read("RNAD_FUSED_DISTINCT"), read("RNAD_FUSED_CHUNK")};
+            read("RNAD_SCATTER_ROWS"), read("RNAD_FUSED_DISTINCT"), read("RNAD_FUSED_CHUNK"), read("RNAD_FUSED_SLOTS")};
+}
+
+constexpr int kFusedPassesMax = 4;
+int fused_passes(int64_t B, int n_buckets, int64_t slots) {
+    for (int r = 1; r < kFusedPassesMax; ++r)
+        if ((int64_t)n_buckets + B / ((int64_t)kChunkDefault * r) <= slots) return r;
+    return kFusedPassesMax;
+}
+int fused_lane_chunk(int64_t B, int n_buckets, int64_t slots, const Switches &sw, int plan_chunk) {
+    if (sw.bucket_chunk.set || sw.fused_chunk.set) return plan_chunk;
+    if (sw.fused_slots.set) slots = std::max(1, sw.fused_slots.v);
+    return kChunkDefault * fused_passes(B, n_buckets, slots);
 }
 
 struct Plan {
@@ -931,9 +945,16 @@
 
 constexpr int kItemsInline = 16;
 
+__device__ __forceinline__ Item cut_item(int32_t start, int32_t n, int32_t ni, int32_t j, int chunk, int bucket, bool equal) {
+    if (!equal) return Item{start + j * chunk, min(chunk, n - j * chunk), bucket, ni == 1 ? 1 : 0};
+    const int32_t q = n / ni, r = n - q * ni;
+    return Item{start + j * q + min(j, r), q + (j < r ? 1 : 0), bucket, ni == 1 ? 1 : 0};
+}
+
 __device__ __forceinline__ void items_phase(int n_buckets, int chunk, const int32_t *__restrict__ totals, int32_t *__restrict__ start_s,
                                             int32_t *__restrict__ first_s, bool write_items, Item *__restrict__ items,
-                                            int32_t *__restrict__ n_items, int32_t *__restrict__ bucket_start_out = nullptr) {
+                                            int32_t *__restrict__ n_items, int32_t *__restrict__ bucket_start_out = nullptr,
+                                            bool equal = false) {
     __shared__ int32_t wave_l[16], wave_i[16];
     __shared__ int32_t total_s, most;
     if (threadIdx.x == 0) most = 0;
@@ -988,7 +1009,7 @@
     if (most <= kItemsInline) {
         for (int i = threadIdx.x; i < n_buckets; i += kSortThreads) {
             const int32_t n = totals[i], first = first_s[i], ni = first_s[i + 1] - first, start = start_s[i];
-            for (int32_t j = 0; j < ni; ++j) items[first + j] = Item{start + j * chunk, min(chunk, n - j * chunk), i, ni == 1 ? 1 : 0};
+            for (int32_t j = 0; j < ni; ++j) items[first + j] = cut_item(start, n, ni, j, chunk, i, equal);
         }
         return;
     }
@@ -1000,7 +1021,7 @@
             else hi = mid;
         }
         const int32_t n = totals[lo], j = k - first_s[lo], start = start_s[lo];
-        items[k] = Item{start + j * chunk, min(chunk, n - j * chunk), lo, n <= chunk ? 1 : 0};
+        items[k] = cut_item(start, n, (n + chunk - 1) / chunk, j, chunk, lo, equal);
     }
 }
 
@@ -1069,7 +1090,8 @@
                                                                  const uint32_t *__restrict__ stage_root, uint32_t *__restrict__ stage_sorted,
                                                                  const uint32_t *__restrict__ stage_mark0, int32_t *__restrict__ stage_rows0,
                                                                  unsigned long long *__restrict__ stage_count0, uint64_t seed,
-                                                                 const rnad_step_params_t *__restrict__ sp, int32_t *__restrict__ bucket_start_out) {
+                                                                 const rnad_step_params_t *__restrict__ sp, int32_t *__restrict__ bucket_start_out,
+                                                                 int equal_items) {
     extern __shared__ int32_t cnt[];
     const int wave = threadIdx.x >> 6, lane = threadIdx.x & 63;
     const int64_t base = (int64_t)blockIdx.x * TILE + (int64_t)wave * (TILE / 16);
@@ -1131,7 +1153,7 @@
     }
     const int32_t *row = hist + (int64_t)blockIdx.x * n_buckets;
     const int32_t row_first = (int)threadIdx.x < n_buckets ? row[threadIdx.x] : 0;
-    items_phase(n_buckets, chunk, totals, cnt, cnt + n_buckets, blockIdx.x == 0, items, n_items, bucket_start_out);
+    items_phase(n_buckets, chunk, totals, cnt, cnt + n_buckets, blockIdx.x == 0, items, n_items, bucket_start_out, equal_items != 0);
     __syncthreads();
     if ((int)threadIdx.x < n_buckets) cnt[threadIdx.x] += row_first;
     for (int i = threadIdx.x + kSortThreads; i < n_buckets; i += kSortThreads) cnt[i] += row[i];
@@ -1282,55 +1304,62 @@
            lc.bucket_col0[bucket + 1] - lc.bucket_col0[bucket] <= kLeafHist;
 }
 
-template <int A, typename REL, int L, bool DISTINCT = false, bool HIST = false>
-__device__ __forceinline__ void rollout_items_body(const Trans *__restrict__ trans, int C, int64_t S, int64_t B, int T_cap,
-                                                                   const float *__restrict__ policy_tab, int64_t tab_stride, int vec4,
-                                                                   uint64_t seed, const rnad_step_params_t *__restrict__ sp, int64_t lane0,
-                                                                   const int32_t *__restrict__ lane_ids,
-                                                                   const unsigned long long *__restrict__ decisions,
-                                                                   const Item *__restrict__ items, const int32_t *__restrict__ n_items,
-                                                                   const int32_t *__restrict__ bucket_path, const int32_t *__restrict__ bucket_lo,
-                                                                   const int32_t *__restrict__ path_states, int path_stride, int n_groups,
-                                                                   REL *__restrict__ states, int32_t *__restrict__ alive_part,
-                                                                   unsigned long long *__restrict__ acts_out,
-                                                                   float *__restrict__ reward_out, int32_t *__restrict__ visited,
-                                                                   double *__restrict__ norm_rep = nullptr, Hand *hand = nullptr,
-                                                                   const Distinct distinct = Distinct{},
-                                                                   const int32_t *__restrict__ col_of = nullptr,
-                                                                   int32_t *__restrict__ leaf_col = nullptr, const LeafCount lc = LeafCount{}) {
-    constexpr int NT = kThreads / L, NW = NT / 64;
-    __shared__ int32_t leaf_hist[HIST ? kLeafHist : 1];
-    static_assert(NT >= 64 && NT > kCompactSteps, "a wave at least, and a thread per alive counter");
-    __shared__ int32_t cnt[NW][kMaxSteps + 1];
-    int32_t *my_alive = alive_part + (norm_rep ? (int64_t)(blockIdx.x & (kReplicas - 1)) : (int64_t)blockIdx.x) * (T_cap + 1);
-    const int my_item = xcd_item(*n_items);
-    if (my_item < 0) {
-        if (!norm_rep && (int)threadIdx.x <= T_cap) my_alive[threadIdx.x] = 0;
-        return;
-    }
-    const Item item = items[my_item];
-    if (sp) seed = sp->seed;
+struct PlayItem {
+    Item item;
+    uint64_t seed;
+    bool shared;
+    int n_shared, lo;
+    const int32_t *my_path;
+    bool count_here = false;
+    int32_t col0 = 0, n_bins = 0;
+};
+using AliveRow = int32_t[kMaxSteps + 1];
+
+template <bool HIST, int NT>
+__device__ __forceinline__ PlayItem rollout_prologue(const Item &item, int T_cap, uint64_t seed, const rnad_step_params_t *__restrict__ sp,
+                                                     const int32_t *__restrict__ bucket_path, const int32_t *__restrict__ bucket_lo,
+                                                     const int32_t *__restrict__ path_states, int path_stride, int n_groups, AliveRow *cnt,
+                                                     int32_t *leaf_hist, const LeafCount &lc) {
+    PlayItem pi;
+    pi.item = item;
+    pi.seed = sp ? sp->seed : seed;
     const int wave = threadIdx.x >> 6;
     const int path_word = bucket_path[item.bucket];
-    const bool shared = item.bucket < n_groups && (path_word & kSharedRoot) != 0;
-    const int n_shared = (path_word & (kSharedRoot - 1)) + (shared ? 2 : 0);
-    const int lo = bucket_lo[item.bucket];
-    const int32_t *my_path = path_states + (int64_t)item.bucket * path_stride;
-    const uint32_t B32 = (uint32_t)B;
+    pi.shared = item.bucket < n_groups && (path_word & kSharedRoot) != 0;
+    pi.n_shared = (path_word & (kSharedRoot - 1)) + (pi.shared ? 2 : 0);
+    pi.lo = bucket_lo[item.bucket];
+    pi.my_path = path_states + (int64_t)item.bucket * path_stride;
     if ((threadIdx.x & 63) == 0)
         for (int t = 0; t <= T_cap; ++t) cnt[wave][t] = 0;
-    bool count_here = false;
-    int32_t col0 = 0, n_bins = 0;
     if constexpr (HIST) {
-        count_here = leaf_crowded(lc, item.bucket);
-        if (count_here) {
-            col0 = lc.bucket_col0[item.bucket];
-            n_bins = lc.bucket_col0[item.bucket + 1] - col0;
-            for (int i = threadIdx.x; i < n_bins; i += NT) leaf_hist[i] = 0;
+        pi.count_here = leaf_crowded(lc, item.bucket);
+        if (pi.count_here) {
+            pi.col0 = lc.bucket_col0[item.bucket];
+            pi.n_bins = lc.bucket_col0[item.bucket + 1] - pi.col0;
+            for (int i = threadIdx.x; i < pi.n_bins; i += NT) leaf_hist[i] = 0;
             __syncthreads();
         }
     }
-    for (int base = 0; base < item.count; base += kThreads) {
+    return pi;
+}
+
+template <int A, typename REL, int L, bool DISTINCT, bool HIST>
+__device__ __forceinline__ void rollout_pass(const PlayItem &pi, int base, const unsigned tid, const Trans *__restrict__ trans, int C, int64_t S, int64_t B, int T_cap,
+                                             const float *__restrict__ policy_tab, int64_t tab_stride, int vec4, int64_t lane0,
+                                             const int32_t *__restrict__ lane_ids, const unsigned long long *__restrict__ decisions,
+                                             REL *__restrict__ states, unsigned long long *__restrict__ acts_out,
+                                             float *__restrict__ reward_out, int32_t *__restrict__ visited, AliveRow *cnt, int32_t *leaf_hist,
+                                             Hand *hand, const Distinct &distinct, const int32_t *__restrict__ col_of,
+                                             int32_t *__restrict__ leaf_col) {
+    constexpr int NT = kThreads / L;
+    const Item &item = pi.item;
+    const uint64_t seed = pi.seed;
+    const bool shared = pi.shared, count_here = pi.count_here;
+    const int n_shared = pi.n_shared, lo = pi.lo, wave = tid >> 6;
+    const int32_t *my_path = pi.my_path;
+    const int32_t col0 = pi.col0;
+    const uint32_t B32 = (uint32_t)B;
+    {
         bool active[L];
         uint32_t j[L];
         int32_t lane_local[L];
@@ -1338,7 +1367,7 @@
         unsigned long long packed[L];
 #pragma unroll
         for (int l = 0; l < L; ++l) {
-            const int k = base + l * NT + (int)threadIdx.x;
+            const int k = base + l * NT + (int)tid;
             active[l] = k < item.count;
             j[l] = (uint32_t)(item.begin + k);
             lane_local[l] = active[l] ? lane_ids[j[l]] : 0;
@@ -1373,12 +1402,12 @@
 #pragma unroll
             for (int l = 0; l < L; ++l) live_now += (int32_t)__popcll(__ballot(active[l]));
             for (int t = 0; t < n_pre; t += 2) {
-                if ((threadIdx.x & 63) == 0) {
+                if ((tid & 63) == 0) {
                     cnt[wave][t] += live_now;
                     cnt[wave][t + 1] += live_now;
                 }
                 const int bits0 = (int)(packed[0] >> (6 * t)) & 63, bits1 = (int)(packed[0] >> (6 * (t + 1))) & 63;
-                if (visited && threadIdx.x == 0 && base == 0) {
+                if (visited && tid == 0 && base == 0) {
                     const int at = my_path[t];
                     visited[at] = visited[S + at] = 1;
                 }
@@ -1395,7 +1424,7 @@
             int32_t live = 0;
 #pragma unroll
             for (int l = 0; l < L; ++l) live += (int32_t)__popcll(__ballot(state[l] != 0));
-            if ((threadIdx.x & 63) == 0) {
+            if ((tid & 63) == 0) {
                 cnt[wave][t] += live;
                 if (two) cnt[wave][t + 1] += live;
             }
@@ -1477,7 +1506,7 @@
             }
             live += (int32_t)__popcll(__ballot(state[l] != 0));
         }
-        if ((threadIdx.x & 63) == 0) cnt[wave][T_cap] += live;
+        if ((tid & 63) == 0) cnt[wave][T_cap] += live;
         if (DISTINCT) {
 #pragma unroll
             for (int l = 0; l < L; ++l) {
@@ -1493,12 +1522,18 @@
         }
         if (hand) *hand = Hand{acts[0], relq, reward_final[0], active[0] ? (int)rel_of<REL>(state[0], lo) : 0};
     }
+}
+
+template <bool HIST, int NT>
+__device__ __forceinline__ void rollout_epilogue(const PlayItem &pi, int T_cap, int32_t *__restrict__ my_alive, double *__restrict__ norm_rep,
+                                                 AliveRow *cnt, const int32_t *leaf_hist, const LeafCount &lc) {
+    constexpr int NW = NT / 64;
     __syncthreads();
     if constexpr (HIST) {
-        if (count_here) {
-            for (int i = threadIdx.x; i < n_bins; i += NT) {
+        if (pi.count_here) {
+            for (int i = threadIdx.x; i < pi.n_bins; i += NT) {
                 const int32_t n = leaf_hist[i];
-                if (n != 0) atomicAdd(lc.col_count + col0 + i, n);
+                if (n != 0) atomicAdd(lc.col_count + pi.col0 + i, n);
             }
         }
     }
@@ -1518,6 +1553,40 @@
             if (n != 0) atomicAdd(norm_rep + 2 * (blockIdx.x & (kReplicas - 1)) + threadIdx.x, (double)n);
         }
     }
+}
+
+template <int A, typename REL, int L, bool DISTINCT = false, bool HIST = false>
+__device__ __forceinline__ void rollout_items_body(const Trans *__restrict__ trans, int C, int64_t S, int64_t B, int T_cap,
+                                                                   const float *__restrict__ policy_tab, int64_t tab_stride, int vec4,
+                                                                   uint64_t seed, const rnad_step_params_t *__restrict__ sp, int64_t lane0,
+                                                                   const int32_t *__restrict__ lane_ids,
+                                                                   const unsigned long long *__restrict__ decisions,
+                                                                   const Item *__restrict__ items, const int32_t *__restrict__ n_items,
+                                                                   const int32_t *__restrict__ bucket_path, const int32_t *__restrict__ bucket_lo,
+                                                                   const int32_t *__restrict__ path_states, int path_stride, int n_groups,
+                                                                   REL *__restrict__ states, int32_t *__restrict__ alive_part,
+                                                                   unsigned long long *__restrict__ acts_out,
+                                                                   float *__restrict__ reward_out, int32_t *__restrict__ visited,
+                                                                   double *__restrict__ norm_rep = nullptr, Hand *hand = nullptr,
+                                                                   const Distinct distinct = Distinct{},
+                                                                   const int32_t *__restrict__ col_of = nullptr,
+                                                                   int32_t *__restrict__ leaf_col = nullptr, const LeafCount lc = LeafCount{}) {
+    constexpr int NT = kThreads / L, NW = NT / 64;
+    __shared__ int32_t leaf_hist[HIST ? kLeafHist : 1];
+    static_assert(NT >= 64 && NT > kCompactSteps, "a wave at least, and a thread per alive counter");
+    __shared__ AliveRow cnt[NW];
+    int32_t *my_alive = alive_part + (norm_rep ? (int64_t)(blockIdx.x & (kReplicas - 1)) : (int64_t)blockIdx.x) * (T_cap + 1);
+    const int my_item = xcd_item(*n_items);
+    if (my_item < 0) {
+        if (!norm_rep && (int)threadIdx.x <= T_cap) my_alive[threadIdx.x] = 0;
+        return;
+    }
+    const PlayItem pi = rollout_prologue<HIST, NT>(items[my_item], T_cap, seed, sp, bucket_path, bucket_lo, path_states, path_stride, n_groups, cnt,
+                                                   leaf_hist, lc);
+    for (int base = 0; base < pi.item.count; base += kThreads)
+        rollout_pass<A, REL, L, DISTINCT, HIST>(pi, base, threadIdx.x, trans, C, S, B, T_cap, policy_tab, tab_stride, vec4, lane0, lane_ids, decisions, states,
+                                                acts_out, reward_out, visited, cnt, leaf_hist, hand, distinct, col_of, leaf_col);
+    rollout_epilogue<HIST, NT>(pi, T_cap, my_alive, norm_rep, cnt, leaf_hist, lc);
 }
 
 template <int A, typename REL, int L>
@@ -2083,6 +2152,182 @@
 #else
 #define RNAD_LEARN_ATTR
 #endif
+struct LearnItem {
+    Item item;
+    int s_b, n_path, n_shared;
+    int t_low;
+    const int32_t *my_path;
+};
+template <int A>
+__device__ __forceinline__ LearnItem learn_prologue(const Item &item, int T, int sub_rows, int path_words, int n_groups,
+                                                    const int32_t *__restrict__ bucket_lo, const int32_t *__restrict__ bucket_path,
+                                                    const int32_t *__restrict__ path_states, int path_stride, unsigned long long *tab,
+                                                    int32_t *path_state) {
+    constexpr int PS = (A + 1) | 1, TS = kTabStride<A>;
+    LearnItem li;
+    li.item = item;
+    li.s_b = bucket_lo[item.bucket];
+    const int path_word = bucket_path[item.bucket];
+    li.n_path = path_word & (kSharedRoot - 1);
+    li.n_shared = li.n_path + ((item.bucket < n_groups && (path_word & kSharedRoot)) ? 2 : 0);
+    li.my_path = path_states + (int64_t)item.bucket * path_stride;
+    li.t_low = min(T, li.n_shared);
+    const int n_tab = item.bucket < n_groups ? path_words + 2 * sub_rows * TS : li.n_path * kPathSlots * PS;
+    for (int i = threadIdx.x; i < n_tab; i += kThreads) tab[i] = 0ull;
+    if ((int)threadIdx.x < li.n_shared) path_state[threadIdx.x] = li.my_path[threadIdx.x];
+    __syncthreads();
+    return li;
+}
+
+template <int A, typename REL, bool LOSSES, bool DISTINCT, bool WEIGHTED>
+__device__ __forceinline__ void learn_pass(const LearnItem &li, int base, const unsigned tid, int n_work, int T, int64_t B, int64_t S, int sub_rows, int path_words,
+                                           const REL *__restrict__ states, const float *__restrict__ rec_,
+                                           const unsigned long long *__restrict__ acts_, const float *__restrict__ reward_,
+                                           const float *__restrict__ logit_, const rnad_learn_params_t &hp, const FixedPoint &fx,
+                                           unsigned long long *tab, const int32_t *w_lds, const Hand *hand, const Distinct &distinct,
+                                           double (&part)[4], bool &ovf) {
+    constexpr int PS = (A + 1) | 1, TS = kTabStride<A>, FS = kFastStride<A>, RS = kRowStride<A>;
+    constexpr bool by_trajectory = DISTINCT || WEIGHTED;
+    const int kPathWords = path_words;
+    const Item &item = li.item;
+    const int s_b = li.s_b, t_low = li.t_low, n_shared = li.n_shared;
+    const int32_t *my_path = li.my_path;
+    const VtHp vh{-hp.eta, hp.lambda_, hp.c, hp.rho, hp.gamma};
+    const uint32_t B32 = (uint32_t)B, S32 = (uint32_t)S;
+    {
+        bool active = base + (int)tid < n_work;
+        const uint32_t j = DISTINCT ? (uint32_t)(active ? distinct.column[base + tid] : item.begin) : (uint32_t)(item.begin + base) + tid;
+        long long weight = DISTINCT ? (long long)(active ? distinct.count[distinct.key[base + tid]] : 0) : 1ll;
+        if (WEIGHTED) {
+            const int32_t w = active ? w_lds[tid] : 0;
+            weight = w;
+            active = w != 0;
+            if (__ballot(active) == 0ull) return;
+        }
+        Carry cy[2];
+        const bool handed = hand != nullptr && item.count <= kThreads;
+        const unsigned long long acts = handed ? hand->acts : active ? acts_[j] : 0ull;
+        const float reward_final = handed ? hand->reward : active ? reward_[j] : 0.0f;
+        const int last_pair = (T - 1) >> 1;
+        auto state_at = [&](int t) {
+            if (handed) {
+                if (t == T) return hand->final_rel;
+                const int k = last_pair - (t >> 1);
+                if (k < kHandPairs) return (int)((hand->relq >> (16 * k)) & 0xffffull);
+            }
+            return (int)*at_bytes<REL>(states, ((uint32_t)t * B32 + j) * (uint32_t)sizeof(REL));
+        };
+        bool after_zero = active && (T < n_shared ? false : state_at(T) == 0);
+        if (t_low < T && !(RNAD_ABLATE & 8)) {
+            struct Slot {
+                float rec[FS];
+                float lg[A];
+            };
+            auto fetch = [&](int t, int rel, Slot &o) {
+                if (rel == 0) return;
+                const uint32_t row = (uint32_t)(t & 1) * S32 + (uint32_t)(s_b + rel - 1);
+                const float4 *rp = at_bytes<float4>(rec_, row * (uint32_t)(FS * sizeof(float)));
+#pragma unroll
+                for (int u = 0; u < FS / 4; ++u) {
+                    const float4 r4 = rp[u];
+                    o.rec[4 * u] = r4.x; o.rec[4 * u + 1] = r4.y; o.rec[4 * u + 2] = r4.z; o.rec[4 * u + 3] = r4.w;
+                }
+                if (LOSSES) {
+                    const float *lp = at_bytes<float>(logit_, row * (uint32_t)(RS * sizeof(float)));
+#pragma unroll
+                    for (int a = 0; a < A; ++a) o.lg[a] = lp[a];
+                }
+            };
+            int r_next = active ? state_at(T - 1) : 0;
+            int r_next2 = (active && T - 2 >= t_low) ? state_at(T - 2) : 0;
+            Slot nxt;
+            fetch(T - 1, r_next, nxt);
+            for (int t = T - 1; t >= t_low; --t) {
+                const int rel = r_next;
+                const Slot cur = nxt;
+                r_next = r_next2;
+                if (t - 1 >= t_low) fetch(t - 1, r_next, nxt);
+                r_next2 = (active && t - 2 >= t_low) ? state_at(t - 2) : 0;
+                const bool valid = rel != 0;
+                long long q[A + 1];
+#pragma unroll
+                for (int a = 0; a <= A; ++a) q[a] = 0;
+                if (valid) {
+                    const int act = (int)(acts >> (3 * t)) & 7;
+                    if (t & 1)
+                        fast_slot<A, LOSSES, 1>(cur.rec, cur.lg, act, after_zero ? reward_final : 0.0f, vh, hp, fx, cy, q, part, ovf);
+                    else
+                        fast_slot<A, LOSSES, 0>(cur.rec, cur.lg, act, 0.0f, vh, hp, fx, cy, q, part, ovf);
+#if RNAD_ABLATE & 1
+                    ovf |= (q[0] ^ q[1] ^ q[A]) == 0x123456789ll;
+#else
+                    unsigned long long *dst = tab + kPathWords + ((t & 1) * sub_rows + (rel - 1)) * TS;
+#pragma unroll
+                    for (int a = 0; a <= A; ++a) atomicAdd(dst + a, (unsigned long long)(by_trajectory ? q[a] * weight : q[a]));
+#endif
+                } else {
+                    cy[0] = Carry{};
+                    cy[1] = Carry{};
+                }
+                after_zero = !valid;
+            }
+        }
+        if (active && t_low > 0 && !(RNAD_ABLATE & 16)) {
+            auto row_of = [&](int t, int state) { return (uint32_t)(t & 1) * S32 + (uint32_t)state; };
+            auto load_rec = [&](uint32_t row, float (&f)[FS], float (&lg)[A]) {
+#if RNAD_PHASE2_VMEM
+                asm volatile("" : "+v"(row));
+                const float4 *r4p = at_bytes<float4>(rec_, row * (uint32_t)(FS * sizeof(float)));
+#pragma unroll
+                for (int u = 0; u < FS / 4; ++u) {
+                    const float4 r4 = r4p[u];
+                    f[4 * u] = r4.x; f[4 * u + 1] = r4.y; f[4 * u + 2] = r4.z; f[4 * u + 3] = r4.w;
+                }
+#else
+                const float *rp = at_bytes<float>(rec_, row * (uint32_t)(FS * sizeof(float)));
+#pragma unroll
+                for (int u = 0; u < FS; ++u) f[u] = rp[u];
+#endif
+                if (LOSSES) {
+                    const float *lp = at_bytes<float>(logit_, row * (uint32_t)(RS * sizeof(float)));
+#pragma unroll
+                    for (int a = 0; a < A; ++a) lg[a] = lp[a];
+                }
+            };
+            auto slot = [&](int t, const float (&f)[FS], const float (&lg)[A]) {
+                const int act = (int)(acts >> (3 * t)) & 7;
+                long long q[A + 1];
+                if (t & 1)
+                    fast_slot<A, LOSSES, 1>(f, lg, act, after_zero ? reward_final : 0.0f, vh, hp, fx, cy, q, part, ovf);
+                else
+                    fast_slot<A, LOSSES, 0>(f, lg, act, 0.0f, vh, hp, fx, cy, q, part, ovf);
+                after_zero = false;
+#if RNAD_ABLATE & 1
+                ovf |= (q[0] ^ q[1] ^ q[A]) == 0x123456789ll;
+#else
+                unsigned long long *dst = tab + (t * kPathSlots + (tid & (kPathSlots - 1))) * PS;
+#pragma unroll
+                for (int a = 0; a <= A; ++a) atomicAdd(dst + a, (unsigned long long)(by_trajectory ? q[a] * weight : q[a]));
+#endif
+            };
+            float fa[FS], la[A], fb[FS], lb[A];
+            int t = t_low - 1;
+            load_rec(row_of(t, __builtin_amdgcn_readfirstlane(my_path[t])), fa, la);
+            if (!(t & 1)) {
+                slot(t, fa, la);
+                --t;
+                if (t >= 0) load_rec(row_of(t, __builtin_amdgcn_readfirstlane(my_path[t])), fa, la);
+            }
+            for (; t >= 1; t -= 2) {
+                load_rec(row_of(t - 1, __builtin_amdgcn_readfirstlane(my_path[t - 1])), fb, lb);
+                slot(t, fa, la);
+                if (t >= 2) load_rec(row_of(t - 2, __builtin_amdgcn_readfirstlane(my_path[t - 2])), fa, la);
+                slot(t - 1, fb, lb);
+            }
+        }
+    }
+}
+
 template <int A, typename REL, bool LOSSES, bool DISTINCT = false, bool WEIGHTED = false>
 __device__ __forceinline__ void learn_c_body(int T, int64_t B, int64_t S, int sub_rows, int path_words, int n_groups, int up_stride,
                                                              const Item *__restrict__ items, const int32_t *__restrict__ n_items,
@@ -2100,29 +2345,16 @@
                                                              const int32_t *__restrict__ lane_start = nullptr,
                                                              const int32_t *__restrict__ lane_total = nullptr, const LeafCount lc = LeafCount{}) {
     extern __shared__ unsigned long long tab[];
-    constexpr int PS = (A + 1) | 1, TS = kTabStride<A>, FS = kFastStride<A>, RS = kRowStride<A>;
-    const int kPathWords = path_words;
     __shared__ int32_t path_state[kMaxPath];
     __shared__ double loss_part[kThreads / 64][4];
     if (alive_part && (int)blockIdx.x < T1) alive_column(alive_blocks, T1, blockIdx.x, alive_part, alive, norm_out);
     const int my_item = xcd_item(*n_items);
     if (my_item < 0) return;
-    const Item item = items[my_item];
-    const int s_b = bucket_lo[item.bucket];
-    const int path_word = bucket_path[item.bucket];
-    const int n_path = path_word & (kSharedRoot - 1);
-    const int n_shared = n_path + ((item.bucket < n_groups && (path_word & kSharedRoot)) ? 2 : 0);
-    const int32_t *my_path = path_states + (uint32_t)item.bucket * (uint32_t)path_stride;
-    const int n_tab = item.bucket < n_groups ? kPathWords + 2 * sub_rows * TS : n_path * kPathSlots * PS;
-    for (int i = threadIdx.x; i < n_tab; i += kThreads) tab[i] = 0ull;
-    if ((int)threadIdx.x < n_shared) path_state[threadIdx.x] = my_path[threadIdx.x];
-    __syncthreads();
-    const VtHp vh{-hp.eta, hp.lambda_, hp.c, hp.rho, hp.gamma};
-    const uint32_t B32 = (uint32_t)B, S32 = (uint32_t)S;
-    const int t_low = min(T, n_shared);
+    const LearnItem li = learn_prologue<A>(items[my_item], T, sub_rows, path_words, n_groups, bucket_lo, bucket_path, path_states, path_stride, tab,
+                                           path_state);
+    const Item &item = li.item;
     double part[4] = {0.0, 0.0, 0.0, 0.0};
     bool ovf = false;
-    constexpr bool by_trajectory = DISTINCT || WEIGHTED;
     __shared__ int32_t w_lds[WEIGHTED ? kThreads : 1];
     if (WEIGHTED) {
         if (leaf_crowded(lc, item.bucket)) {
@@ -2144,139 +2376,10 @@
         __syncthreads();
     }
     const int n_work = DISTINCT ? *distinct.n : item.count;
-    for (int base = 0; base < n_work; base += kThreads) {
-        bool active = base + (int)threadIdx.x < n_work;
-        const uint32_t j = DISTINCT ? (uint32_t)(active ? distinct.column[base + threadIdx.x] : item.begin) : (uint32_t)(item.begin + base) + threadIdx.x;
-        long long weight = DISTINCT ? (long long)(active ? distinct.count[distinct.key[base + threadIdx.x]] : 0) : 1ll;
-        if (WEIGHTED) {
-            const int32_t w = active ? w_lds[threadIdx.x] : 0;
-            weight = w;
-            active = w != 0;
-            if (__ballot(active) == 0ull) continue;
-        }
-        Carry cy[2];
-        const bool handed = hand != nullptr && item.count <= kThreads;
-        const unsigned long long acts = handed ? hand->acts : active ? acts_[j] : 0ull;
-        const float reward_final = handed ? hand->reward : active ? reward_[j] : 0.0f;
-        const int last_pair = (T - 1) >> 1;
-        auto state_at = [&](int t) {
-            if (handed) {
-                if (t == T) return hand->final_rel;
-                const int k = last_pair - (t >> 1);
-                if (k < kHandPairs) return (int)((hand->relq >> (16 * k)) & 0xffffull);
-            }
-            return (int)*at_bytes<REL>(states, ((uint32_t)t * B32 + j) * (uint32_t)sizeof(REL));
-        };
-        bool after_zero = active && (T < n_shared ? false : state_at(T) == 0);
-        if (t_low < T && !(RNAD_ABLATE & 8)) {
-            struct Slot {
-                float rec[FS];
-                float lg[A];
-            };
-            auto fetch = [&](int t, int rel, Slot &o) {
-                if (rel == 0) return;
-                const uint32_t row = (uint32_t)(t & 1) * S32 + (uint32_t)(s_b + rel - 1);
-                const float4 *rp = at_bytes<float4>(rec_, row * (uint32_t)(FS * sizeof(float)));
-#pragma unroll
-                for (int u = 0; u < FS / 4; ++u) {
-                    const float4 r4 = rp[u];
-                    o.rec[4 * u] = r4.x; o.rec[4 * u + 1] = r4.y; o.rec[4 * u + 2] = r4.z; o.rec[4 * u + 3] = r4.w;
-                }
-                if (LOSSES) {
-                    const float *lp = at_bytes<float>(logit_, row * (uint32_t)(RS * sizeof(float)));
-#pragma unroll
-                    for (int a = 0; a < A; ++a) o.lg[a] = lp[a];
-                }
-            };
-            int r_next = active ? state_at(T - 1) : 0;
-            int r_next2 = (active && T - 2 >= t_low) ? state_at(T - 2) : 0;
-            Slot nxt;
-            fetch(T - 1, r_next, nxt);
-            for (int t = T - 1; t >= t_low; --t) {
-                const int rel = r_next;
-                const Slot cur = nxt;
-                r_next = r_next2;
-                if (t - 1 >= t_low) fetch(t - 1, r_next, nxt);
-                r_next2 = (active && t - 2 >= t_low) ? state_at(t - 2) : 0;
-                const bool valid = rel != 0;
-                long long q[A + 1];
-#pragma unroll
-                for (int a = 0; a <= A; ++a) q[a] = 0;
-                if (valid) {
-                    const int act = (int)(acts >> (3 * t)) & 7;
-                    if (t & 1)
-                        fast_slot<A, LOSSES, 1>(cur.rec, cur.lg, act, after_zero ? reward_final : 0.0f, vh, hp, fx, cy, q, part, ovf);
-                    else
-                        fast_slot<A, LOSSES, 0>(cur.rec, cur.lg, act, 0.0f, vh, hp, fx, cy, q, part, ovf);
-#if RNAD_ABLATE & 1
-                    ovf |= (q[0] ^ q[1] ^ q[A]) == 0x123456789ll;
-#else
-                    unsigned long long *dst = tab + kPathWords + ((t & 1) * sub_rows + (rel - 1)) * TS;
-#pragma unroll
-                    for (int a = 0; a <= A; ++a) atomicAdd(dst + a, (unsigned long long)(by_trajectory ? q[a] * weight : q[a]));
-#endif
-                } else {
-                    cy[0] = Carry{};
-                    cy[1] = Carry{};
-                }
-                after_zero = !valid;
-            }
-        }
-        if (active && t_low > 0 && !(RNAD_ABLATE & 16)) {
-            auto row_of = [&](int t, int state) { return (uint32_t)(t & 1) * S32 + (uint32_t)state; };
-            auto load_rec = [&](uint32_t row, float (&f)[FS], float (&lg)[A]) {
-#if RNAD_PHASE2_VMEM
-                asm volatile("" : "+v"(row));
-                const float4 *r4p = at_bytes<float4>(rec_, row * (uint32_t)(FS * sizeof(float)));
-#pragma unroll
-                for (int u = 0; u < FS / 4; ++u) {
-                    const float4 r4 = r4p[u];
-                    f[4 * u] = r4.x; f[4 * u + 1] = r4.y; f[4 * u + 2] = r4.z; f[4 * u + 3] = r4.w;
-                }
-#else
-                const float *rp = at_bytes<float>(rec_, row * (uint32_t)(FS * sizeof(float)));
-#pragma unroll
-                for (int u = 0; u < FS; ++u) f[u] = rp[u];
-#endif
-                if (LOSSES) {
-                    const float *lp = at_bytes<float>(logit_, row * (uint32_t)(RS * sizeof(float)));
-#pragma unroll
-                    for (int a = 0; a < A; ++a) lg[a] = lp[a];
-                }
-            };
-            auto slot = [&](int t, const float (&f)[FS], const float (&lg)[A]) {
-                const int act = (int)(acts >> (3 * t)) & 7;
-                long long q[A + 1];
-                if (t & 1)
-                    fast_slot<A, LOSSES, 1>(f, lg, act, after_zero ? reward_final : 0.0f, vh, hp, fx, cy, q, part, ovf);
-                else
-                    fast_slot<A, LOSSES, 0>(f, lg, act, 0.0f, vh, hp, fx, cy, q, part, ovf);
-                after_zero = false;
-#if RNAD_ABLATE & 1
-                ovf |= (q[0] ^ q[1] ^ q[A]) == 0x123456789ll;
-#else
-                unsigned long long *dst = tab + (t * kPathSlots + (threadIdx.x & (kPathSlots - 1))) * PS;
-#pragma unroll
-                for (int a = 0; a <= A; ++a) atomicAdd(dst + a, (unsigned long long)(by_trajectory ? q[a] * weight : q[a]));
-#endif
-            };
-            float fa[FS], la[A], fb[FS], lb[A];
-            int t = t_low - 1;
-            load_rec(row_of(t, __builtin_amdgcn_readfirstlane(my_path[t])), fa, la);
-            if (!(t & 1)) {
-                slot(t, fa, la);
-                --t;
-                if (t >= 0) load_rec(row_of(t, __builtin_amdgcn_readfirstlane(my_path[t])), fa, la);
-            }
-            for (; t >= 1; t -= 2) {
-                load_rec(row_of(t - 1, __builtin_amdgcn_readfirstlane(my_path[t - 1])), fb, lb);
-                slot(t, fa, la);
-                if (t >= 2) load_rec(row_of(t - 2, __builtin_amdgcn_readfirstlane(my_path[t - 2])), fa, la);
-                slot(t - 1, fb, lb);
-            }
-        }
-    }
-    learn_epilogue<A>(tab, path_state, item, s_b, n_path, n_shared, kPathWords, sub_rows, S, n_groups, up_stride, bucket_of, part, ovf,
+    for (int base = 0; base < n_work; base += kThreads)
+        learn_pass<A, REL, LOSSES, DISTINCT, WEIGHTED>(li, base, threadIdx.x, n_work, T, B, S, sub_rows, path_words, states, rec_, acts_, reward_, logit_, hp, fx, tab,
+                                                       w_lds, hand, distinct, part, ovf);
+    learn_epilogue<A>(tab, path_state, item, li.s_b, li.n_path, li.n_shared, path_words, sub_rows, S, n_groups, up_stride, bucket_of, part, ovf,
                       loss_part, acc, rep, losses_raw, overflow);
 }
 
@@ -2351,12 +2454,50 @@
         __syncthreads();
     }
     Hand hand{0ull, 0ull, 0.0f, 0};
-    rollout_items_body<A, REL, 1, DISTINCT>(trans, C, S, B, T_cap, policy_tab, tab_stride, vec4, seed, sp, lane0, lane_ids, decisions, items, n_items,
-                                  bucket_path, bucket_lo, path_states, path_stride, n_groups, states, alive_rep, acts, reward, nullptr, norm_rep,
-                                  RNAD_HANDOVER ? &hand : nullptr, dd);
-    learn_c_body<A, REL, false, DISTINCT>(T_cap, B, S, sub_rows, path_words, n_groups, up_stride, items, n_items, bucket_of, bucket_lo, bucket_path,
-                                path_states, path_stride, states, rec_, acts, reward, nullptr, hp, fx, acc, rep, nullptr, overflow, nullptr, 0,
-                                T_cap + 1, nullptr, nullptr, RNAD_HANDOVER ? &hand : nullptr, dd);
+    if constexpr (!DISTINCT) {
+        __shared__ AliveRow cnt[kThreads / 64];
+        __shared__ int32_t path_state[kMaxPath];
+        struct Late {
+            int32_t *alive_rep, *overflow;
+            double *norm_rep;
+            const int32_t *bucket_of;
+            unsigned long long *acc, *rep;
+            int64_t S;
+            int up_stride, n_groups;
+        };
+        __shared__ Late late_s;
+        const int my_item = xcd_item(*n_items);
+        if (my_item < 0) return;
+        const Item item = items[my_item];
+        if (threadIdx.x == 0) late_s = Late{alive_rep, overflow, norm_rep, bucket_of, acc, rep, S, up_stride, n_groups};
+        const PlayItem pi = rollout_prologue<false, kThreads>(item, T_cap, seed, sp, bucket_path, bucket_lo, path_states, path_stride, n_groups, cnt,
+                                                              nullptr, LeafCount{});
+        const LearnItem li = learn_prologue<A>(item, T_cap, sub_rows, path_words, n_groups, bucket_lo, bucket_path, path_states, path_stride, lds_all,
+                                               path_state);
+        double part[4] = {0.0, 0.0, 0.0, 0.0};
+        bool ovf = false;
+        for (int base = 0; base < item.count; base += kThreads) {
+            unsigned tid = threadIdx.x;
+            asm volatile("" : "+v"(tid));
+            rollout_pass<A, REL, 1, false, false>(pi, base, tid, trans, C, S, B, T_cap, policy_tab, tab_stride, vec4, lane0, lane_ids, decisions, states, acts,
+                                                  reward, nullptr, cnt, nullptr, RNAD_HANDOVER ? &hand : nullptr, dd, nullptr, nullptr);
+            asm volatile("" : "+v"(tid));
+            learn_pass<A, REL, false, false, false>(li, base, tid, item.count, T_cap, B, S, sub_rows, path_words, states, rec_, acts, reward, nullptr, hp, fx,
+                                                    lds_all, nullptr, RNAD_HANDOVER ? &hand : nullptr, dd, part, ovf);
+        }
+        const Late late = late_s;
+        rollout_epilogue<false, kThreads>(pi, T_cap, late.alive_rep + (int64_t)(blockIdx.x & (kReplicas - 1)) * (T_cap + 1), late.norm_rep, cnt,
+                                          nullptr, LeafCount{});
+        learn_epilogue<A>(lds_all, path_state, item, li.s_b, li.n_path, li.n_shared, path_words, sub_rows, late.S, late.n_groups, late.up_stride,
+                          late.bucket_of, part, ovf, nullptr, late.acc, late.rep, nullptr, late.overflow);
+    } else {
+        rollout_items_body<A, REL, 1, true>(trans, C, S, B, T_cap, policy_tab, tab_stride, vec4, seed, sp, lane0, lane_ids, decisions, items, n_items,
+                                            bucket_path, bucket_lo, path_states, path_stride, n_groups, states, alive_rep, acts, reward, nullptr,
+                                            norm_rep, RNAD_HANDOVER ? &hand : nullptr, dd);
+        learn_c_body<A, REL, false, true>(T_cap, B, S, sub_rows, path_words, n_groups, up_stride, items, n_items, bucket_of, bucket_lo, bucket_path,
+                                          path_states, path_stride, states, rec_, acts, reward, nullptr, hp, fx, acc, rep, nullptr, overflow, nullptr,
+                                          0, T_cap + 1, nullptr, nullptr, RNAD_HANDOVER ? &hand : nullptr, dd);
+    }
 }
 
 template <int A>
@@ -2677,6 +2818,11 @@
     out[10] = p.chunk;
     note_sized(tree, B, p);
     return 0;
+}
+
+extern "C" int rnad_fused_chunk(int64_t B, int n_buckets, int slots) {
+    const Switches sw = read_switches();
+    return fused_lane_chunk(B, n_buckets, slots, sw, sw.bucket_chunk.set ? std::max(64, sw.bucket_chunk.v) : kChunkDefault);
 }
 
 extern "C" int rnad_bucket_map(const rnad_tree_t *tree, int64_t B, int32_t *bucket_of, int32_t *n_groups) {
@@ -2857,13 +3003,37 @@
     int chunk;
     int distinct_keys;
     size_t lds;
+    bool equal_items = false;
+    int64_t grid = 0;
 };
-FusedPlan plan_fused(const rnad_tree_t *tree, const Plan &p, const Switches &sw, bool asked) {
+
+int64_t resident_slots(const void *kern, size_t lds) {
+    static std::mutex guard;
+    static std::map<std::tuple<int, const void *, size_t>, int64_t> known;
+    int dev = 0, cus = 0, per_cu = 0;
+    if (hipGetDevice(&dev) != hipSuccess) return 0;
+    std::lock_guard<std::mutex> lock(guard);
+    const auto key = std::make_tuple(dev, kern, lds);
+    auto it = known.find(key);
+    if (it != known.end()) return it->second;
+    if (hipDeviceGetAttribute(&cus, hipDeviceAttributeMultiprocessorCount, dev) != hipSuccess ||
+        hipOccupancyMaxActiveBlocksPerMultiprocessor(&per_cu, kern, kThreads, lds) != hipSuccess)
+        return 0;
+    return known[key] = (int64_t)cus * per_cu;
+}
+
+FusedPlan plan_fused(const rnad_tree_t *tree, int64_t B, const Plan &p, const Switches &sw, bool asked, const void *play_learn_lane) {
     if (sw.fused_distinct.set) asked = sw.fused_distinct.v != 0;
     const int keys = asked ? p.cut->rows * (tree->A * tree->A * tree->C + 1) : 0;
     auto lds_with = [&](int chunk) { return (size_t)p.lds + ((size_t)keys + 2 + 2 * (size_t)chunk) * 4; };
     FusedPlan f{p.chunk, 0, (size_t)p.lds};
-    if (keys == 0) return f;
+    if (keys == 0) {
+        const int64_t slots = sw.fused_slots.set ? 1 : resident_slots(play_learn_lane, f.lds);
+        if (slots > 0) f.chunk = fused_lane_chunk(B, p.cut->n_buckets, slots, sw, p.chunk);
+        f.equal_items = true;
+        f.grid = std::min<int64_t>(p.max_items, (int64_t)p.cut->n_buckets + B / f.chunk + 1 + 7);
+        return f;
+    }
     const int chunk = std::max(sw.fused_chunk.set ? std::max(64, sw.fused_chunk.v) : kFusedChunkDefault, p.chunk);
     if (lds_with(chunk) <= (size_t)kFusedLdsBudget) f.chunk = chunk;
     if ((f.chunk > p.chunk || sw.fused_chunk.set) && lds_with(f.chunk) <= (size_t)kFusedLdsBudget) {
@@ -2871,6 +3041,11 @@
         f.lds = lds_with(f.chunk);
     }
     return f;
+}
+
+int play_learn_lane_kernel(const rnad_tree_t *tree, const Plan &p, const void *&kern) {
+    RNAD_DISPATCH_REL(p, RNAD_DISPATCH_A(tree->A, kern = (const void *)k_bucket_play_learn<kA, REL, false>));
+    return 0;
 }
 
 struct RolloutCall {
@@ -2932,7 +3107,7 @@
     template <int A, class REL>
     int play_learn(const Accumulators &acc, const FixedPoint &fx) const {
         auto kern = fplan.distinct_keys > 0 ? k_bucket_play_learn<A, REL, true> : k_bucket_play_learn<A, REL, false>;
-        return launch_lds(kern, dim3((unsigned)p.max_items), dim3(kThreads), fplan.lds, stream, tree->trans, tree->C, S, B, rq.T_cap, policy_tab,
+        return launch_lds(kern, dim3((unsigned)(fplan.grid > 0 ? fplan.grid : p.max_items)), dim3(kThreads), fplan.lds, stream, tree->trans, tree->C, S, B, rq.T_cap, policy_tab,
                           policy_stride, vec4, seed, device_params, lane0, (const int32_t *)rq.sort.lane_ids, (const unsigned long long *)s.decisions,
                           (const Item *)rq.sort.items, (const int32_t *)rq.sort.n_items, (const int32_t *)cut.bucket_path,
                           (const int32_t *)cut.bucket_lo, (const int32_t *)cut.path_states, std::max(cut.max_path, 1), cut.n_groups,
@@ -3005,7 +3180,7 @@
                                                       (const int32_t *)cut.bucket_lo, (const int32_t *)cut.bucket_span, (const int32_t *)cut.group_by_lo,
                                                       rq.staged_rows, rq.n_staged, rq.out.visited, (const uint32_t *)stage.root, stage.sorted,
                                                       (const uint32_t *)stage.mark0, stage.root ? rq.stage_rows0 : nullptr, stage.counts, seed,
-                                                      device_params, s.bucket_start)) return rc);
+                                                      device_params, s.bucket_start, fplan.equal_items ? 1 : 0)) return rc);
         if (rq.group_flags)
             hipLaunchKernelGGL(k_group_flags, dim3(blocks_for(S)), dim3(kThreads), 0, stream, S, (const int32_t *)cut.bucket_of, cut.n_groups,
                                (const int32_t *)s.totals, rq.group_flags);
@@ -3051,8 +3226,13 @@
     if (int rc = plan_for(tree, rq.B, sw, "rnad_rollout_bucketed", true, p)) return rc;
     const int64_t B = rq.B, S = tree->S;
     const hipStream_t stream = rq.stream;
-    RolloutCall c{tree, rq, sw, p, *p.cut, carve_scratch(rq.sort.scratch, tree, B, p), carve_stage(rq.stage, B, S),
-                  rq.fused ? plan_fused(tree, p, sw, rq.fused->distinct) : FusedPlan{p.chunk, 0, (size_t)p.lds}, B, S,
+    FusedPlan fplan{p.chunk, 0, (size_t)p.lds};
+    if (rq.fused && !rq.fused->leaf) {
+        const void *kern = nullptr;
+        if (int rc = play_learn_lane_kernel(tree, p, kern)) return rc;
+        fplan = plan_fused(tree, B, p, sw, rq.fused->distinct, kern);
+    }
+    RolloutCall c{tree, rq, sw, p, *p.cut, carve_scratch(rq.sort.scratch, tree, B, p), carve_stage(rq.stage, B, S), fplan, B, S,
                   std::min(p.cut->max_path, rq.T_cap), stream, rq.draws.seed, rq.draws.lane0, rq.draws.device_params, rq.actor.table, rq.actor.stride, 0};
     ProfScope prof(PROF_ACT, stream);
     const bool sort_phase = (rq.phases & 1) != 0, play_phase = (rq.phases & 2) != 0;
diff --git a/r-nad_amd/rnad_hip/__init__.py b/r-nad_amd/rnad_hip/__init__.py
--- a/r-nad_amd/rnad_hip/__init__.py
+++ b/r-nad_amd/rnad_hip/__init__.py
@@ -843,7 +843,7 @@
 
 
 def plan_knobs():
-    return tuple(os.environ.get(k) for k in ("RNAD_BUCKET_ROWS", "RNAD_BUCKET_CHUNK", "RNAD_SORT_TILE"))
+    return tuple(os.environ.get(k) for k in ("RNAD_BUCKET_ROWS", "RNAD_BUCKET_CHUNK", "RNAD_SORT_TILE", "RNAD_FUSED_SLOTS"))
 
 
 def bucket_plan(tree, B):
```

New measurement: 65.62 billion env-steps/s. 10.0% lower.
